# justinmgarrigus/accel-sim-framework-distributed

Hardware: AMD Instinct MI355X
Metric: sim KIPS (whole node) (higher is better)
Workload: dtype n/a (integer cycle-level model)

## Files before the change

csrc/bindings/py_asim.cc:

```cpp
#include <chrono>
#include <pybind11/functional.h>
#include <pybind11/numpy.h>
#include <pybind11/pybind11.h>
#include <pybind11/stl.h>

#include <cstring>

#include "../config/icnt_config.h"
#include "../driver/icnt_bench.h"
#include "../driver/simulator.h"
#include "../engine/icnt_sweep.h"

namespace py = pybind11;
using namespace asim;
static const size_t kLinkPktBytes = sizeof(LinkPkt);

namespace {

py::dict link_dict(const LinkParams& p) {
  py::dict d;
  d["link_gbps"] = p.link_gbps;
  d["latency_ns"] = p.latency_ns;
  d["links"] = p.links;
  d["slice_bytes"] = p.slice_bytes;
// ... 137 lines not shown
  for (int i = 0; i < 7; ++i) a[an[i]] = r.activity[i];
  d["activity"] = a;
  py::dict e;
  e["buffer"] = r.e_buffer;
  e["crossbar"] = r.e_xbar;
  e["link"] = r.e_link;
  e["allocator"] = r.e_alloc;
  e["leakage"] = r.e_leak;
  d["energy_pj"] = e;
  d["power_w"] = r.power_w;
  return d;
}

static std::vector<RequestReplyParams> rr_points_from(const std::vector<py::dict>& points) {
  std::vector<RequestReplyParams> ps;
  for (const py::dict& d : points) {
    RequestReplyParams p;
    for (const auto& kv : d) {
      const std::string k = py::cast<std::string>(kv.first);
      const py::handle v = kv.second;
      if (k == "traffic") p.traffic = py::cast<std::string>(v);
      else if (k == "rate") p.rate = py::cast<double>(v);
      else if (k == "cycles") p.cycles = py::cast<uint64_t>(v);
      else if (k == "warmup") p.warmup = py::cast<uint64_t>(v);
      else if (k == "seed") p.seed = py::cast<uint64_t>(v);
      else if (k == "write_fraction") p.write_fraction = py::cast<double>(v);
      else if (k == "read_request_size") p.read_request_size = py::cast<uint32_t>(v);
      else if (k == "read_reply_size") p.read_reply_size = py::cast<uint32_t>(v);
      else if (k == "write_request_size") p.write_request_size = py::cast<uint32_t>(v);
      else if (k == "write_reply_size") p.write_reply_size = py::cast<uint32_t>(v);
      else if (k == "reply_delay") p.reply_delay = py::cast<uint64_t>(v);
      else if (k == "mem_nodes") p.mem_nodes = py::cast<uint32_t>(v);
      else throw std::invalid_argument("icnt_request_reply_batch: point " + std::to_string(ps.size()) +
                                       ": unknown field '" + k + "'");
    }
    ps.push_back(p);
  }
  return ps;
}

PYBIND11_MODULE(_asim, m) {
  m.doc() = "MI355X-native trace-driven GPU simulator (native core)";
  m.attr("sizeof_SMState") = sizeof(SMState);
  m.attr("sizeof_ChanState") = sizeof(ChanState);
  m.attr("offsetof_SMState_skipped") = offsetof(SMState, skipped_cycles);
  m.attr("epoch_dependent_SMState") = std::vector<std::pair<size_t, size_t>>{
      {offsetof(SMState, skey), sizeof(SMState::skey)}, {offsetof(SMState, sref), sizeof(SMState::sref)},
      {offsetof(SMState, srank), sizeof(SMState::srank)}, {offsetof(SMState, pub_nz), sizeof(SMState::pub_nz)},
      {offsetof(SMState, skipped_cycles), sizeof(SMState::skipped_cycles)}};
  m.attr("epoch_dependent_ChanState") = std::vector<std::pair<size_t, size_t>>{
      {offsetof(ChanState, skey), sizeof(ChanState::skey)}, {offsetof(ChanState, sref), sizeof(ChanState::sref)},
      {offsetof(ChanState, srank), sizeof(ChanState::srank)}, {offsetof(ChanState, pub_nz), sizeof(ChanState::pub_nz)}};
  m.attr("sizeof_TInst") = sizeof(TInst);

  m.def("gpu_available", &gpu_engine_available, "True if a HIP device is usable by the GPU engine");
  {
    py::dict lim;
    lim["max_warps"] = kMaxWarps;
    lim["max_cta"] = kMaxCta;
    lim["l1_lines"] = kMaxL1Lines;
    lim["l1_mshr"] = kMaxL1Mshr;
    lim["l2_lines_per_channel"] = kMaxL2LinesCh;
    lim["l2_mshr"] = kMaxL2Mshr;
    lim["sm_total"] = kMaxSmTot;
    lim["sub_total"] = kMaxSubTot;
    m.attr("limits") = lim;
  }
  m.def("gpu_cu_count", &gpu_cu_count, "compute units of the current HIP device");
  m.def("gpu_pool_stats", &gpu_pool_stats, "GPU engine caching allocator: cached bytes, caps, trims");
  m.def("gpu_engine_modes", &gpu_engine_modes, "per GPU-engine build (lds / global / split): LDS bytes, blocks per CU, registers");
  m.def("gpu_batch_stats", &gpu_batch_stats, "global-state batch launches: batches, launches, blocks per CU");
  m.def("gpu_pool_trim", &gpu_pool_trim, "give the GPU engine allocator's cached blocks back to the driver");
  m.def("gpu_cus_per_sim", &gpu_cus_per_sim, "CUs one GPU-engine simulation of this shape reserves (ASIM_GPU_STATE)");
  m.def("gpu_engine_kernel_info", []() {
    const EngineKernelInfo k = gpu_engine_kernel_info();
    py::dict d;
    if (!k.valid) return d;
    d["vgprs_per_lane"] = k.num_regs;
    d["scratch_bytes_per_lane"] = k.local_bytes;
    d["lds_static"] = k.shared_static;
    d["lds_dynamic"] = k.lds_dynamic;
    d["max_threads_per_block"] = k.max_threads;
    d["binary_version"] = k.binary_version;
    d["sm_state_bytes"] = k.sm_state_bytes;
    d["chan_state_bytes"] = k.chan_state_bytes;
    return d;
  }, "compiled resources of the persistent HIP engine kernel (needs a GPU)");
  m.def("option_names", []() {
    OptionRegistry r;
    register_sim_options(r);
    return r.names();
  });
  m.def("unmodelled_option_warnings", [](const std::vector<std::string>& args) {
    OptionRegistry r;
    register_sim_options(r);
    r.parse_cmdline(args, false);
    return unmodelled_option_warnings(r);
  }, "warnings for options that are accepted but have no effect");
  m.def("parse_config", [](const std::vector<std::string>& args) { return cfg_dict(cfg_from_args(args)); },
        "derive the model configuration from accel-sim style arguments");
  m.def("addr_decode", [](const std::vector<std::string>& args, uint64_t addr) {
    SimCfg c = cfg_from_args(args);
    AddrTlx t = addr_decode(c, addr);
    py::dict d;
    d["chip"] = t.chip;
    d["bk"] = t.bk;
// ... 843 lines not shown
```

csrc/config/sim_options.cc:

```cpp
#include "sim_options.h"

#include <unistd.h>

#include "icnt_config.h"
#include "../model/addrdec.h"

#include <algorithm>
#include <cmath>
#include <cstring>
#include <sstream>

namespace asim {

namespace {

struct OptDef {
  const char* name;
  char type;
  const char* deflt;
  const char* help;
};

const OptDef kOptions[] = {
    {"-trace", 's', "./traces/kernelslist.g", "traces kernel list file"},
// ... 270 lines not shown
    {"-sim_check_corrupt_mailbox", 'u', "0", "-sim_engine check self-test: perturb a request-mailbox count instead of a unit state"},
    {"-sim_epochs_per_launch", 'u', "4096", "GPU engine epochs per persistent launch"},
    {"-sim_debug", 'b', "0", "interactive timing debugger (reference gpgpu_debug; also GPGPUSIM_DEBUG=1): single step, "
                            "PC / cycle breakpoints, memory-line watchpoints, pipeline dumps"},
    {"-sim_debug_script", 's', "", "debugger commands from this file instead of stdin"},
    {"-sim_debug_step", 'u', "0", "cycles per debugger step (0: one PDES epoch)"},
    {"-sim_break_cycle", 'u', "0", "enter the debugger when the simulation reaches this cycle (reference g_single_step)"},
    {"-collective_model", 's', "const", "const | ring | tree | packet collective timing"},
    {"-xgmi_link_bandwidth_gbps", 'f', "153.0", "per-link xGMI bandwidth (GB/s)"},
    {"-xgmi_link_latency_ns", 'f', "1000.0", "collective step latency (ns)"},
    {"-xgmi_links_per_gpu", 'u', "7", "xGMI links per GPU"},
    {"-sim_event_skip", 'b', "1", "fast-forward quiet SM cycles inside an epoch (results identical)"},
    {"-power_in_loop", 'b', "1",
     "power samples taken by the engine inside its cycle loop (GPU engine: in engine_kernel, f64 MFMA sums), "
     "0 = one engine run per sample with the host evaluating (results identical; DVFS always uses the latter)"},
    {"-trace_host_budget_mb", 'f', "0",
     "read a kernel's text trace per thread block, as the trace window advances, when the file is larger than this "
     "many MiB: host trace memory then follows the window (-gpu_trace_window, 2 when 0) instead of the kernel "
     "(0 = load whole kernels; results identical)"},
    {"-gpu_trace_window", 'i', "4",
     "GPU engine: kernel trace resident in HBM per kernel, in multiples of its resident-CTA capacity; CTAs "
     "stream in as they dispatch (0 = whole kernel; results identical)"},
    {"-sim_xcd", 'u', "0",
     "XCDs with private L2s (0 = one shared L2): SM s belongs to XCD s % N and uses the n_subpart/N slices of its XCD"},
    {"-sim_mall", 's', "none",
     "memory-attached last-level cache (Infinity Cache) per DRAM channel: <sets>:<assoc> of 128 B sectored lines, or none"},
    {"-sim_mall_miss_latency", 'u', "0", "extra core cycles of an HBM access over a MALL hit"},
    {"-sim_host_launch_interval", 'u', "0",
     "host model: core cycles between the host's kernel submissions after a sync (0 = a host that is never the "
     "bottleneck); a kernel submitted after the previous one ended launches into an idle GPU"},
    {"-sim_kernel_min_cycles_queued", 'u', "0",
     "a kernel queued right behind another lasts at least this many core cycles (the command processor's "
     "back-to-back dispatch interval of dependent kernels; 0 = off)"},
    {"-sim_first_kernel_latency", 'u', "0",
     "extra launch cycles of the run's first kernel behind the initial host copies (cold start: the copies' "
     "completion and the first touch of their pages; ub_launch after-copy)"},
    {"-sim_copy_latency_every_kernel", 'b', "0",
     "apply -sim_first_kernel_latency to every kernel launched behind a host copy, not only the run's first "
     "(ub_launch measures it on every one of its copy -> kernel repetitions)"},
    {"-collective_mem_traffic", 'b', "0",
     "run every collective's local memory traffic (send-buffer reads, receive-buffer writes) as an RCCL-style copy "
     "kernel that loads the simulated L2/MALL/HBM and contends with overlapping kernels"},
    {"-sim_l1_write_request_bytes", 'u', "128",
     "largest L1 -> L2 write request: 64 sends a store touching both halves of a line as two requests (gfx950 "
     "TCP -> TCC), 128 one per line"},
    {"-sim_single_valu", 'b', "0",
     "CDNA: integer, fp64 and transcendental vector instructions issue through the SIMD's one VALU (the SP unit of "
     "their scheduler, at their own initiation interval) instead of separate INT / DP / SFU pipelines"},
    {"-sim_l2_kernel_release", 'b', "0",
     "at the end of every kernel write the L2s' dirty sectors back to memory (the MALL if any) and invalidate them "
     "(the release / acquire of a multi-XCD GPU, whose XCD L2s are not coherent with each other)"},
    {"-sim_cpu_threads", 'u', "1", "CPU engine: OpenMP threads over the units of one epoch (1 = serial; "
                                  "run simulations job-parallel instead)"},
    {"-sim_router_pass", 's', "serial",
     "-icnt_link_contention 2: serial | par, the epoch pass over the routers: one lane (rt_simulate) or the "
     "lane-parallel pass (rt_simulate_par; on the GPU engine 64 lanes and one block per subnet); same results"},
    {"-sim_router_step_cap", 'u', "0",
     "-sim_router_pass par: loop iterations after which a pass gives up with an error (0 = the pass's own bound; "
     "a diagnostic)"},
    {"-icnt_capture", 's', "",
     "write every SM-to-L2 request and L2-to-SM reply packet the cycle engine injects to this file "
     "(model/icnt_capture.h; replay it with the standalone network mode)"},
    {"-icnt_capture_buf_kb", 'u', "0",
     "-icnt_capture: KB of the engine's log per subnet (0 = default; a diagnostic: a small log forces many "
     "hand-overs, on the GPU engine many launches)"},
    {"-collective_slice_bytes", 'u', "131072", "packet model: bytes per link packet (RCCL slice)"},
    {"-collective_max_channels", 'u', "16", "packet model: max parallel rings (channels)"},
    {"-collective_reduce_gbps", 'f', "900.0", "packet model: local memory bandwidth for reduce/copy (GB/s)"},
};

uint32_t parse_u(const std::string& s, const char* what) {
  char* end = nullptr;
  std::string t = trim(s);
  unsigned long v = strtoul(t.c_str(), &end, 0);
  if (t.empty() || *end) throw OptionError(std::string("bad integer '") + s + "' in " + what);
  return (uint32_t)v;
}

std::pair<uint32_t, uint32_t> parse_lat_ii(const std::string& s, const char* what) {
  auto v = split(strip_ws(s), ',');
  if (v.size() < 2) throw OptionError(std::string("expected <latency,initiation> for ") + what);
  return {parse_u(v[0], what), parse_u(v[1], what)};
}

void mask_limits(uint64_t m, uint8_t& hi, uint8_t& lo) {
  if (!m) {
    hi = 0;
    lo = 0;
    return;
  }
  lo = (uint8_t)__builtin_ctzll(m);
  hi = (uint8_t)(64 - __builtin_clzll(m));
}

uint32_t log2_floor(uint32_t x) {
  uint32_t r = 0;
  while ((1u << (r + 1)) <= x) ++r;
  return r;
}

void setup_addrdec(SimCfg& c, const std::string& mapping, int mask_mode) {
  int chip_s = 10;
  uint64_t m[AF_COUNT] = {0x0000000000001C00ull, 0x0000000000000300ull, 0x000000000FFF0000ull,
                          0x000000000000E0FFull, 0x000000000000000Full};
  switch (mask_mode) {
    case 0:
// ... 498 lines not shown
  c.rw_turnaround = r.getb("-dram_elimnate_rw_turnaround") ? 0u : 1u;
  c.wq_enable = r.getb("-dram_seperate_write_queue_enable") ? 1u : 0u;
  {
    auto v = split(strip_ws(r.gets("-dram_write_queue_size")), ':');
    if (v.size() != 3) throw OptionError("-dram_write_queue_size expects <size>:<high>:<low>");
    c.wq_size = parse_u(v[0], "-dram_write_queue_size");
    c.wq_hi = parse_u(v[1], "-dram_write_queue_size");
    c.wq_lo = parse_u(v[2], "-dram_write_queue_size");
    if (c.wq_enable) {
      c.wq_size = std::max<uint32_t>(1, std::min<uint32_t>(c.wq_size, kDramQ / 2));
      c.dram_queue = std::min<uint32_t>(c.dram_queue, (uint32_t)kDramQ - c.wq_size);
      c.wq_hi = std::min(c.wq_hi, c.wq_size);
      c.wq_lo = std::min(c.wq_lo, c.wq_hi);
    }
  }
  c.BL = (uint32_t)r.getu("-gpgpu_dram_burst_length");
  c.busW = (uint32_t)r.getu("-gpgpu_dram_buswidth");
  c.data_cmd_ratio = std::max<uint32_t>(1, (uint32_t)r.getu("-dram_data_command_freq_ratio"));
  c.dual_bus = (uint32_t)r.getu("-dram_dual_bus_interface");
  c.perfect_mem = r.getb("-gpgpu_perfect_mem") ? 1u : 0u;
  c.simple_dram = r.getb("-gpgpu_simple_dram_model") ? 1u : 0u;
  c.event_skip = r.getb("-sim_event_skip") ? 1u : 0u;
  c.trace_window = (uint32_t)std::max<long long>(0, r.geti("-gpu_trace_window"));
  {
    c.l1_wr_req_bytes = (uint32_t)r.getu("-sim_l1_write_request_bytes");
    c.single_valu = r.getb("-sim_single_valu") ? 1u : 0u;
    if (c.l1_wr_req_bytes != 64 && c.l1_wr_req_bytes != 128)
      throw OptionError("-sim_l1_write_request_bytes must be 64 or 128");
    c.n_xcd = (uint32_t)r.getu("-sim_xcd");
    c.log2_spx = 0;
    if (c.n_xcd > 1) {
      if (c.n_subpart % c.n_xcd) throw OptionError("-sim_xcd must divide the number of L2 sub-partitions");
      if (c.n_xcd > (uint32_t)kMaxXcd || c.n_xcd > c.n_sm)
        throw OptionError("-sim_xcd: at most " + std::to_string(kMaxXcd) + " XCDs and no more than the SMs");
      const uint32_t spx = c.n_subpart / c.n_xcd;
      if (spx & (spx - 1)) throw OptionError("-sim_xcd: sub-partitions per XCD must be a power of two");
      while ((1u << c.log2_spx) < spx) ++c.log2_spx;
    } else {
      c.n_xcd = 0;
    }
    c.mall_sets = c.mall_assoc = 0;
    const std::string m = strip_ws(r.gets("-sim_mall"));
    if (!m.empty() && m != "none" && m != "0") {
      auto v = split(m, ':');
      if (v.size() != 2) throw OptionError("-sim_mall expects <sets>:<assoc>");
      c.mall_sets = parse_u(v[0], "-sim_mall");
      c.mall_assoc = parse_u(v[1], "-sim_mall");
      if (!c.mall_sets || (c.mall_sets & (c.mall_sets - 1)) || !c.mall_assoc || c.mall_assoc > 64)
        throw OptionError("-sim_mall: sets must be a power of two and 1 <= assoc <= 64");
    }
    c.mall_miss_fs = (uint64_t)r.getu("-sim_mall_miss_latency");
  }
  c.cpu_threads = r.getu("-sim_cpu_threads");
  {
    const std::string rp = strip_ws(r.gets("-sim_router_pass"));
    if (rp != "serial" && rp != "par") throw OptionError("-sim_router_pass must be serial or par, not '" + rp + "'");
    c.router_pass = rp == "par" ? 1u : 0u;
    c.router_step_cap = r.getu("-sim_router_step_cap");
  }
  c.trace_mask = 0;
  if (r.getb("-trace_enabled")) {
    static const std::pair<const char*, uint32_t> streams[] = {
        {"WARP_SCHEDULER", TS_WARP_SCHEDULER},
        {"SCOREBOARD", TS_SCOREBOARD},
        {"MEMORY_PARTITION_UNIT", TS_MEMORY_PARTITION_UNIT},
        {"MEMORY_SUBPARTITION_UNIT", TS_MEMORY_SUBPARTITION_UNIT},
        {"INTERCONNECT", TS_INTERCONNECT},
        {"LIVENESS", TS_LIVENESS}};
    for (auto& tok : split(strip_ws(r.gets("-trace_components")), ',')) {
      if (tok.empty() || tok == "none") continue;
      bool found = false;
      for (auto& s : streams)
        if (tok == s.first || tok == "all") {
          c.trace_mask |= s.second;
          found = true;
        }
      if (!found) throw OptionError("-trace_components: unknown stream " + tok);
    }
  }
  c.trace_sm = (int32_t)r.geti("-trace_sampling_core");
  c.trace_mem = (int32_t)r.geti("-trace_sampling_memory_partition");
  c.trace_cap = 1u << 16;
  c.trace_ev = nullptr;
  c.trace_cnt = nullptr;
  c.bk_index_policy = (uint32_t)r.getu("-dram_bnk_indexing_policy");
  c.bkgrp_index_policy = (uint32_t)r.getu("-dram_bnkgrp_indexing_policy");
  c.atom_size = c.BL * c.busW * (uint32_t)r.getu("-gpgpu_n_mem_per_ctrlr");
  setup_addrdec(c, trim(r.gets("-gpgpu_mem_addr_mapping")), (int)r.geti("-gpgpu_mem_address_mask"));
  {
    uint32_t pi = (uint32_t)r.getu(user_set("-memory_partition_indexing") ? "-memory_partition_indexing"
                                                                           : "-gpgpu_memory_partition_indexing");
    if (pi > 5) throw OptionError("-gpgpu_memory_partition_indexing out of range");
    c.part_index = (uint8_t)pi;
  }
  {
    auto v = split(strip_ws(r.gets("-gpgpu_clock_domains")), ':');
    if (v.size() != 4) throw OptionError("-gpgpu_clock_domains expects 4 frequencies");
    double f[4];
    for (int i = 0; i < 4; ++i) {
      f[i] = atof(v[i].c_str());
      if (f[i] <= 0) throw OptionError("clock frequency must be positive");
    }
    c.per_core = (uint64_t)llround(1e9 / f[0]);
    c.per_icnt = (uint64_t)llround(1e9 / f[1]);
    c.per_l2 = (uint64_t)llround(1e9 / f[2]);
    c.per_dram = (uint64_t)llround(1e9 / f[3]);
// ... 182 lines not shown
```

csrc/driver/debugger.cc:

```cpp
#include "debugger.h"

#include <cstdio>
#include <fstream>
#include <iostream>
#include <sstream>

namespace asim {

Debugger::Debugger(const std::string& script, uint64_t stop_at, Hooks hooks) : h_(std::move(hooks)), stop_at_(stop_at) {
  if (!script.empty()) {
    file_.reset(new std::ifstream(script));
    if (!*file_) throw std::runtime_error("-sim_debug_script: cannot read " + script);
    from_file_ = true;
  }
  stepping_ = stop_at == 0;
  steps_left_ = stepping_ ? 1 : 0;
}

bool Debugger::next_line(std::string& line) {
  if (from_file_) return (bool)std::getline(*file_, line);
  std::fputs("(asim debugger) ", stdout);
  std::fflush(stdout);
  return (bool)std::getline(std::cin, line);
}

void Debugger::help() {
  h_.print(
      "asim debugger commands:\n"
      "  s [n]              step n steps (default 1) of -sim_debug_step cycles\n"
      "  c                  continue to the next breakpoint / watchpoint\n"
      "  b <pc> [sm] [warp] break when a warp issues the instruction at pc (hex)\n"
      "  bc <cycle>         break when the simulation reaches a cycle\n"
      "  w <addr>           watch memory requests to the 128 B line holding addr (hex)\n"
      "  d <id>             delete a breakpoint / watchpoint\n"
      "  l                  list breakpoints and watchpoints\n"
      "  dp [sm]            dump the pipeline of an SM (default: every busy SM)\n"
      "  dm [ch]            dump a memory channel (default: every busy channel)\n"
      "  i                  run status (cycle, instructions)\n"
      "  q                  stop the simulation here\n"
      "  h                  this help\n");
}

bool Debugger::after_step(uint64_t now, const std::vector<TraceEv>& ev, uint32_t n_sm, uint32_t l2_num,
                          uint32_t l2_den) {
  if (quit_) return false;
  bool stop = false;
  char b[256];
  for (const TraceEv& e : ev)
    for (auto& kv : bps_) {
      Bp& bp = kv.second;
      bool hit = false;
      if (bp.kind == Bp::PC && e.kind == EV_ISSUE && (e.b & 0xffffffffull) == bp.v &&
          (bp.sm < 0 || e.unit == (uint32_t)bp.sm) && (bp.warp < 0 || e.a == (uint16_t)bp.warp)) {
        hit = true;
        snprintf(b, sizeof(b), "asim debugger: breakpoint %d hit: core %u warp %u issued pc 0x%llx at cycle %llu\n",
                 kv.first, e.unit, e.a, (unsigned long long)bp.v, (unsigned long long)e.cycle);
      } else if (bp.kind == Bp::ADDR && (e.b >> 7) == (bp.v >> 7)) {
        if (e.kind == EV_PKT_SEND && e.unit < n_sm) {
          hit = true;
          snprintf(b, sizeof(b),
                   "asim debugger: watchpoint %d hit: core %u sends a request for line 0x%llx (addr 0x%llx) to "
                   "sub-partition %u at cycle %llu\n",
                   kv.first, e.unit, (unsigned long long)e.b, (unsigned long long)bp.v, e.a,
                   (unsigned long long)e.cycle);
        } else if (e.kind == EV_L2_ACCESS) {
          static const char* o[] = {"hit", "miss", "mshr-hit", "write-through"};
          hit = true;
          snprintf(b, sizeof(b),
                   "asim debugger: watchpoint %d hit: channel %u sub %u L2 %s for line 0x%llx at cycle ~%llu\n",
                   kv.first, e.unit - n_sm, e.a >> 8, o[e.a & 3], (unsigned long long)e.b,
                   (unsigned long long)(l2_den ? e.cycle * l2_num / l2_den : e.cycle));
        }
      }
      if (hit) {
        ++bp.hits;
        h_.print(b);
        stop = true;
      }
    }
  for (auto& kv : bps_)
    if (kv.second.kind == Bp::CYCLE && !kv.second.hits && now >= kv.second.v) {
      ++kv.second.hits;
      snprintf(b, sizeof(b), "asim debugger: breakpoint %d hit: cycle %llu reached (now %llu)\n", kv.first,
               (unsigned long long)kv.second.v, (unsigned long long)now);
      h_.print(b);
      stop = true;
    }
  if (stop_at_ && now >= stop_at_) {
    stop_at_ = 0;
    stop = true;
  }
// ... 34 lines not shown
      bp.v = std::stoull(pc, nullptr, 16);
      is >> bp.sm >> bp.warp;
      bps_[next_id_] = bp;
      snprintf(b, sizeof(b), "breakpoint %d at pc 0x%llx\n", next_id_++, (unsigned long long)bp.v);
      h_.print(b);
    } else if (cmd == "bc") {
      Bp bp{Bp::CYCLE, 0};
      if (!(is >> bp.v)) {
        h_.print("usage: bc <cycle>\n");
        continue;
      }
      bps_[next_id_] = bp;
      snprintf(b, sizeof(b), "breakpoint %d at cycle %llu\n", next_id_++, (unsigned long long)bp.v);
      h_.print(b);
    } else if (cmd == "w" || cmd == "watch") {
      std::string a;
      if (!(is >> a)) {
        h_.print("usage: w <addr>\n");
        continue;
      }
      Bp bp{Bp::ADDR, std::stoull(a, nullptr, 16)};
      bps_[next_id_] = bp;
      snprintf(b, sizeof(b), "watchpoint %d on line 0x%llx\n", next_id_++, (unsigned long long)(bp.v & ~127ull));
      h_.print(b);
    } else if (cmd == "d" || cmd == "delete") {
      int id = 0;
      is >> id;
      h_.print(bps_.erase(id) ? "deleted\n" : "no such breakpoint\n");
    } else if (cmd == "l" || cmd == "list") {
      if (bps_.empty()) h_.print("no breakpoints\n");
      for (auto& kv : bps_) {
        const Bp& p = kv.second;
        if (p.kind == Bp::PC)
          snprintf(b, sizeof(b), "%d: break pc 0x%llx sm %d warp %d (hits %llu)\n", kv.first,
                   (unsigned long long)p.v, p.sm, p.warp, (unsigned long long)p.hits);
        else if (p.kind == Bp::CYCLE)
          snprintf(b, sizeof(b), "%d: break cycle %llu (hits %llu)\n", kv.first, (unsigned long long)p.v,
                   (unsigned long long)p.hits);
        else
          snprintf(b, sizeof(b), "%d: watch line 0x%llx (hits %llu)\n", kv.first, (unsigned long long)(p.v & ~127ull),
                   (unsigned long long)p.hits);
        h_.print(b);
      }
    } else if (cmd == "dp") {
      int sm = -1;
      is >> sm;
      h_.print(h_.dump(sm, -2));
    } else if (cmd == "dm") {
      int ch = -1;
      is >> ch;
      h_.print(h_.dump(-2, ch));
    } else if (cmd == "i" || cmd == "info") {
      h_.print(h_.status() + "\n");
    } else if (cmd == "q" || cmd == "quit") {
      quit_ = true;
      h_.print("asim debugger: simulation stopped by the user\n");
      return false;
    } else if (cmd == "h" || cmd == "help") {
      help();
    } else {
      h_.print("unknown command '" + cmd + "' (h for help)\n");
    }
  }
  bps_.clear();
  stepping_ = false;
  return true;
}

}
```

csrc/driver/debugger.h:

```cpp
#pragma once
#include <cstdint>
#include <functional>
#include <istream>
#include <map>
#include <memory>
#include <string>
#include <vector>

#include "../model/config.h"

namespace asim {

class Debugger {
 public:
  struct Hooks {
    std::function<void(const std::string&)> print;
    std::function<std::string(int sm, int ch)> dump;
    std::function<std::string()> status;
  };
  Debugger(const std::string& script, uint64_t stop_at, Hooks hooks);

  static uint32_t trace_mask() { return TS_WARP_SCHEDULER | TS_INTERCONNECT | TS_MEMORY_SUBPARTITION_UNIT; }

  bool after_step(uint64_t now, const std::vector<TraceEv>& ev, uint32_t n_sm, uint32_t l2_to_core_num,
                  uint32_t l2_to_core_den);

  size_t commands_run() const { return ncmd_; }

 private:
  struct Bp {
    enum Kind { PC, ADDR, CYCLE } kind;
    uint64_t v;
    int sm = -1;
    int warp = -1;
    uint64_t hits = 0;
  };
  bool prompt(uint64_t now);
  bool next_line(std::string& line);
  void help();

  Hooks h_;
  std::unique_ptr<std::istream> file_;
  bool from_file_ = false;
  bool stepping_ = true;
  uint64_t steps_left_ = 0;
  uint64_t stop_at_ = 0;
  std::map<int, Bp> bps_;
  int next_id_ = 1;
  size_t ncmd_ = 0;
  bool quit_ = false;
};

}
```

csrc/driver/simulator.cc:

```cpp
#include "simulator.h"

#include <sys/stat.h>

#include <algorithm>
#include <cmath>
#include <cstdarg>
#include <cstring>
#include <filesystem>
#include <stdexcept>

namespace asim {

template <class T>
static void stat_delta(const std::vector<T>& a, const std::vector<T>& b, std::vector<T>& out) {
  static_assert(sizeof(T) % 8 == 0, "stat structs are arrays of 64-bit counters");
  out.resize(a.size());
  for (size_t i = 0; i < a.size(); ++i) {
    const uint64_t* x = (const uint64_t*)&a[i];
    uint64_t* o = (uint64_t*)&out[i];
    if (i < b.size()) {
      const uint64_t* y = (const uint64_t*)&b[i];
      for (size_t k = 0; k < sizeof(T) / 8; ++k) o[k] = x[k] - y[k];
    } else {
      for (size_t k = 0; k < sizeof(T) / 8; ++k) o[k] = x[k];
// ... 46 lines not shown
  }
  ~CaptureFile() override {
    try {
      finish();
    } catch (...) {
    }
  }
};

uint64_t Simulator::icnt_capture_packets(uint32_t subnet) const { return capture_ ? capture_->h.count[subnet ? 1 : 0] : 0; }

Simulator::Simulator(const std::vector<std::string>& args) {
  t_start_ = std::chrono::steady_clock::now();
  register_sim_options(reg_);
  reg_.parse_cmdline(args, false);
  cfg_ = derive_sim_cfg(reg_);
  dopt_ = derive_driver_opts(reg_);
  if (dopt_.engine == "gpu") {
    eng_ = make_gpu_engine();
    if (!eng_) throw std::runtime_error("-sim_engine gpu requested but the HIP engine is unavailable");
    if (dopt_.gpu_ingest) ingest_dev_ = gpu_current_device();
  } else if (dopt_.engine == "cpu") {
    eng_ = make_cpu_engine();
  } else if (dopt_.engine == "check") {
    std::unique_ptr<Engine> primary;
    if (dopt_.check_primary == "gpu") {
      primary = make_gpu_engine();
      if (!primary) throw std::runtime_error("-sim_engine check: the HIP engine is unavailable");
    } else if (dopt_.check_primary == "cpu") {
      primary = make_cpu_engine();
    } else {
      throw OptionError("-sim_check_primary must be cpu or gpu");
    }
    eng_ = make_check_engine(std::move(primary), make_cpu_engine(), dopt_.check_interval, dopt_.check_corrupt_at,
                             dopt_.check_corrupt_mailbox != 0);
  } else {
    throw OptionError("-sim_engine must be cpu, gpu or check");
  }
  print_mask_ = cfg_.trace_mask;
  if (dopt_.debug) {
    cfg_.trace_mask |= Debugger::trace_mask();
    print_sm_ = cfg_.trace_sm;
    print_mem_ = cfg_.trace_mem;
    cfg_.trace_sm = -1;
    cfg_.trace_mem = -1;
    Debugger::Hooks h;
    h.print = [this](const std::string& s) { print("%s", s.c_str()); };
    h.dump = [this](int sm, int ch) { return dump_pipeline(sm, ch); };
    h.status = [this]() {
      char b[200];
      snprintf(b, sizeof(b), "cycle %llu, kernels completed %zu, thread instructions of completed kernels %llu",
               (unsigned long long)eng_->now(), results_.size(), (unsigned long long)tot_insn_);
      return std::string(b);
    };
    dbg_.reset(new Debugger(dopt_.debug_script, dopt_.break_cycle, h));
  }
  eng_->init(cfg_);
  if (!dopt_.icnt_capture.empty()) {
    capture_.reset(new CaptureFile(dopt_.icnt_capture, cfg_));
    eng_->capture_arm(capture_.get(), dopt_.icnt_capture_buf_kb);
  } else if (dopt_.icnt_capture_buf_kb) {
    throw OptionError("-icnt_capture_buf_kb needs -icnt_capture");
  }
  per_core_nom_ = cfg_.per_core;
  if (dopt_.power_enabled) {
    power_.reset(new PowerModel());
    std::string err;
    if (!power_->load_xml(dopt_.power_xml, &err)) throw std::runtime_error("power model: " + err);
    power_->set_param("dvfs_min_clock_ratio",
                      std::max(power_->param("dvfs_min_clock_ratio", 0.0), dopt_.dvfs_min_clock_ratio));
    power_report_.reset(new std::ofstream(dopt_.power_report_file));
    if (!*power_report_) throw std::runtime_error("cannot write " + dopt_.power_report_file);
    if (power_->param("energy_model", 0.0) >= 1.0) {
      ArchEnergyParams ap;
      ap.node_nm = power_->param("core_tech_node", ap.node_nm);
      ap.vdd = power_->param("core_vdd", 0.0);
      ap.dram_pj_per_bit = power_->param("dram_pj_per_bit", ap.dram_pj_per_bit);
      ap.dram_act_nj = power_->param("dram_act_nj", ap.dram_act_nj);
      ap.tensor_macs_per_lane = power_->param("tensor_macs_per_lane", 0.0);
      const ArchEnergy ae = arch_energy(cfg_, ap);
      power_->set_base(ae.base_nj);
      *power_report_ << "architectural energy model (energy_model = 1)\n" << arch_energy_report(ae) << "\n";
    }
    if (dopt_.power_trace) {
      power_trace_.reset(new std::ofstream("accelwattch_power_trace.csv"));
      ptrack_.write_trace_header(*power_trace_);
    }
    if (dopt_.steady_power) {
      power_steady_.reset(new std::ofstream("accelwattch_steady_state.csv"));
      *power_steady_ << "kernel,start_cycle,end_cycle,samples,avg_power\n";
      ptrack_.set_steady(dopt_.steady_dev_pct, dopt_.steady_samples);
    }
  }
  if (dopt_.visualizer) {
    visualizer_.reset(new std::ofstream(dopt_.visualizer_file));
    if (!*visualizer_) throw std::runtime_error("cannot write " + dopt_.visualizer_file);
  }
}

Simulator::~Simulator() = default;

void Simulator::print(const char* fmt, ...) {
  char buf[4096];
  va_list ap;
  va_start(ap, fmt);
  int n = vsnprintf(buf, sizeof(buf), fmt, ap);
// ... 1351 lines not shown
```

csrc/engine/cpu_engine.cc:

```cpp
#include <cstdlib>
#include <cstring>
#include <stdexcept>

#include <functional>

#include <atomic>
#include <exception>
#include <mutex>

#include "../model/icnt_router_par.h"
#include "engine.h"
#include "thread_team.h"
#include "trace_window.h"

namespace asim {

uint32_t reply_cap(const SimCfg& c) {
  uint64_t win = (uint64_t)c.icnt_latency * std::max(c.per_core, c.per_core_max);
  return (uint32_t)((win + c.per_icnt - 1) / c.per_icnt + 1);
}

uint32_t icnt_cap_log_records(const SimCfg& c, uint32_t cap_req, uint32_t cap_rep, uint64_t buf_kb) {
  const uint64_t worst = icnt_cap_epoch_max(c, std::max(cap_req, cap_rep));
  const uint64_t min_kb = (worst * sizeof(IcntCapRec) + 1023) / 1024;
  if (!buf_kb)
    buf_kb = std::max(min_kb, std::min(kIcntCapMaxDefaultKb, std::max(kIcntCapDefaultKb, kIcntCapDefaultEpochs * min_kb)));
  const uint64_t recs = buf_kb * 1024 / sizeof(IcntCapRec);
  if (recs < worst)
    throw std::invalid_argument("-icnt_capture_buf_kb " + std::to_string(buf_kb) +
                                ": the log must hold one epoch's worst case, " + std::to_string(worst) +
                                " records per subnet: at least " + std::to_string(min_kb) + " KB");
  return (uint32_t)std::min<uint64_t>(recs, 0x7fffffffu);
}

void check_core_clock(const SimCfg& c, uint64_t per_core) {
  if (per_core == 0 || per_core > std::max(c.per_core, c.per_core_max))
    throw std::runtime_error("set_core_clock: core period beyond the configured DVFS range (-dvfs_min_clock_ratio)");
}

void init_sm_state(SMState& s, uint32_t id) {
  memset(&s, 0, sizeof(SMState));
  s.id = id;
}

void init_chan_state(ChanState& ch, uint32_t id, const SimCfg& c) {
  memset(&ch, 0, sizeof(ChanState));
  ch.id = id;
  ch.t_icnt = 0;
  ch.t_l2 = 0;
  ch.t_dram = 0;
  (void)c;
}

void host_memcpy_fill(ChanState* chs, uint32_t nch, const SimCfg& c, uint64_t addr, uint64_t bytes) {
  if (c.l2.disabled || c.n_xcd) return;
  const uint64_t first = addr & ~127ull;
  const uint64_t last = (addr + bytes + 127) & ~127ull;
  uint64_t cap_lines = (uint64_t)c.l2.nsets * c.l2.assoc * c.n_subpart;
  uint64_t start = first;
  if ((last - first) / 128 > 2 * cap_lines) start = last - 2 * cap_lines * 128;
  for (uint64_t line = start; line < last; line += 128) {
    AddrTlx t = addr_decode(c, line);
    uint32_t ch = t.sub / c.n_sub_per_mem, sub = t.sub % c.n_sub_per_mem;
    if (ch >= nch) continue;
// ... 20 lines not shown
  if (h.n_sm != w.n_sm || h.n_mem != w.n_mem || h.sm_bytes != w.sm_bytes || h.ch_bytes != w.ch_bytes ||
      h.pub_bytes != w.pub_bytes || h.box_req != w.box_req || h.cnt_req != w.cnt_req || h.box_rep != w.box_rep ||
      h.cnt_rep != w.cnt_rep || h.ovf != w.ovf || h.mall != w.mall || h.links != w.links)
    throw std::runtime_error("engine state: image was written for a different configuration or build");
}

void host_flush_l2(ChanState* chs, uint32_t nch, const SimCfg& c, bool writeback, L2Line* mall) {
  const uint32_t per_sub = c.l2.nsets * c.l2.assoc;
  for (uint32_t i = 0; i < nch; ++i) {
    ChanState& ch = chs[i];
    if (writeback && !c.l2.disabled) {
      for (uint32_t j = 0; j < c.n_sub_per_mem; ++j) {
        MemStats& st = ch.sp[j].st;
        const L2Line* T = l2_tags(ch, c, j);
        for (uint32_t k = 0; k < per_sub; ++k) {
          const L2Line& L = T[k];
          if (!L.dirty) continue;
          const uint32_t n = (uint32_t)popc64(L.dirty);
          st.l2_mem_wr += n;
          st.l2_mem_wr_req += wr_requests(L.dirty);
          st.l2_evict_dirty++;
          if (!mall) {
            st.dram_wr += n;
            continue;
          }
          L2Line* b = mall + (size_t)i * mall_lines(c) + (size_t)mall_set(c, L.tag) * c.mall_assoc;
          int w = mall_find<SeqPar>(b, c.mall_assoc, L.tag);
          if (w < 0) {
            w = mall_victim<SeqPar>(b, c.mall_assoc);
            if (b[w].valid && b[w].dirty) {
              const uint32_t nv = (uint32_t)popc64(b[w].dirty);
              ch.sp[0].st.mall_wb += nv;
              ch.sp[0].st.dram_wr += nv;
            }
            b[w] = L2Line{};
            b[w].tag = L.tag;
          }
          b[w].valid |= L.dirty;
          b[w].dirty |= L.dirty;
          b[w].lru = ++ch.mall_stamp;
          ch.sp[0].st.mall_wr += n;
        }
      }
    }
    for (auto& L : ch.l2) {
      L.valid = 0;
      L.dirty = 0;
    }
  }
}

namespace {

class CpuEngine : public Engine {
 public:
  const char* name() const override { return "cpu"; }

  void init(const SimCfg& c) override {
    c_ = c;
    sms_.assign(c.n_sm, SMState());
    for (uint32_t i = 0; i < c.n_sm; ++i) init_sm_state(sms_[i], i);
    chs_.assign(c.n_mem, ChanState());
    for (uint32_t i = 0; i < c.n_mem; ++i) init_chan_state(chs_[i], i, c);
    pub_.reset(new EpochPub());
    memset(pub_.get(), 0, sizeof(EpochPub));
    cap_req_ = c.icnt_latency;
    cap_rep_ = reply_cap(c);
    for (int p = 0; p < 2; ++p) {
      box_req_[p].assign((size_t)c.n_subpart * c.n_sm * cap_req_, Pkt{});
      cnt_req_[p].assign((size_t)c.n_subpart * c.n_sm, 0);
      box_rep_[p].assign((size_t)c.n_sm * c.n_subpart * cap_rep_, Pkt{});
      cnt_rep_[p].assign((size_t)c.n_sm * c.n_subpart, 0);
    }
    ovf_cap_ = backlog_cap(c);
    ovf_.assign((size_t)c.n_subpart * ovf_cap_, Pkt{});
    mall_.assign((size_t)(c.n_mem * mall_lines(c)), L2Line{});
    link_free_.clear();
    link_refs_.clear();
    n_link_state_ = 0;
    rt_pc_ = RtPassCount{};
    if (c.link_contention && (icnt_link_count(c) > kMaxIcntLinks || !icnt_contention_fits(c, cap_req_, cap_rep_) ||
                              icnt_scratch_words(c, cap_req_, cap_rep_) > kMaxIcntScratchWords))
      throw std::runtime_error("-icnt_link_contention: topology or mailboxes too large for the link pass");
    if (icnt_contention_on(c)) {
      n_link_state_ = (size_t)icnt_state_words(c, cap_req_, cap_rep_);
      link_free_.assign(n_link_state_ + kIcntStatWords, 0);
      link_refs_.assign((size_t)icnt_scratch_words(c, cap_req_, cap_rep_), 0);
    }
    epoch_ = 0;
    cycle_ = 0;
    kt_ = KernelTab{};
    kt_.mix = c.concurrent_kernel_sm;
    if (c_.trace_mask) {
      const size_t units = (size_t)c.n_sm + c.n_mem;
      trace_ev_.assign(units * c_.trace_cap, TraceEv{});
      trace_cnt_.assign(units, 0);
      c_.trace_ev = trace_ev_.data();
      c_.trace_cnt = trace_cnt_.data();
    }
  }

  void trace_drain(std::vector<TraceEv>& out, uint64_t* dropped) override {
    out.clear();
    for (size_t u = 0; u < trace_cnt_.size(); ++u) {
      const uint32_t n = trace_cnt_[u], k = std::min(n, c_.trace_cap);
      out.insert(out.end(), trace_ev_.begin() + (long)(u * c_.trace_cap), trace_ev_.begin() + (long)(u * c_.trace_cap + k));
      if (dropped) *dropped += n - k;
      trace_cnt_[u] = 0;
    }
  }

  void launch(uint32_t slot, ReadyKernel& k, const KernelDesc& kd) override {
    if (slot >= (uint32_t)kMaxConc || (kt_.active >> slot & 1u)) throw std::runtime_error("launch: kernel slot busy");
    if (!k.streamed() && k.insts.size() > kIdxMask) throw std::runtime_error("kernel trace exceeds 2^29 warp instructions");
    KernelDesc& d = kt_.k[slot];
    d = kd;
    tw_.launch(slot, k, d, c_);
    kt_.active |= 1u << slot;
  }
  uint32_t running() const override { return kt_.active; }

  RunResult run(const RunLimits& lim) override {
    RunResult res;
    if (!kt_.active) {
      res.end_cycle = cycle_;
      return res;
    }
    const uint32_t nthr = std::max<uint32_t>(1, std::min<uint32_t>(c_.cpu_threads, (uint32_t)(sms_.size() + chs_.size())));
    bar_.reset(nthr);
    const uint64_t epoch0 = epoch_, cycle0 = cycle_;
    uint64_t end_epoch = epoch0, end_cycle = cycle0;
    std::atomic<bool> abort{false};
    std::exception_ptr err;
    std::mutex err_mu;
    auto fail = [&]() {
      std::lock_guard<std::mutex> g(err_mu);
      if (!err) err = std::current_exception();
      abort.store(true, std::memory_order_release);
    };
    std::function<void(uint32_t)> job = [&](uint32_t tid) {
      const SimCfg& c = c_;
      const uint64_t E = c.icnt_latency;
      const int nsm = (int)sms_.size(), nch = (int)chs_.size();
      uint64_t epoch = epoch0, cycle = cycle0, epochs = 0;
      bool refill = true;
      uint64_t pw_next = pw_on_ ? pw_.t_prev + pw_.freq : 0;
      uint64_t reqm[2] = {~0ull, ~0ull}, repm[2] = {~0ull, ~0ull};
      RunResult r;
      for (;;) {
        if (refill && tw_.any_streamed()) {
          if (nthr > 1) bar_.wait();
          if (tid == 0) {
            try {
              tw_.ensure(kt_, c, [&](DispatchView& v) { read_dispatch(v); });
            } catch (...) {
              fail();
            }
          }
          if (nthr > 1) bar_.wait();
          if (abort.load(std::memory_order_acquire)) break;
        }
        const uint32_t cur = (uint32_t)(epoch & 1), prev = cur ^ 1u;
        const uint64_t t0 = cycle, t1 = t0 + E;
        const int s0 = (int)((uint64_t)nsm * tid / nthr), s1 = (int)((uint64_t)nsm * (tid + 1) / nthr);
        const int c0 = (int)((uint64_t)nch * tid / nthr), c1 = (int)((uint64_t)nch * (tid + 1) / nthr);
        try {
        for (int q = 0; q < (s1 - s0) + (c1 - c0); ++q) {
          const int i = q < s1 - s0 ? s0 + q : nsm + c0 + (q - (s1 - s0));
          if (i < nsm) {
            SMState& s = sms_[i];
            SmCtx x = ctx_sm(cur);
            sm_epoch<SeqPar>(s, x, *pub_, prev, t0, t1, box_rep_[prev].data(), cnt_rep_[prev].data(), cap_rep_,
                             c.n_subpart, epoch, repm);
            sm_publish<SeqPar>(s, x, *pub_, cur);
          } else {
            ChanState& ch = chs_[i - nsm];
            MemCtx m = ctx_mem(cur, t1);
            m.mall = mall_.empty() ? nullptr : mall_.data() + (size_t)(i - nsm) * mall_lines(c);
            chan_epoch<SeqPar>(ch, m, box_req_[prev].data(), cnt_req_[prev].data(), cap_req_, core_fs(c, t0), reqm);
            chan_publish<SeqPar>(ch, m, *pub_, cur);
          }
        }
        } catch (...) {
          fail();
        }
        if (nthr > 1) bar_.wait();
        if (abort.load(std::memory_order_acquire)) break;
        if (cap_sink_ && tid == 0) {
          try {
            capture_epoch(cur);
          } catch (...) {
            fail();
          }
        }
        if (!link_free_.empty()) {
          if (tid == 0) {
            try {
              if (router_par()) {
                if (rt_epoch_run_par<SeqPar>(c, box_req_[cur].data(), cnt_req_[cur].data(), cap_req_,
                                             box_rep_[cur].data(), cnt_rep_[cur].data(), cap_rep_, link_free_.data(),
                                             link_refs_.data(), RT_DIR_BOTH, &rt_pc_) != RT_STATUS_OK)
                  throw std::runtime_error(kRouterStepCapMsg);
              } else {
                icnt_epoch_pass<SeqPar>(c, box_req_[cur].data(), cnt_req_[cur].data(), cap_req_, box_rep_[cur].data(),
                                        cnt_rep_[cur].data(), cap_rep_, link_free_.data(), link_refs_.data());
              }
            } catch (...) {
              fail();
            }
          }
          if (nthr > 1) bar_.wait();
          if (abort.load(std::memory_order_acquire)) break;
        }
        const uint64_t mc = pw_on_ ? (lim.max_cycle ? std::min(lim.max_cycle, pw_next) : pw_next) : lim.max_cycle;
        const EpochDecision d = epoch_decide<SeqPar>(c, *pub_, cur, t1, kt_, epoch, mc);
        refill = d.refill != 0;
        reqm[0] = d.req_dst[0];
        reqm[1] = d.req_dst[1];
        repm[0] = d.rep_dst[0];
        repm[1] = d.rep_dst[1];
        ++epoch;
        ++epochs;
        cycle = d.next_start;
        if (pw_on_) {
          const bool exits = d.done || d.deadlock || d.limit || (lim.max_cycle && cycle >= lim.max_cycle) ||
                             (lim.max_epochs && epochs >= lim.max_epochs);
          if (exits || cycle >= pw_next) {
            if (tid == 0) {
              try {
                power_sample(cycle);
              } catch (...) {
                fail();
              }
            }
            if (nthr > 1) bar_.wait();
            if (abort.load(std::memory_order_acquire)) break;
            pw_next = cycle + pw_.freq;
          }
        }
        if (d.done) {
          r.done = true;
          r.done_mask = d.done;
        } else if (d.deadlock) {
          r.deadlock = true;
        } else if (d.limit) {
          r.hit_limit = true;
          r.cap = true;
        } else if ((lim.max_cycle && cycle >= lim.max_cycle) || (lim.max_epochs && epochs >= lim.max_epochs)) {
          r.hit_limit = true;
        } else {
          continue;
        }
        break;
      }
      if (tid == 0) {
        r.epochs = epochs;
        res = r;
        end_epoch = epoch;
        end_cycle = cycle;
      }
    };
    team_.run(nthr, job);
    if (err) std::rethrow_exception(err);
    if (cap_sink_) capture_flush();
    epoch_ = end_epoch;
    cycle_ = end_cycle;
    if (res.done) {
      kt_.active &= ~res.done_mask;
      for (uint32_t k = 0; k < (uint32_t)kMaxConc; ++k)
        if (res.done_mask >> k & 1u) tw_.done(k);
    }
    res.end_cycle = cycle_;
    return res;
  }

  uint64_t now() const override { return cycle_; }
  void trace_residency(uint64_t* peak_bytes, uint64_t* refills) const override {
    *peak_bytes = tw_.resident_peak;
    *refills = tw_.refills;
  }
  bool power_sampler() const override { return true; }
  void power_arm(const PwrArm& a) override {
    pw_ = a;
    pw_on_ = true;
    pw_out_.clear();
  }
  void power_disarm() override { pw_on_ = false; }
  void power_drain(std::vector<PwrSample>& out) override {
    out.swap(pw_out_);
    pw_out_.clear();
  }
  void power_sample(uint64_t now) {
    std::vector<const MemStats*> mem;
    for (auto& ch : chs_)
      for (uint32_t j = 0; j < c_.n_sub_per_mem; ++j) mem.push_back(&ch.sp[j].st);
    std::vector<const SMStats*> sm(sms_.size());
    for (size_t i = 0; i < sms_.size(); ++i) sm[i] = &sms_[i].st;
    double S[PS_COUNT];
    pwr_sums_of(sm.data(), sm.size(), mem.data(), mem.size(), S);
    pw_out_.push_back(pwr_take(pw_, S, now));
  }
  void read_dispatch(DispatchView& v) const {
    const SMState& s0 = sms_[0];
    memcpy(v.k_uid, s0.k_uid, sizeof(v.k_uid));
    memcpy(v.next_cta, s0.next_cta, sizeof(v.next_cta));
    memcpy(v.next_ctax, s0.next_ctax, sizeof(v.next_ctax));
    v.sms.resize(sms_.size());
    for (size_t m = 0; m < sms_.size(); ++m) {
      memcpy(v.sms[m].cta_id, sms_[m].cta_id, sizeof(v.sms[m].cta_id));
      memcpy(v.sms[m].cta_valid, sms_[m].cta_valid, sizeof(v.sms[m].cta_valid));
      memcpy(v.sms[m].cta_ks, sms_[m].cta_ks, sizeof(v.sms[m].cta_ks));
    }
  }
  struct HostMem {
// ... 15 lines not shown
    host_memcpy_fill(chs_.data(), (uint32_t)chs_.size(), c_, addr, bytes);
  }
  void set_core_clock(uint64_t per_core, uint64_t base_cyc, uint64_t base_fs) override {
    check_core_clock(c_, per_core);
    c_.per_core = per_core;
    c_.clk_base_cyc = base_cyc;
    c_.clk_base_fs = base_fs;
    cfg_set_divs(c_);
  }
  void flush_l2(bool writeback) override {
    host_flush_l2(chs_.data(), (uint32_t)chs_.size(), c_, writeback, mall_.empty() ? nullptr : mall_.data());
  }

  void stats(std::vector<SMStats>& sm, std::vector<MemStats>& mem) override {
    sm.clear();
    mem.clear();
    for (auto& s : sms_) sm.push_back(s.st);
    for (auto& ch : chs_)
      for (uint32_t j = 0; j < c_.n_sub_per_mem; ++j) mem.push_back(ch.sp[j].st);
  }

  void snapshot(std::vector<uint8_t>& out) override {
    out.resize(sms_.size() * sizeof(SMState) + chs_.size() * sizeof(ChanState) + mall_.size() * sizeof(L2Line) +
               n_link_state_ * 8);
    uint8_t* p = out.data();
    for (auto& s : sms_) {
      memcpy(p, &s, sizeof(SMState));
      p += sizeof(SMState);
    }
    for (auto& ch : chs_) {
      memcpy(p, &ch, sizeof(ChanState));
      p += sizeof(ChanState);
    }
    if (!mall_.empty()) memcpy(p, mall_.data(), mall_.size() * sizeof(L2Line));
    p += mall_.size() * sizeof(L2Line);
    if (n_link_state_) memcpy(p, link_free_.data(), n_link_state_ * 8);
  }
  void restore(const std::vector<uint8_t>& in) override {
    if (in.size() != sms_.size() * sizeof(SMState) + chs_.size() * sizeof(ChanState) + mall_.size() * sizeof(L2Line) +
                         n_link_state_ * 8)
      throw std::runtime_error("snapshot size mismatch");
    const uint8_t* p = in.data();
    for (auto& s : sms_) {
      memcpy(&s, p, sizeof(SMState));
      p += sizeof(SMState);
    }
    for (auto& ch : chs_) {
      memcpy(&ch, p, sizeof(ChanState));
      p += sizeof(ChanState);
    }
    if (!mall_.empty()) memcpy(mall_.data(), p, mall_.size() * sizeof(L2Line));
    p += mall_.size() * sizeof(L2Line);
    if (n_link_state_) memcpy(link_free_.data(), p, n_link_state_ * 8);
  }
  void link_stats(uint64_t* delayed, uint64_t* wait_cycles, uint64_t* deadlocked) override {
    *delayed = n_link_state_ ? link_free_[n_link_state_] : 0;
    *wait_cycles = n_link_state_ ? link_free_[n_link_state_ + 1] : 0;
    if (deadlocked) *deadlocked = n_link_state_ ? link_free_[n_link_state_ + 2] : 0;
  }
  void capture_arm(IcntCapSink* sink, uint64_t buf_kb) override {
    uint32_t recs = icnt_cap_log_records(c_, cap_req_, cap_rep_, buf_kb);
    const uint64_t worst = icnt_cap_epoch_max(c_, std::max(cap_req_, cap_rep_));
    if (!buf_kb) recs = (uint32_t)std::min<uint64_t>(recs, std::max<uint64_t>(worst, 65536));
    for (int d = 0; d < 2; ++d) {
      cap_rec_[d].assign(recs, IcntCapRec{});
      cap_off_[d].assign((size_t)c_.n_sm * c_.n_subpart, 0);
      cap_log_[d] = IcntCapLog{cap_rec_[d].data(), cap_off_[d].data(), 0, recs};
    }
    cap_sink_ = sink;
  }
  void capture_epoch(uint32_t cur) {
    const uint64_t worst = icnt_cap_epoch_max(c_, std::max(cap_req_, cap_rep_));
    if (cap_log_[0].n + worst > cap_log_[0].cap || cap_log_[1].n + worst > cap_log_[1].cap) capture_flush();
    icnt_capture_append<SeqPar>(c_, 0, box_req_[cur].data(), cnt_req_[cur].data(), cap_req_, &cap_log_[0]);
    icnt_capture_append<SeqPar>(c_, 1, box_rep_[cur].data(), cnt_rep_[cur].data(), cap_rep_, &cap_log_[1]);
  }
  void capture_flush() {
    for (uint32_t d = 0; d < 2; ++d) {
      if (cap_log_[d].n) cap_sink_->put(d, cap_log_[d].rec, cap_log_[d].n);
      cap_log_[d].n = 0;
    }
  }
  bool router_par() const { return c_.link_contention == 2 && c_.router_pass == 1 && !link_free_.empty(); }
  RouterPassStats router_pass_stats() override {
    RouterPassStats r;
    r.mode = c_.router_pass == 1 ? "par" : "serial";
    if (!router_par()) return r;
    r.passes = rt_pc_.passes[0] + rt_pc_.passes[1];
    r.max_packets_req = rt_pc_.max_np[0];
    r.max_packets_rep = rt_pc_.max_np[1];
    r.split_blocks = 1;
    return r;
  }
  void advance(uint64_t cycles) override {
    uint64_t E = c_.icnt_latency;
    cycle_ += (cycles + E - 1) / E * E;
  }

  EngineStateHeader header() const {
    EngineStateHeader h;
    h.n_sm = sms_.size();
    h.n_mem = chs_.size();
    h.sm_bytes = sizeof(SMState);
    h.ch_bytes = sizeof(ChanState);
    h.pub_bytes = sizeof(EpochPub);
    h.box_req = box_req_[0].size();
    h.cnt_req = cnt_req_[0].size();
    h.box_rep = box_rep_[0].size();
    h.cnt_rep = cnt_rep_[0].size();
    h.ovf = ovf_.size();
    h.mall = mall_.size();
    h.links = link_free_.size();
    h.cycle = cycle_;
    h.epoch = epoch_;
    h.ready = kt_.active;
    return h;
  }

  void save_state(std::vector<uint8_t>& out) override {
    out.clear();
    StateOut o{out};
    EngineStateHeader h = header();
    o.put(&h, sizeof(h));
    o.put(sms_.data(), sms_.size() * sizeof(SMState));
    o.put(chs_.data(), chs_.size() * sizeof(ChanState));
    o.put(pub_.get(), sizeof(EpochPub));
    for (int p = 0; p < 2; ++p) {
      o.put(box_req_[p].data(), box_req_[p].size() * sizeof(Pkt));
      o.put(cnt_req_[p].data(), cnt_req_[p].size() * sizeof(uint32_t));
      o.put(box_rep_[p].data(), box_rep_[p].size() * sizeof(Pkt));
      o.put(cnt_rep_[p].data(), cnt_rep_[p].size() * sizeof(uint32_t));
    }
    o.put(ovf_.data(), ovf_.size() * sizeof(Pkt));
    o.put(mall_.data(), mall_.size() * sizeof(L2Line));
    if (!link_free_.empty()) o.put(link_free_.data(), link_free_.size() * 8);
  }

  void load_state(const std::vector<uint8_t>& in) override {
    StateIn r{in};
    EngineStateHeader h;
    r.get(&h, sizeof(h));
    check_state_header(h, header());
    r.get(sms_.data(), sms_.size() * sizeof(SMState));
    r.get(chs_.data(), chs_.size() * sizeof(ChanState));
    r.get(pub_.get(), sizeof(EpochPub));
    for (int p = 0; p < 2; ++p) {
      r.get(box_req_[p].data(), box_req_[p].size() * sizeof(Pkt));
      r.get(cnt_req_[p].data(), cnt_req_[p].size() * sizeof(uint32_t));
      r.get(box_rep_[p].data(), box_rep_[p].size() * sizeof(Pkt));
      r.get(cnt_rep_[p].data(), cnt_rep_[p].size() * sizeof(uint32_t));
    }
    r.get(ovf_.data(), ovf_.size() * sizeof(Pkt));
    r.get(mall_.data(), mall_.size() * sizeof(L2Line));
    if (!link_free_.empty()) r.get(link_free_.data(), link_free_.size() * 8);
    cycle_ = h.cycle;
    epoch_ = h.epoch;
    if (h.ready) throw std::runtime_error("engine state: image taken with kernels running");
  }

 private:
  SmCtx ctx_sm(uint32_t cur) {
    SmCtx x;
    x.cfg = &c_;
    x.kt = &kt_;
    x.outbox = box_req_[cur].data();
    x.outcnt = cnt_req_[cur].data();
    x.out_cap = cap_req_;
    x.n_src_sm = c_.n_sm;
    x.rt_st = c_.link_contention == 2 && !link_free_.empty() ? link_free_.data() : nullptr;
    return x;
  }
  MemCtx ctx_mem(uint32_t cur, uint64_t t1) {
    MemCtx m;
    m.cfg = &c_;
    m.outbox = box_rep_[cur].data();
    m.outcnt = cnt_rep_[cur].data();
    m.out_cap = cap_rep_;
    m.n_src_sub = c_.n_subpart;
    m.win_end = core_fs(c_, t1);
    m.ovf = ovf_.data();
    m.ovf_cap = ovf_cap_;
    m.mall = nullptr;
    m.rt_st = c_.link_contention == 2 && !link_free_.empty() ? link_free_.data() : nullptr;
    return m;
  }

  SimCfg c_{};
  std::vector<SMState> sms_;
  std::vector<ChanState> chs_;
  std::unique_ptr<EpochPub> pub_;
  std::vector<Pkt> box_req_[2], box_rep_[2];
  std::vector<uint32_t> cnt_req_[2], cnt_rep_[2];
  uint32_t cap_req_ = 0, cap_rep_ = 0;
  std::vector<Pkt> ovf_;
  std::vector<L2Line> mall_;
  uint32_t ovf_cap_ = 0;
  std::vector<uint64_t> link_free_;
  std::vector<uint32_t> link_refs_;
  size_t n_link_state_ = 0;
  RtPassCount rt_pc_{};
  IcntCapSink* cap_sink_ = nullptr;
  std::vector<IcntCapRec> cap_rec_[2];
  std::vector<uint32_t> cap_off_[2];
  IcntCapLog cap_log_[2]{};
  uint64_t epoch_ = 0, cycle_ = 0;
  KernelTab kt_{};
};

}

std::unique_ptr<Engine> make_cpu_engine() { return std::unique_ptr<Engine>(new CpuEngine()); }

}
```

csrc/engine/engine.h:

```cpp
#pragma once
#include <cstring>
#include <memory>
#include <stdexcept>
#include <map>
#include <string>
#include <vector>

#include "../model/epoch.h"
#include "../model/icnt_capture.h"
#include "../power/power_eval.h"
#include "../trace/trace.h"

namespace asim {

struct RunLimits {
  uint64_t max_cycle = 0;
  uint64_t max_epochs = 0;
};

struct PwrArm {
  PwrCoef coef;
  uint64_t freq = 0;
  uint64_t t_prev = 0;
  double s_prev[PS_COUNT] = {};
  uint32_t n_sm = 0;
};

struct RunResult {
  uint64_t end_cycle = 0;
  uint64_t epochs = 0;
  bool done = false;
  uint32_t done_mask = 0;
  bool deadlock = false;
  bool hit_limit = false;
  bool cap = false;
};

struct RouterPassStats {
  const char* mode = "serial";
  uint64_t passes = 0;
  uint32_t max_packets_req = 0, max_packets_rep = 0;
  uint32_t split_blocks = 0;
};
constexpr const char* kRouterStepCapMsg = "router pass hit its step cap (-sim_router_step_cap / rt_step_cap)";

struct IcntCapSink {
  virtual ~IcntCapSink() = default;
  virtual void put(uint32_t subnet, const IcntCapRec* rec, size_t n) = 0;
};
constexpr uint64_t kIcntCapDefaultKb = 4096, kIcntCapMaxDefaultKb = 256 * 1024;
constexpr uint64_t kIcntCapDefaultEpochs = 256;
uint32_t icnt_cap_log_records(const SimCfg& c, uint32_t cap_req, uint32_t cap_rep, uint64_t buf_kb);

class Engine {
 public:
  virtual ~Engine() = default;
  virtual const char* name() const = 0;
  virtual void init(const SimCfg& c) = 0;
  virtual void launch(uint32_t slot, ReadyKernel& k, const KernelDesc& kd) = 0;
  virtual RunResult run(const RunLimits& lim) = 0;
  virtual uint32_t running() const = 0;
  virtual uint64_t now() const = 0;
  virtual void memcpy_fill_l2(uint64_t addr, uint64_t bytes) = 0;
  virtual void flush_l2(bool writeback = false) = 0;
  virtual void set_core_clock(uint64_t per_core, uint64_t base_cyc, uint64_t base_fs) = 0;
  virtual void stats(std::vector<SMStats>& sm, std::vector<MemStats>& mem) = 0;
  virtual void snapshot(std::vector<uint8_t>& out) = 0;
  virtual void restore(const std::vector<uint8_t>& in) = 0;
  virtual void advance(uint64_t cycles) = 0;
  virtual void save_state(std::vector<uint8_t>& out) = 0;
  virtual void load_state(const std::vector<uint8_t>& in) = 0;
  virtual void trace_drain(std::vector<TraceEv>& out, uint64_t* dropped) = 0;
  virtual void trace_residency(uint64_t* peak_bytes, uint64_t* refills) const {
    *peak_bytes = 0;
    *refills = 0;
  }
  virtual uint64_t launches() const { return 0; }
  virtual const char* kernel_variant() const { return ""; }
  virtual uint32_t kernel_blocks() const { return 0; }
  virtual void link_stats(uint64_t* delayed, uint64_t* wait_cycles, uint64_t* deadlocked = nullptr) {
    *delayed = 0;
    *wait_cycles = 0;
    if (deadlocked) *deadlocked = 0;
  }
  virtual RouterPassStats router_pass_stats() { return RouterPassStats{}; }
  virtual void capture_arm(IcntCapSink*, uint64_t ) {
    throw std::runtime_error("engine cannot capture the network traffic");
  }
  virtual bool power_sampler() const { return false; }
  virtual void power_arm(const PwrArm&) { throw std::runtime_error("engine has no in-loop power sampler"); }
  virtual void power_disarm() {}
  virtual void power_drain(std::vector<PwrSample>& out) { out.clear(); }
};

inline void pwr_sums_of(const SMStats* const* sm, size_t nsm, const MemStats* const* mem, size_t nmem, double* S) {
  for (int j = 0; j < PS_COUNT; ++j) S[j] = 0;
// ... 102 lines not shown
```

csrc/engine/gpu_engine.hip:

```cpp
#include <hip/hip_runtime.h>

#include <algorithm>
#include <cerrno>
#include <csignal>
#include <cstdio>
#include <cstring>
#include <map>
#include <memory>
#include <stdexcept>
#include <string>

#include <fcntl.h>
#include <sys/file.h>
#include <sys/stat.h>
#include <unistd.h>
#include <chrono>
#include <condition_variable>
#include <deque>
#include <mutex>
#include <vector>

#include "engine_kernel.h"
#include "trace_window.h"

// ... 1168 lines not shown
  uint32_t* d_cap_off_[2] = {nullptr, nullptr};
  uint32_t cap_recs_ = 0, cap_epochs_ = 0;
  uint32_t cap_win_left_ = 0;
  std::vector<IcntCapRec> cap_host_;
  uint32_t ovf_cap_ = 0;
  Pkt* d_box_req_[2] = {nullptr, nullptr};
  uint32_t* d_cnt_req_[2] = {nullptr, nullptr};
  Pkt* d_box_rep_[2] = {nullptr, nullptr};
  uint32_t* d_cnt_rep_[2] = {nullptr, nullptr};
  GpuCtl* d_ctl_ = nullptr;
  GpuCtl* h_ctl_ = nullptr;
  TraceEv* d_trace_ev_ = nullptr;
  uint32_t* d_trace_cnt_ = nullptr;
  struct DevMem {
    static constexpr bool kHost = false;
    void* alloc(size_t n) {
      void* p = nullptr;
      pool_alloc(&p, n);
      return p;
    }
    void free(void* p) {
      DevicePool::get().dev_free(p);
    }
    void write(void* d, const void* h, size_t n) { HIPCHECK(hipMemcpy(d, h, n, hipMemcpyHostToDevice)); }
  };
  TraceWindows<DevMem> tw_;
  uint64_t launches_ = 0;
  const char* variant_ = "";
  bool pw_on_ = false;
  PwrDev* d_pw_ = nullptr;
  double* d_pw_rows_ = nullptr;
  PwrSample* d_pw_ring_ = nullptr;
  uint32_t pw_cap_ = 0;
  std::vector<PwrSample> pw_out_;
  KernelTab kt_{};
  KernelTab* d_kt_ = nullptr;
  uint32_t cap_req_ = 0, cap_rep_ = 0;
  uint64_t epoch_ = 0, cycle_ = 0;
  uint32_t epochs_per_launch_ = 4096;
  bool profiling_ = false;
  bool sliced_ = false;
  int mode_ = kModeLds;
  bool global_ = false;
  bool batch_ = false;
  uint32_t slots_ = kCuSlots;
  uint64_t* d_prof_ = nullptr;
  uint32_t* d_ework_ = nullptr;

 public:
  void dump_profile() {
    if (!profiling_) return;
    std::vector<uint64_t> h((size_t)nblocks_ * kProfSlots);
    HIPCHECK(hipMemcpy(h.data(), d_prof_, h.size() * 8, hipMemcpyDeviceToHost));
    static const char* names[kProfSlots] = {
        "sm.receive", "sm.writeback", "sm.hit_complete", "sm.ldst", "sm.dispatch", "sm.read_operands",
        "sm.alloc_oc", "sm.issue", "sm.fetch", "sm.retire", "sm.inject", "sm.occupancy", "sm.gather",
        "sm.cta_dispatch", "sm.refill", "sm.cycle_loop", "sm.publish", "#sm_cycles", "#quiet_checks", "#epochs_busy", "mem.gather", "mem.dram",
        "mem.l2", "mem.icnt", "mem.window_other", "mem.publish", "barrier", "decide", "post", "sm.issue_sched", "#slowest", "launch_rest",
        "#max_work/epoch", "#epochs(b0)", "#last_arriver_wait", "#last_arrivals", "ldst.l1_probe", "ldst.mshr_find",
        "ldst.pend_reg", "ldst.send", "recv.xbar", "recv.l1_fill", "issue.one", "issue.pick", "quiet_check", "skip",
        "ldst.hit_push", "fill.pend_wake", "iss.pick", "iss.classify", "iss.step1", "iss.step2", "iss.step3",
        "iss.spare53", "iss.spare54", "iss.spare55"};
    double sm[kProfSlots] = {}, mc[kProfSlots] = {}, smt = 0, mct = 0;
    for (uint32_t b = 0; b < nblocks_; ++b)
      for (int k = 0; k < kProfSlots; ++k) {
        double v = (double)h[(size_t)b * kProfSlots + k];
        const bool counter = (k >= 17 && k <= 19) || k == 30 || (k >= 32 && k <= 35);
        if (b < c_.n_sm) { sm[k] += v / c_.n_sm; smt += counter ? 0 : v / c_.n_sm; }
        else { const double nmb = nblocks_ > c_.n_sm ? (double)(nblocks_ - c_.n_sm) : 1.0; mc[k] += v / nmb; mct += counter ? 0 : v / nmb; }
      }
    {
      double cyc_clk = 0, n_cyc = 0, n_q = 0, n_ep = 0, q_clk = 0;
      for (uint32_t b = 0; b < c_.n_sm; ++b) {
        for (int k = 0; k <= 11; ++k) cyc_clk += (double)h[(size_t)b * kProfSlots + k];
        for (int k = 36; k <= 43; ++k) cyc_clk += (double)h[(size_t)b * kProfSlots + k];
        cyc_clk += (double)h[(size_t)b * kProfSlots + 29] + (double)h[(size_t)b * kProfSlots + 46] +
                   (double)h[(size_t)b * kProfSlots + 47];
        for (int k = 48; k <= 52; ++k) cyc_clk += (double)h[(size_t)b * kProfSlots + k];
        q_clk += (double)h[(size_t)b * kProfSlots + 44] + (double)h[(size_t)b * kProfSlots + 45];
        n_cyc += (double)h[(size_t)b * kProfSlots + 17];
        n_q += (double)h[(size_t)b * kProfSlots + 18];
        n_ep += (double)h[(size_t)b * kProfSlots + 19];
      }
      fprintf(stderr, "[asim gpu profile] SM cycles simulated %.0f (%.0f clocks each), quiet checks %.0f "
                      "(cycle_loop %.0f clocks each), busy SM-epochs %.0f\n",
              n_cyc, n_cyc ? cyc_clk / n_cyc : 0, n_q, n_q ? q_clk / n_q : 0, n_ep);
    }
    {
      double mx = 0, ne = 0, lw = 0, nl = 0;
      for (uint32_t b = 0; b < nblocks_; ++b) {
        mx += (double)h[(size_t)b * kProfSlots + 32];
        ne += (double)h[(size_t)b * kProfSlots + 33];
        lw += (double)h[(size_t)b * kProfSlots + 34];
        nl += (double)h[(size_t)b * kProfSlots + 35];
      }
      fprintf(stderr, "[asim gpu profile] epochs %.0f: slowest block's work %.0f clocks/epoch; last arriver's "
                      "barrier wait %.0f clocks/epoch (pure barrier latency)\n",
              ne, ne ? mx / ne : 0, nl ? lw / nl : 0);
    }
    {
      std::vector<std::pair<uint64_t, uint32_t>> sl;
      for (uint32_t b = 0; b < nblocks_; ++b) sl.push_back({h[(size_t)b * kProfSlots + 30], b});
      std::sort(sl.rbegin(), sl.rend());
      fprintf(stderr, "[asim gpu profile] slowest block per epoch (epochs, block, its SM cycles / quiet checks):");
      for (size_t i = 0; i < sl.size() && i < 8 && sl[i].first; ++i)
        fprintf(stderr, " %llu x b%u (%s, %llu/%llu)", (unsigned long long)sl[i].first, sl[i].second,
                sl[i].second < c_.n_sm ? "SM" : "MEM", (unsigned long long)h[(size_t)sl[i].second * kProfSlots + 17],
                (unsigned long long)h[(size_t)sl[i].second * kProfSlots + 18]);
      fprintf(stderr, "\n");
    }
    uint32_t crit = 0;
    double crit_work = -1;
    for (uint32_t b = 0; b < nblocks_; ++b) {
      double w = 0;
      for (int k = 0; k < kProfSlots; ++k)
        if (k != 26 && k != 30 && !(k >= 17 && k <= 19) && !(k >= 32 && k <= 35)) w += (double)h[(size_t)b * kProfSlots + k];
      if (w > crit_work) { crit_work = w; crit = b; }
    }
    fprintf(stderr, "[asim gpu profile] shader-clock cycles per block (mean), share of block time; "
                    "CRIT = block %u (%s), the one with the least barrier wait\n", crit, crit < c_.n_sm ? "SM" : "MEM");
    double ct = 0;
    for (int k = 0; k < kProfSlots; ++k)
      if (k != 30 && !(k >= 17 && k <= 19) && !(k >= 32 && k <= 35)) ct += (double)h[(size_t)crit * kProfSlots + k];
    for (int k = 0; k < kProfSlots; ++k) {
      const double cv = (double)h[(size_t)crit * kProfSlots + k];
      if (sm[k] + mc[k] > 0)
        fprintf(stderr, "  %-18s SM %14.0f (%5.1f%%)   MEM %14.0f (%5.1f%%)   CRIT %14.0f (%5.1f%%)\n", names[k], sm[k],
                100 * sm[k] / smt, mc[k], 100 * mc[k] / mct, cv, 100 * cv / ct);
    }
  }

};

}

bool gpu_engine_available() {
  int n = 0;
  if (hipGetDeviceCount(&n) != hipSuccess) return false;
  return n > 0;
}

std::unique_ptr<Engine> make_gpu_engine() {
  if (!gpu_engine_available()) return nullptr;
  return std::unique_ptr<Engine>(new GpuEngine());
}

}

namespace asim {
std::map<std::string, uint64_t> gpu_pool_stats() {
  const DevicePool::Stats t = DevicePool::get().stats();
  return {{"cached_dev", t.cached_dev}, {"cached_host", t.cached_host}, {"cap_dev", t.cap_dev},
          {"cap_host", t.cap_host}, {"trims", t.trims}, {"freed_over_cap", t.freed_over_cap}};
}
void gpu_pool_trim() { DevicePool::get().trim(); }
void* gpu_pool_alloc(size_t bytes) { return DevicePool::get().dev(bytes); }
void gpu_pool_release(void* p) { DevicePool::get().dev_free(p); }
std::map<std::string, std::map<std::string, uint64_t>> gpu_engine_modes() {
  std::map<std::string, std::map<std::string, uint64_t>> out;
  const struct {
    const char* name;
    int mode;
    const void* f;
    size_t lds;
  } ms[] = {{"lds", kModeLds, (const void*)engine_kernel<WavePar, false, kModeLds>, kLdsBytes},
            {"global", kModeGlobal, (const void*)engine_batch_kernel, kLdsBytesGlobal},
            {"split", kModeSplit, (const void*)engine_kernel<WavePar, true, kModeSplit>, kLdsBytesSplit},
            {"split2", kModeSplit, (const void*)engine_split2_kernel, kLdsBytesSplit}};
  for (const auto& m : ms) {
    auto& o = out[m.name];
    o["lds_bytes"] = m.lds;
    o["blocks_per_cu"] = mode_blocks_per_cu(m.mode);
    int occ = 0;
    if (m.mode == kModeLds) (void)hipFuncSetAttribute(m.f, hipFuncAttributeMaxDynamicSharedMemorySize, (int)kLdsBytes);
    if (hipOccupancyMaxActiveBlocksPerMultiprocessor(&occ, m.f, 64, (int)m.lds) == hipSuccess) o["occupancy_api"] = occ;
    hipFuncAttributes fa;
    if (hipFuncGetAttributes(&fa, m.f) == hipSuccess) {
      o["num_regs"] = (uint64_t)fa.numRegs;
      o["scratch_bytes_per_lane"] = (uint64_t)fa.localSizeBytes;
    }
// ... 54 lines not shown
```

csrc/engine/wave_par.h:

```cpp
#pragma once
#include <hip/hip_runtime.h>

#include "../model/hd.h"
#include "sm_view.h"

namespace asim {

struct WavePar {
  static constexpr int kLanes = 64;
  static __device__ __forceinline__ int lane() { return (int)(threadIdx.x & 63); }

  template <class F>
  static __device__ __forceinline__ uint64_t ballot(int n, F&& f) {
    const int l = lane();
    bool p = false;
    if (l < n) p = f(l);
    return (uint64_t)__ballot(p);
  }
  template <class F>
  static __device__ __forceinline__ void lane_loop(int n, F&& f) {
    for (int i = lane(); i < n; i += 64) f(i);
  }
  static __device__ __forceinline__ uint32_t red_sum(uint32_t v) {
    return wave_reduce(v, [](uint32_t a, uint32_t b) { return a + b; });
// ... 20 lines not shown
    step(dpp<0xB1>(h), dpp<0xB1>(l));
    step(dpp<0x4E>(h), dpp<0x4E>(l));
    step(dpp<0x141>(h), dpp<0x141>(l));
    step(dpp<0x140>(h), dpp<0x140>(l));
    uint32_t rh = rdl(h, 0), rl = rdl(l, 0);
#pragma unroll
    for (int r = 16; r < 64; r += 16) {
      const uint32_t oh = rdl(h, r), ol = rdl(l, r);
      const bool take = kMax ? (oh > rh || (oh == rh && ol > rl)) : (oh < rh || (oh == rh && ol < rl));
      if (take) { rh = oh; rl = ol; }
    }
    return ((uint64_t)rh << 32) | rl;
  }
  static __device__ __forceinline__ uint64_t red_min64(uint64_t v) { return red64<false>(v); }
  static __device__ __forceinline__ uint64_t red_max64(uint64_t v) { return red64<true>(v); }
  template <class F>
  static __device__ __forceinline__ uint64_t ballot_m(uint64_t mask, F&& f) {
    const int l = lane();
    bool p = false;
    if ((mask >> l) & 1ull) p = f(l);
    return (uint64_t)__ballot(p);
  }
  template <class F>
  static __device__ __forceinline__ void each_m(uint64_t mask, F&& f) {
    const int l = lane();
    if ((mask >> l) & 1ull) f(l);
  }
  template <class F>
  static __device__ __forceinline__ void each(int n, F&& f) {
    for (int i = lane(); i < n; i += 64) f(i);
  }
  template <class F>
  static __device__ __forceinline__ void one(F&& f) {
    if (lane() == 0) f();
  }
  template <class T>
  static __device__ __forceinline__ void fetch_copy(T* dst, const T* src, int n) {
    static_assert(sizeof(T) % 16 == 0, "fetch_copy: 16-byte granular records");
    typedef __attribute__((address_space(1))) const uint4 g4;
    typedef __attribute__((address_space(3))) uint4 l4;
    const int chunks = n * (int)(sizeof(T) / 16);
    const int l = lane();
    if (l >= chunks) return;
    typedef __attribute__((address_space(0))) const void flat_cv;
    if (!__builtin_amdgcn_is_shared((flat_cv*)dst)) {
      reinterpret_cast<uint4*>(dst)[l] = reinterpret_cast<const uint4*>(src)[l];
      return;
    }
    __builtin_amdgcn_global_load_lds((g4*)(reinterpret_cast<const uint4*>(src) + l), (l4*)dst, 16, 0, 0);
  }
  static __device__ __forceinline__ void fetch_wait() { asm volatile("s_waitcnt vmcnt(0)" ::: "memory"); }
  static __device__ __forceinline__ void prof(int) {}
  static __device__ __forceinline__ void tick(int) {}
  template <class T>
  static __device__ __forceinline__ T uni(T v) {
    static_assert(sizeof(T) <= 4 || sizeof(T) % 4 == 0, "uni: 1/2/4-byte or word-multiple types");
    static_assert(std::is_trivially_copyable<T>::value, "uni: values only (cast proxies first)");
    if constexpr (sizeof(T) <= 4) {
      uint32_t u = 0;
      __builtin_memcpy(&u, &v, sizeof(T));
      u = (uint32_t)__builtin_amdgcn_readfirstlane((int)u);
      T r;
      __builtin_memcpy(&r, &u, sizeof(T));
      return r;
    } else {
      uint32_t w[sizeof(T) / 4];
      __builtin_memcpy(w, &v, sizeof(T));
#pragma unroll
      for (int i = 0; i < (int)(sizeof(T) / 4); ++i) w[i] = (uint32_t)__builtin_amdgcn_readfirstlane((int)w[i]);
      T r;
      __builtin_memcpy(&r, w, sizeof(T));
      return r;
    }
  }

  static __device__ __forceinline__ void sync() {
    __builtin_amdgcn_fence(__ATOMIC_SEQ_CST, "wavefront");
    __builtin_amdgcn_wave_barrier();
  }
  template <class S, class F>
  static __device__ __forceinline__ void view(S& s, F&& f) {
    sync();
    SmView<S> v(s);
    f(v);
    v.flush();
    sync();
  }
  template <int Ctrl>
  static __device__ __forceinline__ uint32_t dpp(uint32_t v) {
    return (uint32_t)__builtin_amdgcn_update_dpp((int)v, (int)v, Ctrl, 0xf, 0xf, false);
  }
  static __device__ __forceinline__ uint32_t rdl(uint32_t v, int l) {
    return (uint32_t)__builtin_amdgcn_readlane((int)v, l);
  }
  template <class Op>
  static __device__ __forceinline__ uint32_t row_reduce(uint32_t v, Op op) {
    v = op(v, dpp<0xB1>(v));
    v = op(v, dpp<0x4E>(v));
    v = op(v, dpp<0x141>(v));
    v = op(v, dpp<0x140>(v));
    return v;
  }
  template <class Op>
  static __device__ __forceinline__ uint32_t wave_reduce(uint32_t v, Op op) {
    v = row_reduce(v, op);
    return op(op(rdl(v, 0), rdl(v, 16)), op(rdl(v, 32), rdl(v, 48)));
// ... 152 lines not shown
```

csrc/model/config.h:

```cpp
#pragma once
#include "types.h"

namespace asim {

constexpr int kMaxWarps = 64;
constexpr int kMaxWarpLanes = 64;
constexpr int kMaxCta = 32;
constexpr int kMaxSched = 4;
constexpr int kIbuf = 2;
constexpr int kWin = 4;
constexpr int kMaxEpoch = 256;
constexpr int kMaxOC = 16;
constexpr int kMaxBanks = 32;
constexpr int kWbRing = 512;
constexpr int kWbSlot = 8;
constexpr int kMaxL1Lines = 1024;
constexpr int kMaxL1Mshr = 256;
constexpr int kMaxIL1Lines = 512;
constexpr int kMaxIL1Mshr = 16;
constexpr int kMaxCL1Lines = 1024;
constexpr int kMaxCL1Mshr = 32;
constexpr uint64_t kProgramMemStart = 0xF0000000ull;
constexpr uint64_t kScalarBase = 0x7FFE00000000ull;
constexpr int kMaxPend = 1024;
// ... 202 lines not shown
  uint16_t rt_buf;
  uint16_t rt_speedup_q8;
  uint16_t rt_inbuf;
  CacheGeom l2;
  uint32_t rop_latency;
  uint32_t dram_latency;
  uint32_t q_icnt_l2, q_l2_dram, q_dram_l2, q_l2_icnt;
  uint32_t perf_memcpy;
  uint32_t dram_sched;
  uint32_t dram_queue;
  uint32_t dram_ret_queue;
  uint32_t dram_credits;
  uint32_t nbk, nbkgrp, tCCD, tRRD, tRCD, tRAS, tRP, tRC, CL, WL, tCDLR, tWR, tCCDL, tRTPL;
  uint32_t BL, busW, data_cmd_ratio, dual_bus, bk_index_policy, bkgrp_index_policy;
  uint32_t atom_size;
  uint32_t rw_turnaround;
  uint32_t wq_enable;
  uint32_t wq_size, wq_hi, wq_lo;
  uint64_t addr_mask[AF_COUNT];
  uint8_t mk_hi[AF_COUNT];
  uint8_t mk_lo[AF_COUNT];
  uint8_t part_index;
  uint8_t gap;
  int32_t addr_chip_s;
  uint32_t log2ch, log2sub, n_ch_pow2;
  uint64_t sub_id_mask;
  BitRuns addr_runs[AF_COUNT];
  BitRuns part_runs;
  uint64_t per_core, per_icnt, per_l2, per_dram;
  uint64_t clk_base_cyc, clk_base_fs;
  uint64_t per_core_max;
  Div64 dv_core, dv_icnt, dv_l2, dv_dram;
  Div64 dv_epoch;
  uint32_t kernel_launch_latency;
  uint32_t kernel_launch_latency_queued;
  uint32_t tb_launch_latency;
  uint32_t deadlock_window;
  uint64_t max_insn;
  uint32_t max_completed_cta;
  uint32_t trace_window;
  uint32_t max_cycle_lo, max_cycle_hi;
  uint32_t perfect_mem;
  uint32_t simple_dram;
  uint32_t event_skip;
  uint32_t n_xcd;
  uint32_t l1_wr_req_bytes;
  uint32_t single_valu;
  uint32_t log2_spx;
  uint32_t mall_sets, mall_assoc;
  uint64_t mall_miss_fs;
  uint32_t cpu_threads;
  uint32_t router_pass;
  uint64_t router_step_cap;
  uint32_t trace_mask;
  int32_t trace_sm;
  int32_t trace_mem;
  uint32_t trace_cap;
  TraceEv* trace_ev;
  uint32_t* trace_cnt;
};

SIM_HDI void trace_put(const SimCfg& c, uint32_t unit, uint64_t cycle, uint16_t kind, uint16_t a, uint64_t b) {
  uint32_t n = c.trace_cnt[unit];
  if (n < c.trace_cap) {
    TraceEv& e = c.trace_ev[(uint64_t)unit * c.trace_cap + n];
    e.cycle = cycle;
    e.unit = unit;
    e.kind = kind;
    e.a = a;
    e.b = b;
  }
  c.trace_cnt[unit] = n + 1;
}
enum IcntTopo : uint8_t { TOPO_FLY = 0, TOPO_MESH, TOPO_TORUS, TOPO_CMESH, TOPO_FATTREE, TOPO_FLATFLY };

SIM_HDI uint32_t icnt_routers(const SimCfg& c, uint32_t a, uint32_t b) {
  const uint32_t k = c.topo_k ? c.topo_k : 2, n = c.topo_n ? c.topo_n : 1;
  switch (c.topo) {
    case TOPO_FLY:
      return n;
    case TOPO_CMESH:
      a /= (c.topo_conc ? c.topo_conc : 1);
      b /= (c.topo_conc ? c.topo_conc : 1);
      [[fallthrough]];
    case TOPO_MESH:
    case TOPO_TORUS: {
      uint32_t h = 0;
      for (uint32_t d = 0; d < n; ++d) {
        const uint32_t x = a % k, y = b % k;
        uint32_t dd = x > y ? x - y : y - x;
        if (c.topo == TOPO_TORUS && k - dd < dd) dd = k - dd;
        h += dd;
        a /= k;
        b /= k;
      }
      return h + 1;
    }
    case TOPO_FATTREE: {
      uint32_t lvl = 1;
      a /= k;
      b /= k;
      while (a != b && lvl < n) {
        a /= k;
        b /= k;
        ++lvl;
      }
// ... 73 lines not shown
```

csrc/model/epoch.h:

```cpp
#pragma once
#include "icnt_router.h"
#include "mem.h"

namespace asim {

constexpr int kMaxChTot = 128;

struct UnitPub {
  uint64_t next;
  uint64_t prog;
  uint64_t insn;
  uint32_t req;
  uint16_t idle;
  uint8_t kbusy;
  uint8_t pad8;
  uint32_t drained;
  uint32_t ctas;
  uint64_t reqk;
  uint64_t dmask[2];
};
static_assert(sizeof(UnitPub) == 64, "UnitPub layout");
struct EpochPub {
  UnitPub sm[2][kMaxSmTot];
  UnitPub ch[2][kMaxChTot];
// ... 276 lines not shown
    nx = core_fs(c, sm_quiet_until<P>(s, c, kt, s.cycle, s.cycle + kSkipHorizon));
  nx = amin(nx, s.min_emit);
  UnitPub u;
  u.next = nx;
  u.prog = s.last_progress;
  u.insn = s.sget(SK(thread_insn));
  u.req = req;
  u.idle = (uint16_t)idle;
  u.kbusy = (uint8_t)kbusy;
  u.pad8 = 0;
  u.drained = sm_idle(s) ? 1u : 0u;
  u.ctas = (uint32_t)s.sget(SK(ctas_done));
  u.reqk = reqk;
  u.dmask[0] = dm0;
  u.dmask[1] = dm1;
  P::one([&] {
    pub.sm[cur][s.id] = u;
    if (s.id == 0)
      for (int k = 0; k < kMaxConc; ++k) {
        pub.next_cta[cur][k] = s.next_cta[k];
        for (int xi = 0; xi < kMaxXcd; ++xi) pub.next_ctax[cur][k][xi] = s.next_ctax[k][xi];
      }
  });
}

template <class P>
SIM_HDI void chan_epoch(ChanState& ch, const MemCtx& x, const Pkt* inbox, const uint32_t* incnt,
                        uint32_t in_cap, uint64_t t0_fs, const uint64_t* req_dst = nullptr) {
  P::prof(20);
  ch.min_emit = ~0ull;
  if (x.cfg->link_contention == 2 && x.rt_st) {
    const SimCfg& c = *x.cfg;
    ch.inj_t0_fs = t0_fs;
    for (uint32_t j = 0; j < c.n_sub_per_mem; ++j) {
      ch.sp[j].inj_allow0 = rt_inj_allow0(c, x.rt_st, 1, c.n_clusters + ch.id * c.n_sub_per_mem + j, fdiv(t0_fs, c.dv_icnt));
      ch.sp[j].inj_used = 0;
    }
  }
  mem_gather<P>(ch, *x.cfg, x, inbox, incnt, in_cap, t0_fs, req_dst);
  P::one([&] {
    for (uint32_t j = 0; j < x.cfg->n_sub_per_mem; ++j) ch.sp[j].st.icnt_backlog += ch.sp[j].ovf_n;
  });
  P::prof(24);
  mem_window<P>(ch, x);
  P::prof(25);
}

template <class P>
SIM_HDI void chan_publish(ChanState& ch, const MemCtx& x, EpochPub& pub, uint32_t cur) {
  uint64_t dm[2] = {0, 0};
  mem_publish<P>(ch, *x.cfg, x.outcnt, cur, dm);
  uint32_t idle = chan_idle(ch, *x.cfg) ? 1u : 0u;
  uint64_t nx = ~0ull;
  if (x.cfg->event_skip) nx = chan_next_event(ch, *x.cfg, amin(ch.t_dram, amin(ch.t_l2, ch.t_icnt)));
  nx = amin(nx, ch.min_emit);
  UnitPub u;
  u.next = nx;
  u.prog = 0;
  u.insn = 0;
  u.req = 0;
  u.idle = (uint16_t)idle;
  u.kbusy = 0;
  u.pad8 = 0;
  u.drained = idle;
  u.ctas = 0;
  u.reqk = 0;
  u.dmask[0] = dm[0];
  u.dmask[1] = dm[1];
  P::one([&] { pub.ch[cur][ch.id] = u; });
}

template <class P>
SIM_HDI EpochDecision epoch_decide(const SimCfg& c, const EpochPub& pub, uint32_t cur, uint64_t t1,
                                   const KernelTab& kt, uint64_t epoch_idx, uint64_t max_cycle) {
  EpochDecision d;
  uint32_t nbusy = 0, undrained = 0, cbusy = 0, ctas = 0, reqs = 0, kbusy = 0;
  uint64_t sm_next = ~0ull, ch_next = ~0ull, prog = 0, insn = 0;
  uint64_t rq0 = 0, rq1 = 0, rp0 = 0, rp1 = 0;
  P::lane_loop((int)c.n_sm, [&](int j) {
    const UnitPub u = pub.sm[cur][j];
    rq0 |= u.dmask[0];
    rq1 |= u.dmask[1];
    insn += u.insn;
    ctas += u.ctas;
    nbusy += u.idle ? 0u : 1u;
    undrained += u.drained ? 0u : 1u;
    reqs |= u.req;
    kbusy |= u.kbusy;
    sm_next = amin<uint64_t>(sm_next, u.next);
    prog = amax<uint64_t>(prog, u.prog & ((1ull << 56) - 1));
  });
  P::lane_loop((int)c.n_mem, [&](int j) {
    const UnitPub u = pub.ch[cur][j];
    rp0 |= u.dmask[0];
    rp1 |= u.dmask[1];
    cbusy += u.idle ? 0u : 1u;
    ch_next = amin<uint64_t>(ch_next, u.next);
  });
  nbusy = P::uni(P::red_sum(nbusy));
  undrained = P::uni(P::red_sum(undrained));
  reqs = P::uni(P::red_or(reqs));
  kbusy = P::uni(P::red_or(kbusy));
  cbusy = P::uni(P::red_sum(cbusy));
  sm_next = P::uni(P::red_min64(sm_next));
  ch_next = P::uni(P::red_min64(ch_next));
  prog = P::uni(P::red_max64(prog));
  auto or64 = [&](uint64_t v) -> uint64_t {
// ... 62 lines not shown
```

csrc/model/hd.h:

```cpp
#pragma once
#include <stdint.h>

#if defined(__HIP__)
#include <hip/hip_runtime.h>
#define SIM_HD __host__ __device__
#define SIM_HDI __host__ __device__ __forceinline__
#define SIM_HDN __host__ __device__ inline __attribute__((noinline))
#else
#define SIM_HDN inline
#define SIM_HD
#define SIM_HDI inline
#endif

namespace asim {

SIM_HDI int popc64(uint64_t x) { return __builtin_popcountll(x); }
SIM_HDI int ffs64(uint64_t x) { return x ? __builtin_ctzll(x) : -1; }
SIM_HDI uint64_t rotr64(uint64_t x, unsigned r, unsigned n) {
  if (r == 0) return x;
  uint64_t m = (n == 64) ? ~0ull : ((1ull << n) - 1);
  x &= m;
  return ((x >> r) | (x << (n - r))) & m;
}
template <class T>
SIM_HDI T amin(T a, T b) { return a < b ? a : b; }
template <class T>
SIM_HDI T amax(T a, T b) { return a > b ? a : b; }

struct SeqPar {
  static constexpr int kLanes = 64;
  template <class F>
  static SIM_HDI uint64_t ballot(int n, F&& f) {
    uint64_t m = 0;
    for (int i = 0; i < n; ++i)
      if (f(i)) m |= 1ull << i;
    return m;
  }
  template <class F>
  static SIM_HDI void lane_loop(int n, F&& f) {
    for (int i = 0; i < n; ++i) f(i);
  }
  static SIM_HDI uint32_t red_sum(uint32_t v) { return v; }
  static SIM_HDI uint32_t red_or(uint32_t v) { return v; }
  static SIM_HDI uint64_t red_sum64(uint64_t v) { return v; }
  static SIM_HDI uint64_t red_min64(uint64_t v) { return v; }
  static SIM_HDI uint64_t red_max64(uint64_t v) { return v; }
  template <class F>
  static SIM_HDI uint64_t ballot_m(uint64_t mask, F&& f) {
    uint64_t m = 0;
    for (uint64_t r = mask; r; r &= r - 1) {
      const int i = __builtin_ctzll(r);
      if (f(i)) m |= 1ull << i;
    }
    return m;
  }
  template <class F>
  static SIM_HDI void each_m(uint64_t mask, F&& f) {
    for (uint64_t r = mask; r; r &= r - 1) f(__builtin_ctzll(r));
  }
  template <class F>
  static SIM_HDI void each(int n, F&& f) {
    for (int i = 0; i < n; ++i) f(i);
  }
  template <class F>
  static SIM_HDI void one(F&& f) { f(); }
  template <class T>
  static SIM_HDI void fetch_copy(T* dst, const T* src, int n) {
    for (int i = 0; i < n; ++i) dst[i] = src[i];
  }
  static SIM_HDI void fetch_wait() {}
  static SIM_HDI void sync() {}
  static SIM_HDI void prof(int) {}
  static SIM_HDI void tick(int) {}
  template <class T>
  static SIM_HDI T uni(T v) { return v; }
  template <class S, class F>
  static SIM_HDI void view(S& s, F&& f) { f(s); }
  template <class F>
  static SIM_HDI int argmin(int n, F&& key) {
    uint64_t best = ~0ull;
    int bi = -1;
    for (int i = 0; i < n; ++i) {
      uint64_t k = key(i);
      if (k != ~0ull && (bi < 0 || k < best)) {
        best = k;
        bi = i;
      }
    }
    return bi;
  }
  template <class F>
  static SIM_HDI int find_first(int n, F&& pred) {
    for (int i = 0; i < n; ++i)
      if (pred(i)) return i;
    return -1;
  }
  template <class F>
  static SIM_HDI uint32_t sum(int n, F&& f) {
    uint32_t s = 0;
    for (int i = 0; i < n; ++i) s += f(i);
    return s;
  }
  template <class F>
  static SIM_HDI uint32_t vmax(int n, F&& f) {
    uint32_t s = 0;
    for (int i = 0; i < n; ++i) {
      uint32_t v = f(i);
      s = v > s ? v : s;
    }
    return s;
  }
  template <class T, class F>
  struct Lanes {
    F f;
    SIM_HDI T self(int i) const { return f(i); }
    SIM_HDI T at(int i) const { return f(i); }
  };
  template <class T, class F>
  static SIM_HDI Lanes<T, F> lanes(int, F f) {
    return Lanes<T, F>{f};
  }
  template <class F, class G>
  static SIM_HDI uint32_t scan(int n, F&& val, G&& out) {
    uint32_t acc = 0;
    for (int i = 0; i < n; ++i) {
      uint32_t v = val(i);
      out(i, acc);
      acc += v;
    }
    return acc;
  }
  template <class F>
  static SIM_HDI uint64_t vor(int n, F&& f) {
    uint64_t s = 0;
    for (int i = 0; i < n; ++i) s |= f(i);
    return s;
  }
  static SIM_HDI void min32(uint32_t* p, uint32_t v) {
    if (v < *p) *p = v;
  }
  static SIM_HDI void add64(uint64_t* p, uint64_t v) { *p += v; }
  template <class F>
  static SIM_HDI uint64_t order16(int n, uint32_t mask, F&& key) {
    uint64_t ord = 0;
    for (int i = 0; i < n; ++i) {
      if (!(mask >> i & 1u)) continue;
      const uint32_t ki = key(i);
      uint32_t r = 0;
      for (int j = 0; j < n; ++j)
        if ((mask >> j & 1u) && j != i) {
          const uint32_t kj = key(j);
          r += (kj < ki || (kj == ki && j < i)) ? 1u : 0u;
        }
      ord |= (uint64_t)i << (4 * r);
    }
    return ord;
  }
};

}
```

csrc/model/mem.h:

```cpp
#pragma once
#include "sm.h"

namespace asim {

struct L2Line {
  uint64_t tag;
  uint32_t lru;
  uint8_t valid;
  uint8_t dirty;
  uint8_t pad[2];
};

struct L2Mshr {
  uint64_t line;
  uint8_t requested;
  uint8_t valid;
  uint8_t merges;
  uint8_t pad[5];
};

struct L2Wait {
  uint64_t line;
  uint32_t tag;
  uint16_t src;
// ... 768 lines not shown
    if (!ch.q_valid[i]) return ~0ull;
    if (c.dram_sched == 0 && ch.q_age[i] != oldest_age) return ~0ull;
    const DramReq& r = ch.q[i];
    if (only != 2 && r.write != only) return ~0ull;
    const DramBank& b = ch.bk[r.bank];
    if (b.open) {
      if (b.row == r.row || t < b.t_pre_ok) return ~0ull;
      if (c.dram_sched != 0 && (hitmask >> r.bank & 1ull)) return ~0ull;
      return ch.q_age[i];
    }
    if (t < b.t_act_ok || t < ch.t_rrd_ok) return ~0ull;
    return ch.q_age[i];
  });
  if (act >= 0) {
    const DramReq& r = ch.q[act];
    DramBank& b = ch.bk[r.bank];
    if (trace_mem_on(c, TS_MEMORY_PARTITION_UNIT, ch.id))
      P::one([&] {
        trace_put(c, c.n_sm + ch.id, t, EV_DRAM_CMD, b.open ? 3 : 2,
                  (uint64_t)r.bank << 32 | (b.open ? b.row : r.row));
      });
    if (b.open) {
      b.open = 0;
      b.t_act_ok = amax<uint64_t>(b.t_act_ok, t + c.tRP);
      st.dram_pre++;
    } else {
      b.open = 1;
      b.row = r.row;
      b.t_col_ok = t + c.tRCD;
      b.t_pre_ok = t + c.tRAS;
      b.t_act_ok = t + c.tRC;
      ch.t_rrd_ok = t + c.tRRD;
      st.dram_act++;
    }
  }
}

SIM_HDI bool sub_idle(const SubPart& sp) {
  return sp.inq_n == 0 && sp.ovf_n == 0 && sp.rop_n == 0 && sp.rep_n == 0 && sp.fill_n == 0 && sp.n_wait == 0 && sp.n_l2dram == 0;
}
SIM_HDI bool chan_idle(const ChanState& ch, const SimCfg& c) {
  if (ch.lat_n || ch.q_n || ch.ret_n || ch.mret_n) return false;
  for (uint32_t j = 0; j < c.n_sub_per_mem; ++j)
    if (!sub_idle(ch.sp[j])) return false;
  return true;
}

SIM_HDI uint64_t next_tick(uint64_t t, uint64_t per, uint64_t t1) {
  if (t >= t1) return t;
  uint64_t k = (t1 - t + per - 1) / per;
  return t + k * per;
}

SIM_HDI uint64_t chan_next_event(const ChanState& ch, const SimCfg& c, uint64_t now) {
  if (ch.q_n) return now;
  uint64_t nx = ~0ull;
  if (ch.lat_n) nx = amin(nx, ch.lat[ch.lat_head].ready);
  if (ch.ret_n) nx = amin(nx, ch.ret[ch.ret_head].ready);
  if (ch.mret_n) nx = amin(nx, ch.mret[ch.mret_head].ready);
  for (uint32_t j = 0; j < c.n_sub_per_mem; ++j) {
    const SubPart& sp = ch.sp[j];
    if (sp.rep_n || sp.ovf_n) return now;
    if (sp.fill_n) nx = amin(nx, sp.fill[sp.fill_head].ready);
    if (sp.rop_n) nx = amin(nx, sp.rop[sp.rop_head].t);
    if (sp.inq_n && sp.rop_n < (uint32_t)kRopQ && sp.rop_n < c.q_icnt_l2 + c.rop_latency)
      nx = amin(nx, sp.inq[sp.inq_head].t);
  }
  return nx > now ? nx : now;
}

SIM_HDI void chan_quiet_advance(ChanState& ch, const SimCfg& c, uint64_t target) {
  const uint64_t nd = next_tick(ch.t_dram, c.per_dram, target);
  const uint64_t kd = fdiv(nd - ch.t_dram, c.dv_dram);
  ch.sp[0].st.dram_cycles += kd;
  ch.sp[0].st.dram_q_occ += (uint64_t)ch.q_n * kd;
  ch.dcycle += kd;
  ch.t_dram = nd;
  const uint64_t nl = next_tick(ch.t_l2, c.per_l2, target);
  const uint64_t kl = fdiv(nl - ch.t_l2, c.dv_l2);
  for (uint32_t j = 0; j < c.n_sub_per_mem; ++j) {
    ch.sp[j].st.l2_cycles += kl;
    ch.sp[j].st.rop_occ += (uint64_t)ch.sp[j].rop_n * kl;
  }
  ch.t_l2 = nl;
  ch.t_icnt = next_tick(ch.t_icnt, c.per_icnt, target);
}

template <class P>
SIM_HDI void mem_window(ChanState& ch, const MemCtx& x) {
  const SimCfg& c = *x.cfg;
  const uint64_t t1 = x.win_end;
  if (chan_idle(ch, c)) {
    uint64_t nd = next_tick(ch.t_dram, c.per_dram, t1);
    ch.sp[0].st.dram_cycles += fdiv(nd - ch.t_dram, c.dv_dram);
    ch.dcycle += fdiv(nd - ch.t_dram, c.dv_dram);
    ch.t_dram = nd;
    uint64_t nl = next_tick(ch.t_l2, c.per_l2, t1);
    for (uint32_t j = 0; j < c.n_sub_per_mem; ++j) ch.sp[j].st.l2_cycles += fdiv(nl - ch.t_l2, c.dv_l2);
    ch.t_l2 = nl;
    ch.t_icnt = next_tick(ch.t_icnt, c.per_icnt, t1);
    return;
  }
  for (;;) {
    uint64_t tm = amin(ch.t_dram, amin(ch.t_l2, ch.t_icnt));
    if (tm >= t1) break;
    if (c.event_skip) {
      const uint64_t nx = chan_next_event(ch, c, tm);
      if (nx > tm) {
        chan_quiet_advance(ch, c, amin(nx, t1));
        continue;
      }
    }
    if (ch.t_dram == tm) {
      P::prof(21);
      dram_cycle<P>(ch, c, x, tm);
      ch.t_dram += c.per_dram;
    }
    if (ch.t_l2 == tm) {
      P::prof(22);
      for (uint32_t j = 0; j < c.n_sub_per_mem; ++j) l2_cycle<P>(ch, ch.sp[j], c, j, tm);
      ch.t_l2 += c.per_l2;
    }
    if (ch.t_icnt == tm) {
      P::prof(23);
      for (uint32_t j = 0; j < c.n_sub_per_mem; ++j) mem_icnt_cycle<P>(ch, ch.sp[j], c, x, j, tm);
      ch.t_icnt += c.per_icnt;
    }
    P::prof(24);
  }
}

struct Backlog {
  Pkt* ring;
  uint32_t cap;
  uint32_t* head;
  uint32_t* n;
  uint64_t* drop;
};

template <class P>
SIM_HDI uint32_t gather_sorted(const Pkt* box, const uint32_t* cnt, uint32_t dst, uint32_t n_src,
                               uint32_t cap, uint64_t t0, Pkt* q, uint32_t qcap, uint32_t& qhead,
                               uint32_t& qn, uint64_t* skey, uint32_t* sref, uint32_t* srank,
                               uint32_t scap, const Backlog& bl = Backlog{nullptr, 0, nullptr, nullptr, nullptr}) {
  if (bl.ring && *bl.n) {
    const uint32_t m = amin<uint32_t>(*bl.n, qcap - qn);
    const uint32_t h = *bl.head;
    P::each((int)m, [&](int i) { q[(qhead + qn + (uint32_t)i) % qcap] = bl.ring[(h + (uint32_t)i) % bl.cap]; });
    P::sync();
    qn += m;
    *bl.head = (h + m) % bl.cap;
    *bl.n -= m;
  }
  const uint32_t* row = cnt + (uint64_t)dst * n_src;
  const uint32_t total = P::scan((int)n_src, [&](int s) -> uint32_t { return row[s]; },
                                 [&](int s, uint32_t off) { srank[s] = off; });
  P::sync();
  if (total == 0) return 0;
  const Pkt* cell0 = box + (uint64_t)dst * n_src * cap;
  const uint32_t room = (bl.ring && *bl.n) ? 0u : qcap - qn;
// ... 98 lines not shown
```

csrc/model/sm.h:

```cpp
#pragma once
#include <stddef.h>
#if !defined(__HIP_DEVICE_COMPILE__)
#include <stdexcept>
#include <stdio.h>
#endif

#include "addrdec.h"

namespace asim {



enum WarpFlags : uint8_t {
  WF_ACTIVE = 1,
  WF_EXITING = 2,
  WF_BARRIER = 4,
  WF_MEMBAR = 8,
  WF_WAITCNT = 16,
  WF_IMISS = 32,
};

struct HitEnt {
  uint8_t warp;
  uint8_t slot;
// ... 322 lines not shown
  const uint64_t k = now_fs > t0_fs ? fdiv(now_fs - t0_fs, c.dv_icnt) : 0;
  return (int64_t)(used + nfl) <= allow0 + (int64_t)(k < (1ull << 40) ? k : (1ull << 40));
}

template <class P, class S>
SIM_HDI void sm_inject(S& s, const SmCtx& x, uint64_t now) {
  const SimCfg& c = *x.cfg;
  if (P::uni(s.outq_n) == 0) return;
  if (now < P::uni(s.out_port_free)) return;
  Pkt p = P::uni(s.outq[P::uni(s.outq_head)]);
  uint32_t nflits = (p.size + c.flit_size - 1) / c.flit_size;
  uint64_t done = now + nflits - 1;
  uint32_t dst = p.dst;
  uint32_t slot = dst * x.n_src_sm + s.id;
  uint32_t n = P::uni(s.ocnt[dst]);
  if (n >= x.out_cap) return;
  const uint32_t cpc = c.cores_per_cluster ? c.cores_per_cluster : 1;
  if (c.link_contention == 2 &&
      !rt_inj_ok(c, P::uni(s.inj_t0_fs), P::uni(s.inj_allow0), P::uni(s.inj_used), nflits * cpc, core_fs(c, now))) {
    s.sadd(SK(icnt_inj_stall), 1);
    return;
  }
  if (c.link_contention == 2) s.inj_used = s.inj_used + (uint64_t)nflits * cpc;
  s.ocnt[dst] = n + 1;
  p.t = core_fs(c, done) + icnt_pkt_lat_fs(c, s.id, dst);
  s.min_emit = amin(s.min_emit, p.t);
  if (trace_sm_on(c, TS_INTERCONNECT, s.id)) P::one([&] { trace_put(c, s.id, now, EV_PKT_SEND, (uint16_t)dst, p.addr); });
  P::one([&] {
    x.outbox[(uint64_t)slot * x.out_cap + n] = p;
    x.outcnt[slot] = n + 1;
  });
  s.outq_head = (s.outq_head + 1) % kOutQ;
  s.outq_n--;
  s.out_port_free = now + nflits;
  s.outstanding++;
  s.sadd(SK(pkts_out), 1);
  s.sadd(SK(bytes_out), p.size);
}

template <class P, class S>
SIM_HDI void sm_writeback(S& s, const SimCfg& c, uint64_t now) {
  uint32_t slot = (uint32_t)(now % kWbRing);
  if (!((P::uni((uint64_t)s.wb_occ[slot >> 6]) >> (slot & 63)) & 1ull)) return;
  uint32_t n = P::uni(s.wb_cnt[slot]);
  for (uint32_t i = 0; i < n; ++i) {
    WbEnt e = P::uni(s.wb[slot][i]);
    if (trace_sm_on(c, TS_SCOREBOARD, s.id))
      P::one([&] {
        if (e.dst0) trace_put(c, s.id, now, EV_SB_RELEASE, e.warp, e.dst0 - 1u);
        if (e.dst1) trace_put(c, s.id, now, EV_SB_RELEASE, e.warp, e.dst1 - 1u);
      });
    sbc(s.w_sb, e.warp, e.dst0);
    sbc(s.w_sb, e.warp, e.dst1);
    s.w_inflight[e.warp]--;
    s.sadd(SK(rf_writes), (e.dst0 != 0) + (e.dst1 != 0));
  }
  if (n) s.last_progress = now;
  s.wb_cnt[slot] = 0;
  s.wb_occ[slot >> 6] &= ~(1ull << (slot & 63));
}

template <class S>
SIM_HDI void sm_load_slot_done(S& s, uint32_t w, uint32_t slot, uint64_t now) {
  sbc(s.w_sb, w, s.w_slot_dst[w][slot][0]);
  sbc(s.w_sb, w, s.w_slot_dst[w][slot][1]);
  s.sadd(SK(rf_writes), (s.w_slot_dst[w][slot][0] != 0) + (s.w_slot_dst[w][slot][1] != 0));
  s.w_slot_used[w] &= (uint8_t)~(1u << slot);
  s.w_slot_lds[w] &= (uint8_t)~(1u << slot);
  s.w_loads[w]--;
  s.w_inflight[w]--;
  s.last_progress = now;
}

template <class S>
SIM_HDI bool waitcnt_met(S& s, uint32_t w) {
  const uint32_t wt = s.w_wait[w];
  const uint32_t lds_ld = (uint32_t)__builtin_popcount((uint32_t)s.w_slot_lds[w]);
  const uint32_t vm = (uint32_t)s.w_loads[w] - lds_ld + (uint32_t)s.w_stores[w];
  const uint32_t lgkm = lds_ld + (uint32_t)s.w_lds_st[w];
  return vm <= (wt & 0xffu) && lgkm <= (wt >> 8);
}

template <class P, class S>
SIM_HDI void sm_hit_complete(S& s, uint64_t now) {
  uint32_t slot = (uint32_t)(now % kHitRing);
  if (!((P::uni((uint64_t)s.hit_occ[slot >> 6]) >> (slot & 63)) & 1ull)) return;
  uint32_t n = P::uni(s.hit_cnt[slot]);
  for (uint32_t i = 0; i < n; ++i) {
    HitEnt e = P::uni(s.hit[slot][i]);
    if (e.kind == 0) {
      if (--s.w_slot_pend[e.warp][e.slot] == 0) sm_load_slot_done(s, e.warp, e.slot, now);
    } else {
      s.w_inflight[e.warp]--;
      s.w_lds_st[e.warp]--;
      s.last_progress = now;
    }
  }
  s.hit_cnt[slot] = 0;
  s.hit_occ[slot >> 6] &= ~(1ull << (slot & 63));
}

template <class S>
SIM_HDI bool hit_push(S& s, uint64_t when, uint8_t warp, uint8_t slot, uint8_t kind) {
  uint32_t r = (uint32_t)(when % kHitRing);
  if (s.hit_cnt[r] >= kHitSlot) return false;
  s.hit_occ[r >> 6] |= 1ull << (r & 63);
  HitEnt& e = s.hit[r][s.hit_cnt[r]++];
  e.warp = warp;
  e.slot = slot;
  e.kind = kind;
  e.pad = 0;
  return true;
}

template <class S>
SIM_HDI void sm_miss_access_done(S& s, const SimCfg& c, uint32_t w, uint32_t sl, uint64_t now) {
  if (c.l1_miss_ret) {
    for (uint32_t d = 0; d < 16; ++d)
      if (hit_push(s, now + c.l1_miss_ret + d, (uint8_t)w, (uint8_t)sl, 0)) return;
  }
  if (--s.w_slot_pend[w][sl] == 0) sm_load_slot_done(s, w, sl, now);
}

template <class P, class S>
SIM_HDI int l1_find(const S& s, const CacheGeom& g, uint32_t set, uint64_t line) {
  const L1Line* base = &s.l1[set * g.assoc];
  const int assoc = (int)g.assoc;
  if (assoc <= 64) {
    uint64_t m = P::ballot(assoc, [&](int w) { return base[w].valid && base[w].tag == line; });
    return m ? ffs64(m) : -1;
  }
  for (int b = 0; b < assoc; b += 64) {
    int n = amin(64, assoc - b);
    uint64_t m = P::ballot(n, [&](int w) { return base[b + w].valid && base[b + w].tag == line; });
    if (m) return b + ffs64(m);
  }
  return -1;
}

template <class P, class S>
SIM_HDI int l1_victim(const S& s, const CacheGeom& g, uint32_t set) {
  const L1Line* base = &s.l1[set * g.assoc];
  int v = P::argmin((int)g.assoc, [&](int w) -> uint64_t {
    return base[w].valid ? (1ull << 40) | base[w].lru : (uint64_t)w;
  });
  return v;
}

template <class P, class S>
SIM_HDI void l1_evict(S& s, const SimCfg& c, uint32_t idx) {
  L1Line& V = s.l1[idx];
  const uint8_t d = P::uni(V.dirty);
  if (V.valid | d) {
    if (d) {
      if (s.outq_n < (uint32_t)kOutQ) {
        sm_send(s, c, P_WR, P::uni(V.tag), d, (uint16_t)(32 * popc64(d)), kTagL1Writeback);
        s.sadd(SK(l1_wb), 1);
      } else {
        s.sadd(SK(l1_wb_lost), 1);
      }
    }
  }
  V.valid = 0;
  V.dirty = 0;
}

template <class P, class S>
SIM_HDI void l1_fill(S& s, const SmCtx& x, uint64_t line, uint8_t sectors, uint64_t now) {
  const SimCfg& c = *x.cfg;
  const CacheGeom g = l1_geom(c, s);
  if (!g.disabled) {
    uint32_t set = cache_set_index(g, line);
    int w = l1_find<P>(s, g, set, line);
    if (w < 0) {
      w = l1_victim<P>(s, g, set);
      l1_evict<P>(s, c, set * g.assoc + w);
      L1Line& L = s.l1[set * g.assoc + w];
      L.tag = line;
      L.valid = 0;
      L.dirty = 0;
      L.lru = ++s.l1_stamp;
    }
    L1Line& L = s.l1[set * g.assoc + w];
    L.valid |= sectors;
    if (g.repl == REPL_LRU) L.lru = ++s.l1_stamp;
  }
  int mi = P::find_first((int)c.l1.mshr_entries, [&](int i) -> bool { return s.mshr[i].valid && s.mshr[i].line == line; });
  if (mi >= 0) {
    s.mshr[mi].requested &= (uint8_t)~sectors;
    if (s.mshr[mi].requested == 0) {
      s.mshr[mi].valid = 0;
      const uint32_t lat = (uint32_t)now - s.mshr[mi].t_issue;
      s.sadd(SK(mf_lat_sum), lat);
      s.sadd(SK(mf_lat_n), 1);
      if (lat > s.sget(SK(mf_lat_max))) s.sset(SK(mf_lat_max), lat);
      SADD_IN(s, mf_lat_hist, 16, lat ? amin<int>(15, 31 - __builtin_clz(lat)) : 0, 1);
    }
  }
  P::prof(47);
  const uint32_t np = s.n_pend;
  for (uint32_t b = 0; b < np; b += 64) {
    int n = (int)amin<uint32_t>(64, np - b);
    uint64_t m = P::ballot(n, [&](int i) {
      const L1Pend& e = s.pend[b + i];
      return e.valid && e.line == line && (e.need & sectors) != 0;
    });
    while (m) {
      int i = ffs64(m);
      m &= m - 1;
      L1Pend& e = s.pend[b + i];
      e.need &= (uint8_t)~sectors;
      if (e.need) continue;
      e.valid = 0;
      sm_miss_access_done(s, c, e.warp, e.slot, now);
    }
  }
  while (s.n_pend && !s.pend[s.n_pend - 1].valid) s.n_pend--;
  P::prof(41);
}

template <class P, class S>
SIM_HDI int il1_find(const S& s, const CacheGeom& g, uint32_t set, uint64_t line) {
  const L1Line* base = &s.il1[set * g.assoc];
  uint64_t m = P::ballot((int)amin<uint32_t>(g.assoc, 64), [&](int w) { return base[w].valid && base[w].tag == line; });
  return m ? ffs64(m) : -1;
}

template <class P, class S>
SIM_HDI void il1_fill(S& s, const SimCfg& c, uint64_t line) {
  const CacheGeom& g = c.il1;
  const uint32_t set = cache_set_index(g, line);
  if (il1_find<P>(s, g, set, line) < 0) {
    L1Line* base = &s.il1[set * g.assoc];
    const int v = P::argmin((int)amin<uint32_t>(g.assoc, 64), [&](int w) -> uint64_t {
      return base[w].valid ? (1ull << 40) | base[w].lru : (uint64_t)w;
    });
    base[v].tag = line;
    base[v].valid = 0xf;
    base[v].lru = ++s.l1_stamp;
  }
  const int mi = P::find_first((int)g.mshr_entries, [&](int i) -> bool { return s.imshr[i].valid && s.imshr[i].line == line; });
  if (mi >= 0) s.imshr[mi].valid = 0;
  const int nw = (int)amin<uint32_t>(c.max_warps_per_sm, kMaxWarps);
  P::each(nw, [&](int w) {
    if ((s.w_flags[w] & WF_IMISS) && s.w_iline[w] == line) s.w_flags[w] &= (uint8_t)~WF_IMISS;
  });
  P::sync();
}

template <class P, class S>
SIM_HDI void il1_prefetch(S& s, const SimCfg& c, uint64_t line) {
  const CacheGeom& g = c.il1;
  for (uint32_t k = 1; k <= c.inst_prefetch; ++k) {
    const uint64_t l = line + 128ull * k;
    if (il1_find<P>(s, g, cache_set_index(g, l), l) >= 0) continue;
    if (P::find_first((int)g.mshr_entries, [&](int i) -> bool { return s.imshr[i].valid && s.imshr[i].line == l; }) >= 0)
      continue;
    const int mi = P::find_first((int)g.mshr_entries, [&](int i) -> bool { return !s.imshr[i].valid; });
    if (mi < 0 || !sm_can_send(s, c)) return;
    s.imshr[mi].valid = 1;
    s.imshr[mi].line = l;
    s.imshr[mi].merges = 0;
    s.imshr[mi].t_issue = 0;
    sm_send(s, c, P_RD, l, 0xf, 128, 0x40000000u | (uint32_t)mi);
    s.sadd(SK(il1_prefetch), 1);
  }
}
// ... 84 lines not shown
    const Pkt& h = s.rsp_cl[ch];
    const bool ifill = (P::uni(h.tag) & 0xc0000000u) == 0x40000000u && P::uni(h.type) != P_WR_ACK;
    if (ifill) {
      il1_fill<P>(s, c, P::uni(h.addr));
      s.cl_head = (ch + 1) % kEjectQ;
      s.cl_n = P::uni(s.cl_n) - 1;
    } else if (P::uni(s.ld_n) < c.ldst_resp_buf) {
      const uint32_t li = (P::uni(s.ld_head) + P::uni(s.ld_n)) % kLdstRespQ;
      const Pkt v = P::uni(h);
      P::one([&] { s.rsp_ld[li] = v; });
      s.ld_n = P::uni(s.ld_n) + 1;
      s.cl_head = (ch + 1) % kEjectQ;
      s.cl_n = P::uni(s.cl_n) - 1;
    }
  }
  if (P::uni(s.inq_n) && P::uni(s.cl_n) < c.eject_buf &&
      P::uni(s.inq[P::uni(s.inq_head)].t) <= core_fs(c, now)) {
    Pkt q;
    uint32_t head = P::uni(s.inq_head), n = P::uni(s.inq_n);
    uint16_t an = s.arb_next, ac = s.arb_cnt;
    P::prof(40);
    const XbarGrant g = xbar_pick<P>(s.inq, head, n, kInQ, core_fs(c, now), c, fdiv(core_fs(c, now), c.dv_icnt),
                                     an, ac, c.n_subpart);
    P::prof(0);
    s.arb_next = an;
    s.arb_cnt = ac;
    s.sadd(SK(icnt_reply_conflicts), g.ready - 1);
    q = P::uni(xbar_take(s.inq, head, n, kInQ, g.off));
    s.sadd(SK(icnt_reply_queue_cycles), fdiv(core_fs(c, now) - q.t, c.dv_icnt));
    s.inq_head = head;
    s.inq_n = n;
    if (trace_sm_on(c, TS_INTERCONNECT, s.id)) P::one([&] { trace_put(c, s.id, now, EV_PKT_RECV, q.type, q.addr); });
    s.outstanding--;
    s.sadd(SK(pkts_in), 1);
    s.sadd(SK(bytes_in), q.size);
    const uint32_t ci = (P::uni(s.cl_head) + P::uni(s.cl_n)) % kEjectQ;
    P::one([&] { s.rsp_cl[ci] = q; });
    s.cl_n = P::uni(s.cl_n) + 1;
  }
  if (!P::uni(s.ld_n)) return;
  if (P::uni(s.outq_n) >= (uint32_t)kOutQ) return;
  const uint32_t lh = P::uni(s.ld_head);
  const Pkt q = P::uni(s.rsp_ld[lh]);
  s.ld_head = (lh + 1) % kLdstRespQ;
  s.ld_n = P::uni(s.ld_n) - 1;
  if (q.type == P_WR_ACK) {
    if (!(q.tag & kTagL1Writeback)) {
      uint32_t w = q.tag & 0xff;
      s.w_stores[w]--;
    }
    s.last_progress = now;
  } else if (q.tag & 0x80000000u) {
    uint32_t w = q.tag & 0xff, sl = (q.tag >> 8) & 0xff;
    sm_miss_access_done(s, c, w, sl, now);
  } else {
    P::prof(41);
    l1_fill<P>(s, x, q.addr, q.sectors, now);
    P::prof(0);
  }
}

SIM_HDI uint32_t l1_stat_type(uint8_t space, bool write, bool atomic) {
  if (atomic) return L1T_ATOMIC;
  if (space == S_LOCAL) return write ? L1T_LOCAL_W : L1T_LOCAL_R;
  return write ? L1T_GLOBAL_W : L1T_GLOBAL_R;
}

template <class P, class S>
SIM_HDI void sm_ldst(S& s, const SmCtx& x, uint64_t now) {
  const SimCfg& c = *x.cfg;
  LdstState& u = s.ldst;
  if (!P::uni(u.busy)) return;
  const TInst in = P::uni(u.inst);
  const uint32_t w = P::uni(u.warp);
  if (in.space == S_SHARED) {
    const uint32_t cdeg = in.width ? in.width : 1;
    const uint32_t deg = (c.lds_port_bytes && in.ii > cdeg) ? (uint32_t)in.ii : cdeg;
    if ((uint32_t)(now - P::uni(u.start)) + 1 < deg) return;
    uint8_t kind = (in.cls == OC_STORE) ? 1 : 0;
    if (!hit_push(s, now + c.smem_latency, (uint8_t)w, P::uni(u.slot), kind)) return;
    s.sadd(SK(shmem_acc), 1);
    s.sadd(SK(shmem_conflict_cycles), cdeg - 1);
    u.busy = 0;
    return;
  }
  const bool is_store = in.cls == OC_STORE;
  const bool atomic = (in.flags & F_ATOMIC) != 0;
  const CacheGeom g = l1_geom(c, s);
  const bool bypass = atomic || (in.flags & F_BYPASS_L1) || (c.gmem_skip_l1 && in.space != S_CONST) || g.disabled;
  const uint32_t nacc = in.width;
  const uint32_t stype = l1_stat_type(in.space, is_store, atomic);
  uint32_t banks_used = 0;
  uint32_t processed = 0;
  uint32_t unext = P::uni(u.next);
  const uint8_t uslot = P::uni(u.slot);
  P::fetch_wait();
  const bool port = c.l1_port_bytes && in.space != S_CONST;
  while (unext < nacc && processed < c.l1_banks) {
    const TAcc a = P::uni(s.ldst_acc[unext]);
    uint32_t bbit = 1u << (a.bank & 31);
    if (banks_used & bbit) break;
    if (port && (int32_t)(P::uni(u.port_free) - (uint32_t)now) > 0) break;
    if (c.perfect_mem) {
      if (!is_store) {
        if (!hit_push(s, now + c.l1_latency, (uint8_t)w, uslot, 0)) { SADD_IN(s, l1, L1T_COUNT * L1O_COUNT, (stype) * L1O_COUNT + L1O_RES_FAIL, 1); break; }
      }
      SADD_IN(s, l1, L1T_COUNT * L1O_COUNT, (stype) * L1O_COUNT + L1O_HIT, 1);
// ... 331 lines not shown
  if (x < n) return x;
  x -= n;
  return x < n ? x : x % n;
}
SIM_HDI uint32_t sched_of(uint32_t w, uint32_t nsched) {
  return (nsched & (nsched - 1)) == 0 ? (w & (nsched - 1)) : w % nsched;
}

template <class S>
SIM_HDI bool warp_sb_ok(const S& s, int w, const TInst& in) {
  for (int j = 0; j < 5; ++j)
    if (sbt(s.w_sb, w, in.src[j])) return false;
  return !sbt(s.w_sb, w, in.dst[0]) && !sbt(s.w_sb, w, in.dst[1]);
}
template <class S>
SIM_HDI bool warp_can_issue_nosb(const S& s, const SimCfg& c, int w, const TInst& in, uint32_t nsched,
                                 uint64_t idoc_busy) {
  uint8_t f = s.w_flags[w];
  if (!(f & WF_ACTIVE) || (f & (WF_EXITING | WF_BARRIER | WF_MEMBAR | WF_WAITCNT))) return false;
  if (s.w_ibuf[w] == 0) return false;
  uint32_t u = unit_of(c, in.cls);
  uint32_t sc = sched_of((uint32_t)w, nsched);
  if (in.cls == OC_EXIT || in.cls == OC_BARRIER || in.cls == OC_MEMBAR || in.cls == OC_NOP || (in.flags & F_WAITCNT))
    return true;
  if (idoc_busy >> (sc * U_COUNT + u) & 1ull) return false;
  if (u == U_MEM && in.cls == OC_LOAD && s.w_slot_used[w] == 0xff) return false;
  return true;
}
template <class S>
SIM_HDI bool warp_can_issue_i(const S& s, const SimCfg& c, int w, const TInst& in, uint32_t nsched,
                              uint64_t idoc_busy) {
  return warp_can_issue_nosb(s, c, w, in, nsched, idoc_busy) && warp_sb_ok(s, w, in);
}
template <class S>
SIM_HDI bool warp_can_issue(const S& s, const SimCfg& c, const KernelTab& kt, int w, uint32_t nsched,
                            uint64_t idoc_busy) {
  if (!(s.w_flags[w] & WF_ACTIVE) || s.w_ibuf[w] == 0) return false;
  const TInst in = s.w_win[w][s.w_head[w] & (kWin - 1)];
  return warp_can_issue_i(s, c, w, in, nsched, idoc_busy);
}

template <class S>
SIM_HDI bool warp_issue_due(const S& s, const SimCfg& c, int w, uint64_t now) {
  return c.warp_issue_interval <= 1 || now >= s.w_issue_ok[w];
}

template <class P, class S>
SIM_HDI int sm_issue_one(S& s, const SmCtx& x, uint64_t now, uint32_t sc, uint32_t w, const TInst& in,
                         uint32_t hidx) {
  const SimCfg& c = *x.cfg;
  if (trace_sm_on(c, TS_WARP_SCHEDULER, s.id))
    P::one([&] { trace_put(c, s.id, now, EV_ISSUE, (uint16_t)w, (uint64_t)in.pc | (uint64_t)in.opcode << 32); });
  s.w_head[w] = hidx + 1;
  s.w_ibuf[w] = (uint8_t)(P::uni((uint8_t)s.w_ibuf[w]) - 1);
  s.sadd(SK(warp_insn), 1);
  s.sadd(SK(thread_insn), (uint64_t)popc64(in.mask));
  SADD_IN(s, cls_insn, OC_COUNT, in.cls < OC_COUNT ? in.cls : OC_ALU, 1);
  SADD_IN(s, sq_insn, 8, sq_class(in), 1);
  if (in.space == S_CONST) s.sadd(SK(power_acc) + PWR_CONST_OPERAND, 1);
  {
    const uint32_t pk = (uint32_t)(in.flags >> 4);
    if (pk) SADD_IN(s, power_acc, 16, pk, pk == PWR_SALU ? 1ull : (uint64_t)popc64(in.mask));
  }
  s.last_progress = now;
  const uint32_t cta = P::uni((uint8_t)s.w_cta[w]);
  if (in.cls == OC_EXIT) {
    if (hidx + 1 >= P::uni((uint32_t)s.w_end[w])) {
      s.w_flags[w] |= WF_EXITING;
      s.cta_nexit[cta]++;
      sm_barrier_check<P>(s, cta);
    }
    return -1;
  }
  if (in.cls == OC_BARRIER) {
    s.w_flags[w] |= WF_BARRIER;
    s.cta_bar[cta]++;
    sm_barrier_check<P>(s, cta);
    return -1;
  }
  if (in.cls == OC_MEMBAR) {
    if (s.w_stores[w]) {
      s.w_flags[w] |= WF_MEMBAR;
      s.n_wait_flags++;
    }
    return -1;
  }
  if (in.flags & F_WAITCNT) {
    s.w_wait[w] = in.lat;
    if (!waitcnt_met(s, w)) {
      s.w_flags[w] |= WF_WAITCNT;
      s.n_wait_flags++;
    }
    return -1;
  }
  if (in.cls == OC_NOP) return -1;
  const uint32_t u = unit_of(c, in.cls);
  const uint32_t kk = sc * U_COUNT + u;
  TInst ri = in;
  uint32_t lslot = 0xff;
  s.w_inflight[w]++;
  if (in.cls == OC_LOAD) {
    uint8_t used = P::uni((uint8_t)s.w_slot_used[w]);
    uint32_t sl = (uint32_t)ffs64((uint64_t)(uint8_t)~used);
    s.w_slot_used[w] = (uint8_t)(used | (1u << sl));
    s.w_loads[w]++;
    uint32_t nacc = (in.space == S_SHARED) ? 1u : (uint32_t)in.width;
    if (nacc == 0) nacc = 1;
    s.w_slot_pend[w][sl] = (uint16_t)nacc;
    s.w_slot_dst[w][sl][0] = in.dst[0];
    s.w_slot_dst[w][sl][1] = in.dst[1];
    lslot = sl;
    if (in.space != S_SHARED && in.width == 0) {
      s.w_slot_pend[w][sl] = 1;
      ri.space = S_SHARED;
      ri.width = 1;
    }
    if (ri.space == S_SHARED || ri.space == S_CONST) s.w_slot_lds[w] = (uint8_t)(s.w_slot_lds[w] | (1u << sl));
  } else if (in.cls == OC_STORE && in.space != S_SHARED && in.width == 0) {
    ri.space = S_SHARED;
    ri.width = 1;
  }
  if (in.cls == OC_STORE && ri.space == S_SHARED) s.w_lds_st[w]++;
  s.idoc_inst[kk] = ri;
  s.idoc_meta[kk] = idoc_pack(w, lslot, ++s.age_ctr);
  s.idoc_mask |= 1ull << kk;
  sbs(s.w_sb, w, in.dst[0]);
  sbs(s.w_sb, w, in.dst[1]);
  return (int)u;
}

template <class S>
SIM_HDI bool waits_long_op(const S& s, int w, const TInst& in) {
  const uint8_t used = s.w_slot_used[w];
  for (int sl = 0; sl < kLoadSlots; ++sl) {
    if (!(used >> sl & 1u)) continue;
    for (int d = 0; d < 2; ++d) {
      const uint8_t r = s.w_slot_dst[w][sl][d];
      if (!r) continue;
      for (int j = 0; j < 5; ++j)
        if (in.src[j] == r) return true;
    }
  }
  return false;
}

template <class P, class S>
SIM_HDI void sm_stall_masks(const S& s, const SimCfg& c, uint64_t now, uint64_t live, uint64_t& valid_m,
                            uint64_t& sbok_m) {
  valid_m = P::ballot_m(live, [&](int w) -> bool {
    const uint8_t f = s.w_flags[w];
    return (f & WF_ACTIVE) && !(f & (WF_EXITING | WF_BARRIER | WF_MEMBAR | WF_WAITCNT)) && s.w_ibuf[w] != 0 &&
           warp_issue_due(s, c, w, now);
  });
  sbok_m = P::ballot_m(valid_m, [&](int w) -> bool {
    const TInst& in = s.w_win[w][s.w_head[w] & (kWin - 1)];
    for (int j = 0; j < 5; ++j)
      if (sbt(s.w_sb, w, in.src[j])) return false;
    return !sbt(s.w_sb, w, in.dst[0]) && !sbt(s.w_sb, w, in.dst[1]);
  });
}
SIM_HDI uint32_t stall_class(uint64_t mine, uint64_t valid_m, uint64_t sbok_m) {
  return !(valid_m & mine) ? 0u : !(sbok_m & mine) ? 1u : 2u;
}

template <class P, class S>
SIM_HDI int sched_pick(const S& s, const SimCfg& c, uint64_t now, int nw, uint64_t cand, uint32_t last) {
  switch (c.sched_policy) {
    case SCHED_GTO:
      if (last < (uint32_t)nw && (cand >> last & 1ull)) return (int)last;
      [[fallthrough]];
    case SCHED_OLDEST:
      return P::argmin(nw, [&](int w) -> uint64_t {
        return (cand >> w & 1ull) ? ((uint64_t)s.w_age[w] << 8 | (uint64_t)w) : ~0ull;
      });
    case SCHED_RRR: {
      uint32_t start = (uint32_t)(now % (uint64_t)nw);
      uint64_t r = rotr64(cand, start, (unsigned)nw);
      return (int)mod_small((uint32_t)ffs64(r) + start, (uint32_t)nw);
    }
    default: {
      uint32_t start = mod_small(last + 1, (uint32_t)nw);
      uint64_t r = rotr64(cand, start, (unsigned)nw);
      return (int)mod_small((uint32_t)ffs64(r) + start, (uint32_t)nw);
    }
  }
}

SIM_HDI bool issue_special(const TInst& in) {
  return in.cls == OC_EXIT || in.cls == OC_BARRIER || in.cls == OC_MEMBAR || in.cls == OC_NOP || (in.flags & F_WAITCNT);
}

template <class P, class S, class H>
SIM_HDI void sm_issue_par(S& s, const SmCtx& x, uint64_t now, const H& head, uint64_t ready, uint64_t live,
                          uint64_t sbok_all) {
  const SimCfg& c = *x.cfg;
  const int nw = (int)amin<uint32_t>(c.max_warps_per_sm, kMaxWarps);
  const uint32_t nsched = c.n_sched ? c.n_sched : 1;
  uint32_t n_idle = 0, idle_sc = 0, first_idle = nsched;
  uint64_t picks = 0;
  uint32_t pk_of = 0xffffffffu;
  P::prof(48);
  for (uint32_t sc = 0; sc < nsched; ++sc) {
    const uint64_t mine = c.sched_mask[sc];
    const uint64_t cand = ready & mine;
    if (!cand) {
      if (live & mine) {
        ++n_idle;
        idle_sc |= 1u << sc;
        if (first_idle == nsched) first_idle = sc;
      }
      continue;
    }
// ... 48 lines not shown
    s.sadd(SK(warp_insn), 1);
    s.sadd(SK(thread_insn), (uint64_t)popc64(in.mask));
    SADD_IN(s, cls_insn, OC_COUNT, in.cls < OC_COUNT ? in.cls : OC_ALU, 1);
    SADD_IN(s, sq_insn, 8, sq_class(in), 1);
    if (in.space == S_CONST) s.sadd(SK(power_acc) + PWR_CONST_OPERAND, 1);
    {
      const uint32_t pk = (uint32_t)(in.flags >> 4);
      if (pk) SADD_IN(s, power_acc, 16, pk, pk == PWR_SALU ? 1ull : (uint64_t)popc64(in.mask));
    }
    const uint32_t u = unit_of(c, in.cls);
    const uint32_t kk = sc * U_COUNT + u;
    TInst ri = in;
    uint32_t lslot = 0xff;
    if (in.cls == OC_LOAD) {
      lslot = (uint32_t)ffs64((uint64_t)(uint8_t)~P::uni((uint8_t)s.w_slot_used[w]));
      if (in.space != S_SHARED && in.width == 0) {
        ri.space = S_SHARED;
        ri.width = 1;
      }
    } else if (in.cls == OC_STORE && in.space != S_SHARED && in.width == 0) {
      ri.space = S_SHARED;
      ri.width = 1;
    }
    s.idoc_inst[kk] = ri;
    s.idoc_meta[kk] = idoc_pack(w, lslot, ++age);
    idoc |= 1ull << kk;
  }
  s.age_ctr = age;
  s.idoc_mask = idoc;
  P::prof(51);
  P::each_m(picks & ~spec, [&](int w) {
    const TInst in = head.self(w);
    s.w_head[w] = s.w_head[w] + 1u;
    s.w_ibuf[w] = (uint8_t)(s.w_ibuf[w] - 1u);
    s.w_inflight[w] = (uint8_t)(s.w_inflight[w] + 1u);
    const bool nomem = in.space != S_SHARED && in.width == 0;
    if (in.cls == OC_LOAD) {
      const uint8_t used = s.w_slot_used[w];
      const uint32_t sl = (uint32_t)ffs64((uint64_t)(uint8_t)~used);
      s.w_slot_used[w] = (uint8_t)(used | (1u << sl));
      s.w_loads[w] = (uint16_t)(s.w_loads[w] + 1u);
      uint32_t nacc = (in.space == S_SHARED) ? 1u : (uint32_t)in.width;
      if (nacc == 0) nacc = 1;
      s.w_slot_pend[w][sl] = (uint16_t)nacc;
      s.w_slot_dst[w][sl][0] = in.dst[0];
      s.w_slot_dst[w][sl][1] = in.dst[1];
      if (nomem || in.space == S_SHARED || in.space == S_CONST) s.w_slot_lds[w] = (uint8_t)(s.w_slot_lds[w] | (1u << sl));
    } else if (in.cls == OC_STORE && (nomem || in.space == S_SHARED)) {
      s.w_lds_st[w] = (uint8_t)(s.w_lds_st[w] + 1u);
    }
    sbs(s.w_sb, (uint32_t)w, in.dst[0]);
    sbs(s.w_sb, (uint32_t)w, in.dst[1]);
  });
  P::sync();
  P::prof(52);
  if (spec) {
    for (uint32_t sc = 0; sc < nsched; ++sc) {
      const uint32_t w = (pk_of >> (8 * sc)) & 0xffu;
      if (w == 0xffu || !(spec >> w & 1ull)) continue;
      if (!classified && sc > first_idle) classify();
      sm_issue_one<P>(s, x, now, sc, w, head.at((int)w), P::uni((uint32_t)s.w_head[w]));
    }
  }
  if (!classified) classify();
}

template <class P, class S>
SIM_HDI void sm_issue(S& s, const SmCtx& x, uint64_t now) {
  const SimCfg& c = *x.cfg;
  const KernelTab& kt = *x.kt;
  const int nw = (int)amin<uint32_t>(c.max_warps_per_sm, kMaxWarps);
  const uint32_t nsched = c.n_sched ? c.n_sched : 1;
  const uint64_t idoc_busy = P::uni(s.idoc_mask);
  P::fetch_wait();
  const auto head = P::template lanes<TInst>(nw, [&](int w) -> TInst { return s.w_win[w][s.w_head[w] & (kWin - 1)]; });
  const uint64_t live = P::uni(s.live_mask);
  if ((c.sched_policy == SCHED_LRR || c.sched_policy == SCHED_GTO || c.sched_policy == SCHED_OLDEST ||
       c.sched_policy == SCHED_RRR) &&
      c.max_issue_per_warp <= 1 && !trace_sm_on(c, TS_WARP_SCHEDULER, s.id)) {
    const uint64_t sbok = P::ballot_m(live, [&](int w) -> bool { return warp_sb_ok(s, w, head.self(w)); });
    const uint64_t ready = P::ballot_m(live & sbok, [&](int w) -> bool {
      return warp_can_issue_nosb(s, c, w, head.self(w), nsched, idoc_busy) && warp_issue_due(s, c, w, now);
    });
    P::prof(29);
    sm_issue_par<P>(s, x, now, head, ready, live, sbok);
    return;
  }
  uint64_t ready = P::ballot_m(live, [&](int w) -> bool {
    return warp_can_issue_i(s, c, w, head.self(w), nsched, idoc_busy) && warp_issue_due(s, c, w, now);
  });
  uint64_t waiting = 0;
  if (c.sched_policy == SCHED_WARP_LIMITING || c.sched_policy == SCHED_TWO_LEVEL)
    waiting = P::ballot_m(live, [&](int w) -> bool {
      const uint8_t f = s.w_flags[w];
      if (f & (WF_EXITING | WF_BARRIER | WF_MEMBAR | WF_WAITCNT)) return true;
      return c.sched_policy == SCHED_TWO_LEVEL && s.w_ibuf[w] && waits_long_op(s, w, head.self(w));
    });
  P::prof(29);
  bool issued_any = false;
  uint64_t valid_m = 0, sbok_m = 0;
  bool classified = false;
  auto classify = [&]() {
    if (classified) return;
    classified = true;
    sm_stall_masks<P>(s, c, now, live, valid_m, sbok_m);
  };
  for (uint32_t sc = 0; sc < nsched; ++sc) {
    const uint64_t mine = c.sched_mask[sc];
    uint64_t cand = ready & mine;
    const uint32_t last = P::uni((uint32_t)s.sched_last[sc]);
    if (c.sched_policy == SCHED_WARP_LIMITING && cand) {
      uint64_t pool = live & mine & ~waiting, lim = 0;
      for (uint32_t i = 0; i < c.sched_param && pool; ++i) {
        const int o = P::argmin(nw, [&](int w) -> uint64_t {
          return (pool >> w & 1ull) ? ((uint64_t)s.w_age[w] << 8 | (uint64_t)w) : ~0ull;
        });
        if (o < 0) break;
        lim |= 1ull << o;
        pool &= ~(1ull << o);
      }
      if (last < (uint32_t)nw) lim |= 1ull << last;
      cand &= lim;
    } else if (c.sched_policy == SCHED_TWO_LEVEL && cand) {
      uint64_t pool = live & mine & ~waiting, act = 0;
      for (uint32_t i = 0; i < c.sched_param && pool; ++i) {
        const uint64_t b = pool & (~pool + 1);
        act |= b;
        pool &= ~b;
      }
      cand &= act;
    }
    if (!cand) {
      if (live & mine) {
// ... 36 lines not shown
    const TInst in1 = head.at((int)w);
    P::prof(42);
    const int u1 = sm_issue_one<P>(s, x, now, sc, w, in1, hidx);
    P::prof(29);
    issued_any = true;
    SADD_IN(s, issue_distro, 3 + kMaxWarpLanes, 2u + (uint32_t)amin<int>(popc64(in1.mask), kMaxWarpLanes), 1);
    bool dual = false;
    if (c.max_issue_per_warp > 1 && u1 >= 0 && P::uni((uint8_t)s.w_ibuf[w])) {
      const TInst in2 = P::uni(s.w_win[w][(hidx + 1) & (kWin - 1)]);
      const bool special = in2.cls == OC_EXIT || in2.cls == OC_BARRIER || in2.cls == OC_MEMBAR ||
                           in2.cls == OC_NOP || (in2.flags & F_WAITCNT);
      if (!special && (!c.dual_issue_diff || unit_of(c, in2.cls) != (uint32_t)u1) &&
          warp_can_issue_i(s, c, (int)w, in2, nsched, P::uni(s.idoc_mask))) {
        sm_issue_one<P>(s, x, now, sc, w, in2, hidx + 1);
        s.sadd(SK(dual_issued), 1);
        SADD_IN(s, issue_distro, 3 + kMaxWarpLanes, 2u + (uint32_t)amin<int>(popc64(in2.mask), kMaxWarpLanes), 1);
        dual = true;
      }
    }
    if (dual) SADD_IN(s, dual_issue, kMaxSched, sc, 1);
    else SADD_IN(s, single_issue, kMaxSched, sc, 1);
  }
  if (issued_any) s.sadd(SK(busy_cycles), 1);
}

template <class P, class S>
SIM_HDI void sm_fetch(S& s, const SimCfg& c, const KernelTab& kt) {
  const int nw = (int)amin<uint32_t>(c.max_warps_per_sm, kMaxWarps);
  P::fetch_wait();
  uint64_t need = P::ballot_m(P::uni(s.live_mask), [&](int w) {
    uint8_t f = s.w_flags[w];
    return (f & WF_ACTIVE) && !(f & (WF_EXITING | WF_IMISS)) && s.w_ibuf[w] == 0 && s.w_next[w] < s.w_end[w];
  });
  uint32_t start = mod_small(P::uni(s.fetch_rr), (uint32_t)nw);
  uint64_t r = rotr64(need, start, (unsigned)nw);
  const bool icache = !c.perfect_icache && !c.il1.disabled;
  for (uint32_t i = 0; i < c.fetch_throughput && r; ++i) {
    int b = ffs64(r);
    r &= r - 1;
    uint32_t w = mod_small((uint32_t)b + start, (uint32_t)nw);
    if (icache && !il1_fetch<P>(s, c, kt, w)) {
      s.fetch_rr = w + 1;
      break;
    }
    const uint32_t wnext = P::uni((uint32_t)s.w_next[w]);
    const uint32_t wend = P::uni((uint32_t)s.w_end[w]);
    uint32_t avail = wend - wnext;
    uint32_t n = avail < (uint32_t)kIbuf ? avail : (uint32_t)kIbuf;
    for (uint32_t j = 1; j <= n && wnext + j < wend; ++j)
      P::fetch_copy(&s.w_win[w][(wnext + j) & (kWin - 1)], &inst_at(kt, wnext + j), 1);
    s.w_next[w] = wnext + n;
    s.w_ibuf[w] = (uint8_t)n;
    s.fetch_rr = w + 1;
  }
}

#if !defined(__HIP_DEVICE_COMPILE__)
[[noreturn]] inline void throw_cta_fit_error(uint32_t sm, uint32_t cta) {
  char b[128];
  snprintf(b, sizeof(b), "SM %u: no contiguous warp run for CTA %u (dispatch plan out of date)", sm, cta);
  throw std::logic_error(b);
}
#endif

SIM_HDI int warp_run_fit(uint64_t used, uint32_t n, uint32_t nw) {
  if (n == 0 || n > nw) return -1;
  const uint64_t need = n >= 64 ? ~0ull : ((1ull << n) - 1);
  for (uint32_t b = 0; b + n <= nw; ++b)
    if (!((used >> b) & need)) return (int)b;
  return -1;
}

template <class S>
SIM_HDI void sm_cta_release(S& s, const KernelTab& kt, uint32_t cta) {
  const uint32_t ks = s.cta_ks[cta];
  const KernelDesc& k = kt.k[ks];
  const uint32_t nw = s.cta_nw[cta];
  s.cta_wmask = s.cta_wmask & ~((nw >= 64 ? ~0ull : ((1ull << nw) - 1)) << s.cta_wbase[cta]);
  s.n_cta_k[ks] = (uint8_t)(s.n_cta_k[ks] - 1);
  s.used_thr = s.used_thr - k.thr_cta;
  s.used_regs = s.used_regs - k.regs_cta;
  s.used_shmem = s.used_shmem - k.shmem_per_cta;
}

template <class P, class S>
SIM_HDI void sm_retire(S& s, const SmCtx& x, uint64_t now) {
  const SimCfg& c = *x.cfg;
  const int nw = (int)amin<uint32_t>(c.max_warps_per_sm, kMaxWarps);
  const uint64_t live = P::uni(s.live_mask);
  uint64_t done = P::ballot_m(live, [&](int w) {
    uint8_t f = s.w_flags[w];
    if (!(f & WF_ACTIVE)) return false;
    bool drained = s.w_head[w] >= s.w_end[w] && s.w_ibuf[w] == 0;
    return drained && s.w_inflight[w] == 0 && s.w_stores[w] == 0 && s.w_loads[w] == 0;
  });
  if (P::uni(s.n_wait_flags)) {
    uint32_t released = 0;
    const uint64_t rel = P::ballot_m(live, [&](int w) {
      uint8_t f = s.w_flags[w];
      uint32_t r = 0;
      if ((f & WF_MEMBAR) && s.w_stores[w] == 0) { f = f & (uint8_t)~WF_MEMBAR; ++r; }
      if ((f & WF_WAITCNT) && waitcnt_met(s, w)) { f = f & (uint8_t)~WF_WAITCNT; ++r; }
      if (r) s.w_flags[w] = f;
      return r != 0;
    });
    released = (uint32_t)popc64(rel);
// ... 8 lines not shown
    s.w_flags[w] = 0;
    s.live_mask &= ~(1ull << w);
    s.n_warps_live--;
    s.sadd(SK(warps_done), 1);
    s.cta_live[cta]--;
    s.cta_nexit[cta]--;
    if (s.cta_live[cta] == 0) {
      s.cta_valid[cta] = 0;
      s.n_cta_active--;
      sm_cta_release(s, *x.kt, cta);
      s.sadd(SK(ctas_done), 1);
    } else {
      sm_barrier_check<P>(s, cta);
    }
    s.last_progress = now;
  }
}

template <class P, class S>
SIM_HDI void sm_launch_cta(S& s, const SmCtx& x, uint32_t slot, uint32_t cta_id, uint32_t ks) {
  const KernelDesc& k = x.kt->k[ks];
  const SimCfg& c = *x.cfg;
  const uint32_t wpc = k.warps_per_cta;
  const uint32_t nwm = amin<uint32_t>(c.max_warps_per_sm, kMaxWarps);
  const int fit = warp_run_fit(s.cta_wmask, wpc, nwm);
  if (fit < 0) {
#if !defined(__HIP_DEVICE_COMPILE__)
    throw_cta_fit_error(s.id, cta_id);
#endif
    return;
  }
  const uint32_t base = (uint32_t)fit;
  const uint64_t wm = (wpc >= 64 ? ~0ull : ((1ull << wpc) - 1)) << base;
  if (s.n_cta_active == 0) {
    s.l1_sets = (uint16_t)k.l1_sets;
    s.l1_assoc = (uint16_t)k.l1_assoc;
  }
  s.cta_valid[slot] = 1;
  s.cta_id[slot] = cta_id;
  s.cta_live[slot] = (uint8_t)wpc;
  s.cta_bar[slot] = 0;
  s.cta_nexit[slot] = 0;
  s.cta_ks[slot] = (uint8_t)ks;
  s.cta_wbase[slot] = (uint8_t)base;
  s.cta_nw[slot] = (uint8_t)wpc;
  s.cta_wmask |= wm;
  s.n_cta_k[ks]++;
  s.used_thr += k.thr_cta;
  s.used_regs += k.regs_cta;
  s.used_shmem += k.shmem_per_cta;
  s.n_cta_active++;
  s.n_warps_live += wpc;
  s.live_mask |= wm;
  uint32_t age0 = s.age_ctr;
  s.age_ctr += wpc;
  const uint32_t tag = ks << kSlotShift;
  P::each((int)wpc, [&](int i) {
    uint32_t w = base + (uint32_t)i;
    WStream ws = k.streams[(uint64_t)(cta_id & k.cmask) * wpc + (uint32_t)i];
    s.w_next[w] = tag | ws.begin;
    s.w_head[w] = tag | ws.begin;
    s.w_end[w] = tag | (ws.begin + ws.count);
    if (ws.count) s.w_win[w][ws.begin & (kWin - 1)] = k.insts[ws.begin & k.imask];
    s.w_issue_ok[w] = 0;
    s.w_age[w] = age0 + (uint32_t)i;
    s.w_flags[w] = WF_ACTIVE;
    s.w_iline[w] = 0;
    s.w_ibuf[w] = 0;
    s.w_cta[w] = (uint8_t)slot;
    s.w_inflight[w] = 0;
    s.w_stores[w] = 0;
    s.w_loads[w] = 0;
    s.w_slot_used[w] = 0;
    s.w_slot_lds[w] = 0;
    s.w_lds_st[w] = 0;
    s.w_wait[w] = 0;
    sbz(s.w_sb, w);
  });
  P::sync();
}

template <class P, class S>
SIM_HDI void sm_cycle(S& s, const SmCtx& x, uint64_t now) {
  const SimCfg& c = *x.cfg;
  P::prof(0);
  sm_receive<P>(s, x, now);
  P::prof(1);
  sm_writeback<P>(s, c, now);
  P::prof(2);
  sm_hit_complete<P>(s, now);
  P::prof(3);
  sm_ldst<P>(s, x, now);
  P::prof(4);
  sm_dispatch<P>(s, x, now);
  P::prof(5);
  sm_read_operands<P>(s, c);
  P::prof(6);
  sm_alloc_collectors<P>(s, c);
  P::prof(7);
  sm_issue<P>(s, x, now);
  P::prof(8);
  sm_fetch<P>(s, c, *x.kt);
  P::prof(9);
  sm_retire<P>(s, x, now);
  P::prof(10);
  sm_inject<P>(s, x, now);
  P::prof(11);
  if (P::uni(s.n_cta_active)) {
    s.sadd(SK(active_cycles), 1);
    s.sadd(SK(occupancy_acc), P::uni(s.n_warps_live));
  }
}

template <class S>
SIM_HDI bool sm_idle(const S& s) {
  return s.n_cta_active == 0 && s.outq_n == 0 && s.outstanding == 0 && !s.ldst.busy && s.cl_n == 0 && s.ld_n == 0;
}

template <class P, class A>
SIM_HDI uint64_t ring_next(const A& occ, uint32_t ring, uint64_t from, uint64_t limit) {
  const uint32_t nwords = ring / 64;
  const uint32_t start = (uint32_t)(from % ring);
  const uint32_t w0 = start >> 6, b0 = start & 63;
  auto dist = [&](int i) -> uint64_t {
    const uint64_t m = occ[i];
    if (!m) return ~0ull;
    const uint64_t mh = (uint32_t)i == w0 ? (m & (~0ull << b0)) : m;
    const uint32_t p = (uint32_t)i * 64u + (uint32_t)ffs64(mh ? mh : m);
    return (uint64_t)((p + ring - start) & (ring - 1));
  };
  const int j = P::argmin((int)nwords, dist);
  if (j < 0) return limit;
  return amin<uint64_t>(limit, from + P::uni(dist(j)));
}

template <class P, class S>
SIM_HDI uint64_t sm_quiet_until(const S& s, const SimCfg& c, const KernelTab& kt, uint64_t t, uint64_t limit) {
  if (P::uni(s.ldst.busy) || P::uni(s.idoc_mask) || P::uni(s.oc_mask | s.oc_read_mask) || P::uni(s.outq_n) ||
      P::uni(s.cl_n | s.ld_n))
    return t;
  uint64_t nx = ring_next<P>(s.wb_occ, kWbRing, t, limit);
  if (nx == t) return t;
  nx = ring_next<P>(s.hit_occ, kHitRing, t, nx);
  if (nx == t) return t;
  if (P::uni(s.inq_n)) {
    const uint64_t at = core_cyc_ceil(c, P::uni(s.inq[P::uni(s.inq_head)].t));
    if (at <= t) return t;
    nx = amin<uint64_t>(nx, at);
  }
  const int nw = (int)amin<uint32_t>(c.max_warps_per_sm, kMaxWarps);
  const uint32_t nsched = c.n_sched ? c.n_sched : 1;
  const uint64_t act = P::ballot_m(P::uni(s.live_mask), [&](int w) -> bool {
    const uint8_t f = s.w_flags[w];
    if (!(f & WF_ACTIVE)) return false;
    if (!(f & (WF_EXITING | WF_IMISS)) && s.w_ibuf[w] == 0 && s.w_next[w] < s.w_end[w]) return true;
    const bool drained = s.w_head[w] >= s.w_end[w] && s.w_ibuf[w] == 0;
    if (drained && s.w_inflight[w] == 0 && s.w_stores[w] == 0 && s.w_loads[w] == 0) return true;
    if ((f & WF_MEMBAR) && s.w_stores[w] == 0) return true;
    if ((f & WF_WAITCNT) && waitcnt_met(s, w)) return true;
    return warp_can_issue(s, c, kt, w, nsched, s.idoc_mask) && warp_issue_due(s, c, w, t);
  });
  if (act) return t;
  if (c.warp_issue_interval > 1) {
    const int o = P::argmin(nw, [&](int w) -> uint64_t {
      if (!(P::uni(s.live_mask) >> w & 1ull)) return ~0ull;
      return warp_can_issue(s, c, kt, w, nsched, s.idoc_mask) && !warp_issue_due(s, c, w, t) ? s.w_issue_ok[w]
                                                                                                : ~0ull;
    });
    if (o >= 0) nx = amin<uint64_t>(nx, P::uni((uint64_t)s.w_issue_ok[o]));
  }
  return nx;
}

template <class P, class S>
SIM_HDI void sm_skip(S& s, const SimCfg& c, uint64_t k, uint64_t t) {
  const int nw = (int)amin<uint32_t>(c.max_warps_per_sm, kMaxWarps);
  const uint32_t nsched = c.n_sched ? c.n_sched : 1;
  const uint64_t live = P::uni(s.live_mask);
  uint32_t stalled = 0;
  uint64_t valid_m = 0, sbok_m = 0;
  if (live) sm_stall_masks<P>(s, c, t, live, valid_m, sbok_m);
  for (uint32_t sc = 0; sc < nsched; ++sc) {
    if (live & c.sched_mask[sc]) {
      ++stalled;
      SADD_IN(s, issue_distro, 3 + kMaxWarpLanes, stall_class(c.sched_mask[sc], valid_m, sbok_m), k);
    }
  }
  s.sadd(SK(issue_stall_idle), (uint64_t)stalled * k);
  if (P::uni(s.n_cta_active)) {
    s.sadd(SK(active_cycles), k);
    s.sadd(SK(occupancy_acc), (uint64_t)popc64(live) * k);
  }
  s.skipped_cycles += k;
  P::sync();
}

}
```

Before: 296,200.

## Cache per-warp scoreboard verdicts and fast-forward idle DRAM ticks in CPU engine

Adds a per-SM scoreboard-verdict cache on the CPU engine so only warps whose scoreboard or head instruction changed are re-tested each cycle, with dirty marks at writeback, issue, fetch and CTA launch. Extends event skipping so channels with queued DRAM requests can fast-forward to the next tick where bank and bus timing permits a command. It also swaps zero-filled vectors for calloc buffers and adds an optional host profiler and a debugger snapshot round-trip. The cached verdicts must be invalidated at every state change, so a missed dirty mark would alter simulated results.

```diff
diff --git a/csrc/bindings/py_asim.cc b/csrc/bindings/py_asim.cc
--- a/csrc/bindings/py_asim.cc
+++ b/csrc/bindings/py_asim.cc
@@ -213,6 +213,26 @@
       {offsetof(ChanState, skey), sizeof(ChanState::skey)}, {offsetof(ChanState, sref), sizeof(ChanState::sref)},
       {offsetof(ChanState, srank), sizeof(ChanState::srank)}, {offsetof(ChanState, pub_nz), sizeof(ChanState::pub_nz)}};
   m.attr("sizeof_TInst") = sizeof(TInst);
+  m.attr("offsetof_ChanState_subpart") = offsetof(ChanState, sp);
+  m.attr("sizeof_SubPart") = sizeof(SubPart);
+  m.attr("offsetof_SubPart_stats") = offsetof(SubPart, st);
+  {
+    std::vector<std::tuple<std::string, size_t, size_t>> f;
+#define ASIM_MS_FIELD(n) f.emplace_back(#n, offsetof(MemStats, n), sizeof(MemStats::n) / 8)
+    ASIM_MS_FIELD(l2); ASIM_MS_FIELD(dram_rd); ASIM_MS_FIELD(dram_wr); ASIM_MS_FIELD(dram_act); ASIM_MS_FIELD(dram_pre);
+    ASIM_MS_FIELD(dram_busy_cycles); ASIM_MS_FIELD(dram_cycles); ASIM_MS_FIELD(dram_q_occ); ASIM_MS_FIELD(l2_cycles);
+    ASIM_MS_FIELD(l2_busy); ASIM_MS_FIELD(rop_occ); ASIM_MS_FIELD(pkts_in); ASIM_MS_FIELD(pkts_out);
+    ASIM_MS_FIELD(bytes_in); ASIM_MS_FIELD(bytes_out); ASIM_MS_FIELD(l2_evict_dirty); ASIM_MS_FIELD(icnt_stall);
+    ASIM_MS_FIELD(icnt_backlog); ASIM_MS_FIELD(icnt_ovf_drop); ASIM_MS_FIELD(icnt_conflicts);
+    ASIM_MS_FIELD(icnt_queue_cycles); ASIM_MS_FIELD(icnt_arb_cycles); ASIM_MS_FIELD(l2_mem_rd); ASIM_MS_FIELD(l2_mem_wr);
+    ASIM_MS_FIELD(l2_mem_rd_req); ASIM_MS_FIELD(l2_mem_wr_req); ASIM_MS_FIELD(mall_rd_hit); ASIM_MS_FIELD(mall_rd_miss);
+    ASIM_MS_FIELD(mall_wr); ASIM_MS_FIELD(mall_wb); ASIM_MS_FIELD(icnt_inj_stall);
+#undef ASIM_MS_FIELD
+    size_t words = 0;
+    for (auto& e : f) words += std::get<2>(e);
+    if (words * 8 != sizeof(MemStats)) throw std::logic_error("MemStats_fields: a field is missing from the list");
+    m.attr("MemStats_fields") = f;
+  }
 
   m.def("gpu_available", &gpu_engine_available, "True if a HIP device is usable by the GPU engine");
   {
diff --git a/csrc/config/sim_options.cc b/csrc/config/sim_options.cc
--- a/csrc/config/sim_options.cc
+++ b/csrc/config/sim_options.cc
@@ -346,6 +346,13 @@
      "(the release / acquire of a multi-XCD GPU, whose XCD L2s are not coherent with each other)"},
     {"-sim_cpu_threads", 'u', "1", "CPU engine: OpenMP threads over the units of one epoch (1 = serial; "
                                   "run simulations job-parallel instead)"},
+    {"-sim_issue_cache", 'b', "1",
+     "CPU engine: keep each SM's per-warp scoreboard verdicts across cycles and re-test only the warps whose "
+     "scoreboard or next instruction changed (0 = test every live warp every cycle; results identical; the GPU "
+     "engine ignores it)"},
+    {"-sim_dram_skip", 'b', "1",
+     "with -sim_event_skip: fast-forward the DRAM ticks on which bank and bus timing lets no queued request "
+     "issue a command (results identical)"},
     {"-sim_router_pass", 's', "serial",
      "-icnt_link_contention 2: serial | par, the epoch pass over the routers: one lane (rt_simulate) or the "
      "lane-parallel pass (rt_simulate_par; on the GPU engine 64 lanes and one block per subnet); same results"},
@@ -950,6 +957,8 @@
     c.mall_miss_fs = (uint64_t)r.getu("-sim_mall_miss_latency");
   }
   c.cpu_threads = r.getu("-sim_cpu_threads");
+  c.issue_cache = r.getb("-sim_issue_cache") ? 1u : 0u;
+  c.dram_skip = r.getb("-sim_dram_skip") ? 1u : 0u;
   {
     const std::string rp = strip_ws(r.gets("-sim_router_pass"));
     if (rp != "serial" && rp != "par") throw OptionError("-sim_router_pass must be serial or par, not '" + rp + "'");
diff --git a/csrc/driver/debugger.cc b/csrc/driver/debugger.cc
--- a/csrc/driver/debugger.cc
+++ b/csrc/driver/debugger.cc
@@ -37,6 +37,7 @@
       "  dp [sm]            dump the pipeline of an SM (default: every busy SM)\n"
       "  dm [ch]            dump a memory channel (default: every busy channel)\n"
       "  i                  run status (cycle, instructions)\n"
+      "  ck                 take the engine's state image and restore the engine from it\n"
       "  q                  stop the simulation here\n"
       "  h                  this help\n");
 }
@@ -177,6 +178,9 @@
       h_.print(h_.dump(-2, ch));
     } else if (cmd == "i" || cmd == "info") {
       h_.print(h_.status() + "\n");
+    } else if (cmd == "ck") {
+      snprintf(b, sizeof(b), "engine state restored from its image (%zu bytes)\n", h_.roundtrip ? h_.roundtrip() : (size_t)0);
+      h_.print(b);
     } else if (cmd == "q" || cmd == "quit") {
       quit_ = true;
       h_.print("asim debugger: simulation stopped by the user\n");
diff --git a/csrc/driver/debugger.h b/csrc/driver/debugger.h
--- a/csrc/driver/debugger.h
+++ b/csrc/driver/debugger.h
@@ -17,6 +17,7 @@
     std::function<void(const std::string&)> print;
     std::function<std::string(int sm, int ch)> dump;
     std::function<std::string()> status;
+    std::function<size_t()> roundtrip;
   };
   Debugger(const std::string& script, uint64_t stop_at, Hooks hooks);
 
diff --git a/csrc/driver/simulator.cc b/csrc/driver/simulator.cc
--- a/csrc/driver/simulator.cc
+++ b/csrc/driver/simulator.cc
@@ -122,6 +122,12 @@
       snprintf(b, sizeof(b), "cycle %llu, kernels completed %zu, thread instructions of completed kernels %llu",
                (unsigned long long)eng_->now(), results_.size(), (unsigned long long)tot_insn_);
       return std::string(b);
+    };
+    h.roundtrip = [this]() {
+      std::vector<uint8_t> img;
+      eng_->snapshot(img);
+      eng_->restore(img);
+      return img.size();
     };
     dbg_.reset(new Debugger(dopt_.debug_script, dopt_.break_cycle, h));
   }
diff --git a/csrc/engine/cpu_engine.cc b/csrc/engine/cpu_engine.cc
--- a/csrc/engine/cpu_engine.cc
+++ b/csrc/engine/cpu_engine.cc
@@ -1,6 +1,9 @@
+#include <cstdio>
 #include <cstdlib>
 #include <cstring>
+#include <new>
 #include <stdexcept>
+#include <type_traits>
 
 #include <functional>
 
@@ -10,6 +13,7 @@
 
 #include "../model/icnt_router_par.h"
 #include "engine.h"
+#include "seq_par_host.h"
 #include "thread_team.h"
 #include "trace_window.h"
 
@@ -136,9 +140,38 @@
 
 namespace {
 
+template <class T>
+class ZeroBuf {
+  static_assert(std::is_trivially_copyable<T>::value, "ZeroBuf: plain records only");
+
+ public:
+  ZeroBuf() = default;
+  ZeroBuf(const ZeroBuf&) = delete;
+  ZeroBuf& operator=(const ZeroBuf&) = delete;
+  ~ZeroBuf() { std::free(p_); }
+  void assign_zero(size_t n) {
+    std::free(p_);
+    p_ = nullptr;
+    n_ = 0;
+    if (!n) return;
+    p_ = static_cast<T*>(std::calloc(n, sizeof(T)));
+    if (!p_) throw std::bad_alloc();
+    n_ = n;
+  }
+  T* data() { return p_; }
+  const T* data() const { return p_; }
+  size_t size() const { return n_; }
+  bool empty() const { return n_ == 0; }
+
+ private:
+  T* p_ = nullptr;
+  size_t n_ = 0;
+};
+
 class CpuEngine : public Engine {
  public:
   const char* name() const override { return "cpu"; }
+  ~CpuEngine() override { dump_profile(); }
 
   void init(const SimCfg& c) override {
     c_ = c;
@@ -151,14 +184,20 @@
     cap_req_ = c.icnt_latency;
     cap_rep_ = reply_cap(c);
     for (int p = 0; p < 2; ++p) {
-      box_req_[p].assign((size_t)c.n_subpart * c.n_sm * cap_req_, Pkt{});
+      box_req_[p].assign_zero((size_t)c.n_subpart * c.n_sm * cap_req_);
       cnt_req_[p].assign((size_t)c.n_subpart * c.n_sm, 0);
-      box_rep_[p].assign((size_t)c.n_sm * c.n_subpart * cap_rep_, Pkt{});
+      box_rep_[p].assign_zero((size_t)c.n_sm * c.n_subpart * cap_rep_);
       cnt_rep_[p].assign((size_t)c.n_sm * c.n_subpart, 0);
     }
     ovf_cap_ = backlog_cap(c);
-    ovf_.assign((size_t)c.n_subpart * ovf_cap_, Pkt{});
-    mall_.assign((size_t)(c.n_mem * mall_lines(c)), L2Line{});
+    ovf_.assign_zero((size_t)c.n_subpart * ovf_cap_);
+    mall_.assign_zero((size_t)(c.n_mem * mall_lines(c)));
+    sbc_.assign(c.n_sm, SbCache());
+    {
+      const char* pe = getenv("ASIM_CPU_PROFILE");
+      profiling_ = pe && *pe && *pe != '0';
+      prof_.clear();
+    }
     link_free_.clear();
     link_refs_.clear();
     n_link_state_ = 0;
@@ -201,6 +240,7 @@
     d = kd;
     tw_.launch(slot, k, d, c_);
     kt_.active |= 1u << slot;
+    sb_reset();
   }
   uint32_t running() const override { return kt_.active; }
 
@@ -222,7 +262,16 @@
       if (!err) err = std::current_exception();
       abort.store(true, std::memory_order_release);
     };
-    std::function<void(uint32_t)> job = [&](uint32_t tid) {
+    sb_reset();
+    if (profiling_ && prof_.size() < nthr) prof_.resize(nthr);
+    auto body = [&](auto policy, uint32_t tid) {
+      using P = decltype(policy);
+      if (profiling_) {
+        HostProf& pf = prof_[tid];
+        SeqParTls::pf = &pf;
+        pf.slot = 28;
+        pf.last = host_ticks();
+      }
       const SimCfg& c = c_;
       const uint64_t E = c.icnt_latency;
       const int nsm = (int)sms_.size(), nch = (int)chs_.size();
@@ -254,21 +303,24 @@
           if (i < nsm) {
             SMState& s = sms_[i];
             SmCtx x = ctx_sm(cur);
-            sm_epoch<SeqPar>(s, x, *pub_, prev, t0, t1, box_rep_[prev].data(), cnt_rep_[prev].data(), cap_rep_,
-                             c.n_subpart, epoch, repm);
-            sm_publish<SeqPar>(s, x, *pub_, cur);
+            SeqParTls::sb = &sbc_[i];
+            sm_epoch<P>(s, x, *pub_, prev, t0, t1, box_rep_[prev].data(), cnt_rep_[prev].data(), cap_rep_,
+                        c.n_subpart, epoch, repm);
+            sm_publish<P>(s, x, *pub_, cur);
           } else {
             ChanState& ch = chs_[i - nsm];
             MemCtx m = ctx_mem(cur, t1);
             m.mall = mall_.empty() ? nullptr : mall_.data() + (size_t)(i - nsm) * mall_lines(c);
-            chan_epoch<SeqPar>(ch, m, box_req_[prev].data(), cnt_req_[prev].data(), cap_req_, core_fs(c, t0), reqm);
-            chan_publish<SeqPar>(ch, m, *pub_, cur);
+            chan_epoch<P>(ch, m, box_req_[prev].data(), cnt_req_[prev].data(), cap_req_, core_fs(c, t0), reqm);
+            chan_publish<P>(ch, m, *pub_, cur);
           }
         }
         } catch (...) {
           fail();
         }
+        P::prof(26);
         if (nthr > 1) bar_.wait();
+        P::prof(28);
         if (abort.load(std::memory_order_acquire)) break;
         if (cap_sink_ && tid == 0) {
           try {
@@ -297,7 +349,9 @@
           if (abort.load(std::memory_order_acquire)) break;
         }
         const uint64_t mc = pw_on_ ? (lim.max_cycle ? std::min(lim.max_cycle, pw_next) : pw_next) : lim.max_cycle;
-        const EpochDecision d = epoch_decide<SeqPar>(c, *pub_, cur, t1, kt_, epoch, mc);
+        P::prof(27);
+        const EpochDecision d = epoch_decide<P>(c, *pub_, cur, t1, kt_, epoch, mc);
+        P::prof(28);
         refill = d.refill != 0;
         reqm[0] = d.req_dst[0];
         reqm[1] = d.req_dst[1];
@@ -337,6 +391,7 @@
         }
         break;
       }
+      P::prof(28);
       if (tid == 0) {
         r.epochs = epochs;
         res = r;
@@ -344,6 +399,12 @@
         end_cycle = cycle;
       }
     };
+    const bool ic = c_.issue_cache != 0;
+    std::function<void(uint32_t)> job;
+    if (profiling_ && ic) job = [&](uint32_t tid) { body(SeqParHost<true, true>{}, tid); };
+    else if (profiling_) job = [&](uint32_t tid) { body(SeqParHost<false, true>{}, tid); };
+    else if (ic) job = [&](uint32_t tid) { body(SeqParHost<true, false>{}, tid); };
+    else job = [&](uint32_t tid) { body(SeqPar{}, tid); };
     team_.run(nthr, job);
     if (err) std::rethrow_exception(err);
     if (cap_sink_) capture_flush();
@@ -465,6 +526,7 @@
     if (!mall_.empty()) memcpy(mall_.data(), p, mall_.size() * sizeof(L2Line));
     p += mall_.size() * sizeof(L2Line);
     if (n_link_state_) memcpy(link_free_.data(), p, n_link_state_ * 8);
+    sb_reset();
   }
   void link_stats(uint64_t* delayed, uint64_t* wait_cycles, uint64_t* deadlocked) override {
     *delayed = n_link_state_ ? link_free_[n_link_state_] : 0;
@@ -493,6 +555,22 @@
       if (cap_log_[d].n) cap_sink_->put(d, cap_log_[d].rec, cap_log_[d].n);
       cap_log_[d].n = 0;
     }
+  }
+  void dump_profile() const {
+    if (!profiling_ || prof_.empty()) return;
+    double acc[kHostProfSlots] = {}, tot = 0;
+    for (const HostProf& p : prof_)
+      for (int k = 0; k < kHostProfSlots; ++k) {
+        acc[k] += (double)p.acc[k];
+        if (!prof_slot_is_counter(k)) tot += (double)p.acc[k];
+      }
+    fprintf(stderr, "[asim cpu profile] %zu thread(s), issue cache %s, dram skip %s: SM cycles simulated %.0f, quiet checks "
+                    "%.0f, busy SM-epochs %.0f\n",
+            prof_.size(), c_.issue_cache ? "on" : "off", c_.dram_skip && c_.event_skip ? "on" : "off", acc[17], acc[18],
+            acc[19]);
+    for (int k = 0; k < kHostProfSlots; ++k)
+      if (acc[k] > 0 && !prof_slot_is_counter(k))
+        fprintf(stderr, "  %2d %-18s %16.0f (%5.1f%%)\n", k, prof_slot_name(k), acc[k], tot > 0 ? 100 * acc[k] / tot : 0.0);
   }
   bool router_par() const { return c_.link_contention == 2 && c_.router_pass == 1 && !link_free_.empty(); }
   RouterPassStats router_pass_stats() override {
@@ -568,6 +646,7 @@
     if (!link_free_.empty()) r.get(link_free_.data(), link_free_.size() * 8);
     cycle_ = h.cycle;
     epoch_ = h.epoch;
+    sb_reset();
     if (h.ready) throw std::runtime_error("engine state: image taken with kernels running");
   }
 
@@ -602,11 +681,17 @@
   std::vector<SMState> sms_;
   std::vector<ChanState> chs_;
   std::unique_ptr<EpochPub> pub_;
-  std::vector<Pkt> box_req_[2], box_rep_[2];
+  ZeroBuf<Pkt> box_req_[2], box_rep_[2];
   std::vector<uint32_t> cnt_req_[2], cnt_rep_[2];
   uint32_t cap_req_ = 0, cap_rep_ = 0;
-  std::vector<Pkt> ovf_;
-  std::vector<L2Line> mall_;
+  ZeroBuf<Pkt> ovf_;
+  ZeroBuf<L2Line> mall_;
+  std::vector<SbCache> sbc_;
+  void sb_reset() {
+    for (auto& k : sbc_) k = SbCache();
+  }
+  bool profiling_ = false;
+  std::vector<HostProf> prof_;
   uint32_t ovf_cap_ = 0;
   std::vector<uint64_t> link_free_;
   std::vector<uint32_t> link_refs_;
diff --git a/csrc/engine/engine.h b/csrc/engine/engine.h
--- a/csrc/engine/engine.h
+++ b/csrc/engine/engine.h
@@ -42,6 +42,21 @@
   uint32_t max_packets_req = 0, max_packets_rep = 0;
   uint32_t split_blocks = 0;
 };
+constexpr int kProfSlotNames = 56;
+inline const char* prof_slot_name(int k) {
+  static const char* const names[kProfSlotNames] = {
+      "sm.receive", "sm.writeback", "sm.hit_complete", "sm.ldst", "sm.dispatch", "sm.read_operands",
+      "sm.alloc_oc", "sm.issue", "sm.fetch", "sm.retire", "sm.inject", "sm.occupancy", "sm.gather",
+      "sm.cta_dispatch", "sm.refill", "sm.cycle_loop", "sm.publish", "#sm_cycles", "#quiet_checks", "#epochs_busy", "mem.gather", "mem.dram",
+      "mem.l2", "mem.icnt", "mem.window_other", "mem.publish", "barrier", "decide", "post", "sm.issue_sched", "#slowest", "launch_rest",
+      "#max_work/epoch", "#epochs(b0)", "#last_arriver_wait", "#last_arrivals", "ldst.l1_probe", "ldst.mshr_find",
+      "ldst.pend_reg", "ldst.send", "recv.xbar", "recv.l1_fill", "issue.one", "issue.pick", "quiet_check", "skip",
+      "ldst.hit_push", "fill.pend_wake", "iss.pick", "iss.classify", "iss.step1", "iss.step2", "iss.step3",
+      "iss.spare53", "iss.spare54", "iss.spare55"};
+  return k >= 0 && k < kProfSlotNames ? names[k] : "?";
+}
+inline bool prof_slot_is_counter(int k) { return (k >= 17 && k <= 19) || k == 30 || (k >= 32 && k <= 35); }
+
 constexpr const char* kRouterStepCapMsg = "router pass hit its step cap (-sim_router_step_cap / rt_step_cap)";
 
 struct IcntCapSink {
diff --git a/csrc/engine/gpu_engine.hip b/csrc/engine/gpu_engine.hip
--- a/csrc/engine/gpu_engine.hip
+++ b/csrc/engine/gpu_engine.hip
@@ -1244,15 +1244,7 @@
     if (!profiling_) return;
     std::vector<uint64_t> h((size_t)nblocks_ * kProfSlots);
     HIPCHECK(hipMemcpy(h.data(), d_prof_, h.size() * 8, hipMemcpyDeviceToHost));
-    static const char* names[kProfSlots] = {
-        "sm.receive", "sm.writeback", "sm.hit_complete", "sm.ldst", "sm.dispatch", "sm.read_operands",
-        "sm.alloc_oc", "sm.issue", "sm.fetch", "sm.retire", "sm.inject", "sm.occupancy", "sm.gather",
-        "sm.cta_dispatch", "sm.refill", "sm.cycle_loop", "sm.publish", "#sm_cycles", "#quiet_checks", "#epochs_busy", "mem.gather", "mem.dram",
-        "mem.l2", "mem.icnt", "mem.window_other", "mem.publish", "barrier", "decide", "post", "sm.issue_sched", "#slowest", "launch_rest",
-        "#max_work/epoch", "#epochs(b0)", "#last_arriver_wait", "#last_arrivals", "ldst.l1_probe", "ldst.mshr_find",
-        "ldst.pend_reg", "ldst.send", "recv.xbar", "recv.l1_fill", "issue.one", "issue.pick", "quiet_check", "skip",
-        "ldst.hit_push", "fill.pend_wake", "iss.pick", "iss.classify", "iss.step1", "iss.step2", "iss.step3",
-        "iss.spare53", "iss.spare54", "iss.spare55"};
+    static_assert(kProfSlots == kProfSlotNames, "engine.h prof_slot_name covers every slot");
     double sm[kProfSlots] = {}, mc[kProfSlots] = {}, smt = 0, mct = 0;
     for (uint32_t b = 0; b < nblocks_; ++b)
       for (int k = 0; k < kProfSlots; ++k) {
@@ -1317,7 +1309,7 @@
     for (int k = 0; k < kProfSlots; ++k) {
       const double cv = (double)h[(size_t)crit * kProfSlots + k];
       if (sm[k] + mc[k] > 0)
-        fprintf(stderr, "  %-18s SM %14.0f (%5.1f%%)   MEM %14.0f (%5.1f%%)   CRIT %14.0f (%5.1f%%)\n", names[k], sm[k],
+        fprintf(stderr, "  %-18s SM %14.0f (%5.1f%%)   MEM %14.0f (%5.1f%%)   CRIT %14.0f (%5.1f%%)\n", prof_slot_name(k), sm[k],
                 100 * sm[k] / smt, mc[k], 100 * mc[k] / mct, cv, 100 * cv / ct);
     }
   }
diff --git a/csrc/engine/seq_par_host.h b/csrc/engine/seq_par_host.h
--- /dev/null
+++ b/csrc/engine/seq_par_host.h
@@ -0,0 +1,77 @@
+#pragma once
+#include <stdint.h>
+
+#if defined(__x86_64__)
+#include <x86intrin.h>
+#else
+#include <chrono>
+#endif
+
+#include "../model/hd.h"
+
+namespace asim {
+
+struct alignas(64) SbCache {
+  uint64_t ok = 0;
+  uint64_t dirty = ~0ull;
+};
+
+constexpr int kHostProfSlots = 56;
+struct alignas(64) HostProf {
+  uint64_t last = 0;
+  uint32_t slot = 0;
+  uint32_t on = 0;
+  uint64_t acc[kHostProfSlots] = {};
+};
+
+inline uint64_t host_ticks() {
+#if defined(__x86_64__)
+  return __rdtsc();
+#else
+  return (uint64_t)std::chrono::steady_clock::now().time_since_epoch().count();
+#endif
+}
+
+struct SeqParTls {
+  static inline thread_local SbCache* sb __attribute__((tls_model("initial-exec"))) = nullptr;
+  static inline thread_local HostProf* pf __attribute__((tls_model("initial-exec"))) = nullptr;
+};
+
+template <bool kCache, bool kProf>
+struct SeqParHost : SeqPar {
+  static constexpr bool kSbCache = kCache;
+  template <class F>
+  static inline uint64_t sb_ok(uint64_t mask, F&& f) {
+    if constexpr (!kCache) {
+      return ballot_m(mask, f);
+    } else {
+      SbCache& k = *SeqParTls::sb;
+      const uint64_t ev = k.dirty & mask;
+      if (ev) {
+        k.ok = (k.ok & ~ev) | ballot_m(ev, f);
+        k.dirty &= ~ev;
+      }
+      return k.ok & mask;
+    }
+  }
+  static inline void sb_dirty(uint32_t w) {
+    if constexpr (kCache) SeqParTls::sb->dirty |= 1ull << w;
+  }
+  static inline void sb_dirty_m(uint64_t m) {
+    if constexpr (kCache) SeqParTls::sb->dirty |= m;
+  }
+  static inline void prof(int k) {
+    if constexpr (kProf) {
+      HostProf& p = *SeqParTls::pf;
+      const uint64_t t = host_ticks();
+      p.acc[p.slot] += t - p.last;
+      p.slot = (uint32_t)k;
+      p.last = t;
+    }
+  }
+  static inline void tick(int k) {
+    if constexpr (kProf) SeqParTls::pf->acc[k] += 1;
+  }
+};
+
+}
diff --git a/csrc/engine/wave_par.h b/csrc/engine/wave_par.h
--- a/csrc/engine/wave_par.h
+++ b/csrc/engine/wave_par.h
@@ -96,6 +96,13 @@
   static __device__ __forceinline__ void fetch_wait() { asm volatile("s_waitcnt vmcnt(0)" ::: "memory"); }
   static __device__ __forceinline__ void prof(int) {}
   static __device__ __forceinline__ void tick(int) {}
+  static constexpr bool kSbCache = false;
+  template <class F>
+  static __device__ __forceinline__ uint64_t sb_ok(uint64_t mask, F&& f) { return ballot_m(mask, f); }
+  static __device__ __forceinline__ void sb_dirty(uint32_t) {}
+  static __device__ __forceinline__ void sb_dirty_m(uint64_t) {}
+  template <class T>
+  using lane_ref = T;
   template <class T>
   static __device__ __forceinline__ T uni(T v) {
     static_assert(sizeof(T) <= 4 || sizeof(T) % 4 == 0, "uni: 1/2/4-byte or word-multiple types");
diff --git a/csrc/model/config.h b/csrc/model/config.h
--- a/csrc/model/config.h
+++ b/csrc/model/config.h
@@ -278,6 +278,8 @@
   uint32_t cpu_threads;
   uint32_t router_pass;
   uint64_t router_step_cap;
+  uint32_t dram_skip;
+  uint32_t issue_cache;
   uint32_t trace_mask;
   int32_t trace_sm;
   int32_t trace_mem;
diff --git a/csrc/model/epoch.h b/csrc/model/epoch.h
--- a/csrc/model/epoch.h
+++ b/csrc/model/epoch.h
@@ -352,7 +352,7 @@
   mem_publish<P>(ch, *x.cfg, x.outcnt, cur, dm);
   uint32_t idle = chan_idle(ch, *x.cfg) ? 1u : 0u;
   uint64_t nx = ~0ull;
-  if (x.cfg->event_skip) nx = chan_next_event(ch, *x.cfg, amin(ch.t_dram, amin(ch.t_l2, ch.t_icnt)));
+  if (x.cfg->event_skip) nx = chan_next_event<P>(ch, *x.cfg, amin(ch.t_dram, amin(ch.t_l2, ch.t_icnt)));
   nx = amin(nx, ch.min_emit);
   UnitPub u;
   u.next = nx;
diff --git a/csrc/model/hd.h b/csrc/model/hd.h
--- a/csrc/model/hd.h
+++ b/csrc/model/hd.h
@@ -72,6 +72,11 @@
   static SIM_HDI void sync() {}
   static SIM_HDI void prof(int) {}
   static SIM_HDI void tick(int) {}
+  static constexpr bool kSbCache = false;
+  template <class F>
+  static SIM_HDI uint64_t sb_ok(uint64_t mask, F&& f) { return ballot_m(mask, f); }
+  static SIM_HDI void sb_dirty(uint32_t) {}
+  static SIM_HDI void sb_dirty_m(uint64_t) {}
   template <class T>
   static SIM_HDI T uni(T v) { return v; }
   template <class S, class F>
@@ -110,11 +115,13 @@
     }
     return s;
   }
+  template <class T>
+  using lane_ref = const T&;
   template <class T, class F>
   struct Lanes {
     F f;
-    SIM_HDI T self(int i) const { return f(i); }
-    SIM_HDI T at(int i) const { return f(i); }
+    SIM_HDI decltype(auto) self(int i) const { return f(i); }
+    SIM_HDI decltype(auto) at(int i) const { return f(i); }
   };
   template <class T, class F>
   static SIM_HDI Lanes<T, F> lanes(int, F f) {
diff --git a/csrc/model/mem.h b/csrc/model/mem.h
--- a/csrc/model/mem.h
+++ b/csrc/model/mem.h
@@ -844,8 +844,61 @@
   return t + k * per;
 }
 
+template <class P>
+SIM_HDI uint64_t dram_next_cmd(const ChanState& ch, const SimCfg& c) {
+  const uint64_t t = ch.dcycle;
+  if (c.simple_dram) return amax<uint64_t>(t, ch.t_ccd_ok);
+  uint32_t only = 2;
+  if (c.wq_enable) {
+    const bool wm = ch.wmode ? !(ch.qw_n < c.wq_lo) : (ch.qw_n >= c.wq_hi);
+    if (wm != (ch.wmode != 0)) return t;
+    only = wm ? 1u : (ch.q_n > ch.qw_n ? 0u : 1u);
+  }
+  const int qn = (int)ch.q_hi;
+  uint64_t oldest_age = ~0ull;
+  uint64_t hitmask = 0;
+  if (c.dram_sched == 0) {
+    const int o = P::argmin(qn, [&](int i) -> uint64_t {
+      return (ch.q_valid[i] && (only == 2 || ch.q[i].write == only)) ? ch.q_age[i] : ~0ull;
+    });
+    if (o < 0) return ~0ull;
+    oldest_age = ch.q_age[o];
+  } else {
+    hitmask = P::vor(qn, [&](int i) -> uint64_t {
+      if (!ch.q_valid[i]) return 0;
+      const DramReq& r = ch.q[i];
+      if (only != 2 && r.write != only) return 0;
+      const DramBank& b = ch.bk[r.bank];
+      return (b.open && b.row == r.row) ? (1ull << r.bank) : 0ull;
+    });
+  }
+  uint64_t best = ~0ull;
+  P::lane_loop(qn, [&](int i) {
+    if (!ch.q_valid[i]) return;
+    if (c.dram_sched == 0 && ch.q_age[i] != oldest_age) return;
+    const DramReq& r = ch.q[i];
+    if (only != 2 && r.write != only) return;
+    const DramBank& b = ch.bk[r.bank];
+    uint64_t at;
+    if (b.open && b.row == r.row) {
+      at = amax<uint64_t>(b.t_col_ok, ch.t_ccd_ok);
+      at = amax<uint64_t>(at, ch.t_ccdl_ok[dram_bkgrp(c, r.bank) & 7]);
+      at = amax<uint64_t>(at, r.write ? ch.t_wr_ok : ch.t_rd_ok);
+    } else if (b.open) {
+      if (c.dram_sched != 0 && (hitmask >> r.bank & 1ull)) return;
+      at = b.t_pre_ok;
+    } else {
+      at = amax<uint64_t>(b.t_act_ok, ch.t_rrd_ok);
+    }
+    best = amin<uint64_t>(best, at);
+  });
+  best = P::uni(P::red_min64(best));
+  return best == ~0ull ? best : amax<uint64_t>(best, t);
+}
+
+template <class P>
 SIM_HDI uint64_t chan_next_event(const ChanState& ch, const SimCfg& c, uint64_t now) {
-  if (ch.q_n) return now;
+  if (ch.q_n && !c.dram_skip) return now;
   uint64_t nx = ~0ull;
   if (ch.lat_n) nx = amin(nx, ch.lat[ch.lat_head].ready);
   if (ch.ret_n) nx = amin(nx, ch.ret[ch.ret_head].ready);
@@ -857,6 +910,11 @@
     if (sp.rop_n) nx = amin(nx, sp.rop[sp.rop_head].t);
     if (sp.inq_n && sp.rop_n < (uint32_t)kRopQ && sp.rop_n < c.q_icnt_l2 + c.rop_latency)
       nx = amin(nx, sp.inq[sp.inq_head].t);
+  }
+  if (nx <= now) return now;
+  if (ch.q_n) {
+    const uint64_t dc = dram_next_cmd<P>(ch, c);
+    if (dc != ~0ull) nx = amin(nx, ch.t_dram + (dc - ch.dcycle) * c.per_dram);
   }
   return nx > now ? nx : now;
 }
@@ -897,7 +955,7 @@
     uint64_t tm = amin(ch.t_dram, amin(ch.t_l2, ch.t_icnt));
     if (tm >= t1) break;
     if (c.event_skip) {
-      const uint64_t nx = chan_next_event(ch, c, tm);
+      const uint64_t nx = chan_next_event<P>(ch, c, tm);
       if (nx > tm) {
         chan_quiet_advance(ch, c, amin(nx, t1));
         continue;
diff --git a/csrc/model/sm.h b/csrc/model/sm.h
--- a/csrc/model/sm.h
+++ b/csrc/model/sm.h
@@ -398,6 +398,7 @@
       });
     sbc(s.w_sb, e.warp, e.dst0);
     sbc(s.w_sb, e.warp, e.dst1);
+    P::sb_dirty(e.warp);
     s.w_inflight[e.warp]--;
     s.sadd(SK(rf_writes), (e.dst0 != 0) + (e.dst1 != 0));
   }
@@ -406,10 +407,11 @@
   s.wb_occ[slot >> 6] &= ~(1ull << (slot & 63));
 }
 
-template <class S>
+template <class P, class S>
 SIM_HDI void sm_load_slot_done(S& s, uint32_t w, uint32_t slot, uint64_t now) {
   sbc(s.w_sb, w, s.w_slot_dst[w][slot][0]);
   sbc(s.w_sb, w, s.w_slot_dst[w][slot][1]);
+  P::sb_dirty(w);
   s.sadd(SK(rf_writes), (s.w_slot_dst[w][slot][0] != 0) + (s.w_slot_dst[w][slot][1] != 0));
   s.w_slot_used[w] &= (uint8_t)~(1u << slot);
   s.w_slot_lds[w] &= (uint8_t)~(1u << slot);
@@ -435,7 +437,7 @@
   for (uint32_t i = 0; i < n; ++i) {
     HitEnt e = P::uni(s.hit[slot][i]);
     if (e.kind == 0) {
-      if (--s.w_slot_pend[e.warp][e.slot] == 0) sm_load_slot_done(s, e.warp, e.slot, now);
+      if (--s.w_slot_pend[e.warp][e.slot] == 0) sm_load_slot_done<P>(s, e.warp, e.slot, now);
     } else {
       s.w_inflight[e.warp]--;
       s.w_lds_st[e.warp]--;
@@ -459,13 +461,13 @@
   return true;
 }
 
-template <class S>
+template <class P, class S>
 SIM_HDI void sm_miss_access_done(S& s, const SimCfg& c, uint32_t w, uint32_t sl, uint64_t now) {
   if (c.l1_miss_ret) {
     for (uint32_t d = 0; d < 16; ++d)
       if (hit_push(s, now + c.l1_miss_ret + d, (uint8_t)w, (uint8_t)sl, 0)) return;
   }
-  if (--s.w_slot_pend[w][sl] == 0) sm_load_slot_done(s, w, sl, now);
+  if (--s.w_slot_pend[w][sl] == 0) sm_load_slot_done<P>(s, w, sl, now);
 }
 
 template <class P, class S>
@@ -558,7 +560,7 @@
       e.need &= (uint8_t)~sectors;
       if (e.need) continue;
       e.valid = 0;
-      sm_miss_access_done(s, c, e.warp, e.slot, now);
+      sm_miss_access_done<P>(s, c, e.warp, e.slot, now);
     }
   }
   while (s.n_pend && !s.pend[s.n_pend - 1].valid) s.n_pend--;
@@ -749,7 +751,7 @@
     s.last_progress = now;
   } else if (q.tag & 0x80000000u) {
     uint32_t w = q.tag & 0xff, sl = (q.tag >> 8) & 0xff;
-    sm_miss_access_done(s, c, w, sl, now);
+    sm_miss_access_done<P>(s, c, w, sl, now);
   } else {
     P::prof(41);
     l1_fill<P>(s, x, q.addr, q.sectors, now);
@@ -1187,6 +1189,7 @@
   if (trace_sm_on(c, TS_WARP_SCHEDULER, s.id))
     P::one([&] { trace_put(c, s.id, now, EV_ISSUE, (uint16_t)w, (uint64_t)in.pc | (uint64_t)in.opcode << 32); });
   s.w_head[w] = hidx + 1;
+  P::sb_dirty(w);
   s.w_ibuf[w] = (uint8_t)(P::uni((uint8_t)s.w_ibuf[w]) - 1);
   s.sadd(SK(warp_insn), 1);
   s.sadd(SK(thread_insn), (uint64_t)popc64(in.mask));
@@ -1287,12 +1290,7 @@
     return (f & WF_ACTIVE) && !(f & (WF_EXITING | WF_BARRIER | WF_MEMBAR | WF_WAITCNT)) && s.w_ibuf[w] != 0 &&
            warp_issue_due(s, c, w, now);
   });
-  sbok_m = P::ballot_m(valid_m, [&](int w) -> bool {
-    const TInst& in = s.w_win[w][s.w_head[w] & (kWin - 1)];
-    for (int j = 0; j < 5; ++j)
-      if (sbt(s.w_sb, w, in.src[j])) return false;
-    return !sbt(s.w_sb, w, in.dst[0]) && !sbt(s.w_sb, w, in.dst[1]);
-  });
+  sbok_m = P::sb_ok(valid_m, [&](int w) -> bool { return warp_sb_ok(s, w, s.w_win[w][s.w_head[w] & (kWin - 1)]); });
 }
 SIM_HDI uint32_t stall_class(uint64_t mine, uint64_t valid_m, uint64_t sbok_m) {
   return !(valid_m & mine) ? 0u : !(sbok_m & mine) ? 1u : 2u;
@@ -1447,6 +1445,7 @@
     sbs(s.w_sb, (uint32_t)w, in.dst[0]);
     sbs(s.w_sb, (uint32_t)w, in.dst[1]);
   });
+  P::sb_dirty_m(picks & ~spec);
   P::sync();
   P::prof(52);
   if (spec) {
@@ -1468,12 +1467,14 @@
   const uint32_t nsched = c.n_sched ? c.n_sched : 1;
   const uint64_t idoc_busy = P::uni(s.idoc_mask);
   P::fetch_wait();
-  const auto head = P::template lanes<TInst>(nw, [&](int w) -> TInst { return s.w_win[w][s.w_head[w] & (kWin - 1)]; });
+  const auto head = P::template lanes<TInst>(nw, [&](int w) -> typename P::template lane_ref<TInst> {
+    return s.w_win[w][s.w_head[w] & (kWin - 1)];
+  });
   const uint64_t live = P::uni(s.live_mask);
   if ((c.sched_policy == SCHED_LRR || c.sched_policy == SCHED_GTO || c.sched_policy == SCHED_OLDEST ||
        c.sched_policy == SCHED_RRR) &&
       c.max_issue_per_warp <= 1 && !trace_sm_on(c, TS_WARP_SCHEDULER, s.id)) {
-    const uint64_t sbok = P::ballot_m(live, [&](int w) -> bool { return warp_sb_ok(s, w, head.self(w)); });
+    const uint64_t sbok = P::sb_ok(live, [&](int w) -> bool { return warp_sb_ok(s, w, head.self(w)); });
     const uint64_t ready = P::ballot_m(live & sbok, [&](int w) -> bool {
       return warp_can_issue_nosb(s, c, w, head.self(w), nsched, idoc_busy) && warp_issue_due(s, c, w, now);
     });
@@ -1616,6 +1617,7 @@
     s.w_next[w] = wnext + n;
     s.w_ibuf[w] = (uint8_t)n;
     s.fetch_rr = w + 1;
+    P::sb_dirty(w);
   }
 }
 
@@ -1730,6 +1732,7 @@
   s.n_cta_active++;
   s.n_warps_live += wpc;
   s.live_mask |= wm;
+  P::sb_dirty_m(wm);
   uint32_t age0 = s.age_ctr;
   s.age_ctr += wpc;
   const uint32_t tag = ks << kSlotShift;
@@ -1828,6 +1831,9 @@
   }
   const int nw = (int)amin<uint32_t>(c.max_warps_per_sm, kMaxWarps);
   const uint32_t nsched = c.n_sched ? c.n_sched : 1;
+  uint64_t sbok = 0;
+  if constexpr (P::kSbCache)
+    sbok = P::sb_ok(P::uni(s.live_mask), [&](int w) -> bool { return warp_sb_ok(s, w, s.w_win[w][s.w_head[w] & (kWin - 1)]); });
   const uint64_t act = P::ballot_m(P::uni(s.live_mask), [&](int w) -> bool {
     const uint8_t f = s.w_flags[w];
     if (!(f & WF_ACTIVE)) return false;
@@ -1836,6 +1842,11 @@
     if (drained && s.w_inflight[w] == 0 && s.w_stores[w] == 0 && s.w_loads[w] == 0) return true;
     if ((f & WF_MEMBAR) && s.w_stores[w] == 0) return true;
     if ((f & WF_WAITCNT) && waitcnt_met(s, w)) return true;
+    if constexpr (P::kSbCache) {
+      if (!(sbok >> w & 1ull) || s.w_ibuf[w] == 0) return false;
+      return warp_can_issue_nosb(s, c, w, s.w_win[w][s.w_head[w] & (kWin - 1)], nsched, s.idoc_mask) &&
+             warp_issue_due(s, c, w, t);
+    }
     return warp_can_issue(s, c, kt, w, nsched, s.idoc_mask) && warp_issue_due(s, c, w, t);
   });
   if (act) return t;
```

After: 317,000 (median of 6 runs). +7.1%, better.
